# b0nes164/GPUSorting

Measured on NVIDIA H100. Metric: OneSweep sort throughput, 2^30 uint32 keys per GPU, keys-only, uniform-random, higher is better.
Workload: dtype u32

## Files before the change

gpusorting_b200/csrc/osb_common.cuh:

```cuda
#pragma once
#include <cstdint>
#include <type_traits>
#include <cuda_runtime.h>

namespace osb {

constexpr int kRadix = 256;
constexpr int kRadixLog = 8;

constexpr uint64_t kFlagNotReady = 0;
constexpr uint64_t kFlagReduction = 1;
constexpr uint64_t kFlagInclusive = 2;
constexpr uint64_t kFlagMask = 3;
constexpr int kValueBits = 38;
constexpr int kEpochShift = 40;
constexpr uint32_t kEpochMax = (1u << 24) - 1;

__host__ __device__ __forceinline__ uint64_t desc_pack(uint32_t epoch, uint64_t flag, uint64_t value)
{
    return (static_cast<uint64_t>(epoch) << kEpochShift) | ((value & ((1ull << kValueBits) - 1)) << 2) | flag;
}
__host__ __device__ __forceinline__ uint64_t desc_value(uint64_t d) { return (d >> 2) & ((1ull << kValueBits) - 1); }
__host__ __device__ __forceinline__ uint32_t desc_epoch(uint64_t d) { return static_cast<uint32_t>(d >> kEpochShift); }

__device__ __forceinline__ uint32_t lane_id() { uint32_t v; asm("mov.u32 %0, %%laneid;" : "=r"(v)); return v; }
__device__ __forceinline__ uint32_t lanemask_lt() { uint32_t v; asm("mov.u32 %0, %%lanemask_lt;" : "=r"(v)); return v; }

__device__ __forceinline__ uint64_t ld_relaxed_gpu_u64(const uint64_t* p)
{
    uint64_t v;
    asm volatile("ld.relaxed.gpu.global.u64 %0, [%1];" : "=l"(v) : "l"(p) : "memory");
    return v;
}
__device__ __forceinline__ void st_relaxed_gpu_u64(uint64_t* p, uint64_t v)
{
    asm volatile("st.relaxed.gpu.global.u64 [%0], %1;" ::"l"(p), "l"(v) : "memory");
}

template <typename T> __device__ __forceinline__ T ld_stream(const T* p) { return __ldcg(p); }
template <typename T> __device__ __forceinline__ void st_stream(T* p, T v) { __stcs(p, v); }
template <typename T> __device__ __forceinline__ void st_scatter(T* p, T v) { *p = v; }

struct KeyCodec {
    unsigned long long a = 0, b = 0, d = 0;
    uint32_t flags = 0;
};
constexpr uint32_t kCodecEncodeOnLoad = 1u, kCodecDecodeOnStore = 2u;
constexpr uint32_t kCodecFromPlan = 4u;

template <typename KeyT> __device__ __forceinline__ KeyT codec_encode(KeyT k, KeyT a, KeyT b, KeyT d)
{
    using S = typename std::make_signed<KeyT>::type;
    const KeyT sar = static_cast<KeyT>(static_cast<S>(k) >> (sizeof(KeyT) * 8 - 1));
    return k ^ (((sar & a) | b) ^ d);
}
template <typename KeyT> __device__ __forceinline__ KeyT codec_decode(KeyT e, KeyT a, KeyT b, KeyT d)
{
    using S = typename std::make_signed<KeyT>::type;
    e ^= d;
    const KeyT sar = static_cast<KeyT>(static_cast<S>(e) >> (sizeof(KeyT) * 8 - 1));
    return e ^ ((~sar & a) | b);
}

template <typename KeyT> __device__ __forceinline__ uint32_t digit_of(KeyT k, uint32_t shift)
{
    return static_cast<uint32_t>(k >> shift) & (kRadix - 1);
}
template <typename KeyT> __device__ __forceinline__ uint32_t digit_of(KeyT k, uint32_t shift, uint32_t mask)
{
    return static_cast<uint32_t>(k >> shift) & mask;
}

constexpr uint32_t kPlanHotShift = 16;
struct SortPlan {
    uint32_t skip_mask;
    uint32_t executed;
    uint32_t first_exec;
    uint32_t last_exec;
};
__device__ __forceinline__ bool plan_src_is_alt(const SortPlan& pl, uint32_t place)
{
    return __popc(~pl.skip_mask & ((1u << place) - 1u)) & 1u;
}

}
```

gpusorting_b200/csrc/osb_host.cu:

```cuda
#include <cstdio>
#include <cstring>
#include <new>

#include "../../include/onesweep_b200.h"
#include "osb_kernels.cuh"
#include "osb_common.cuh"
#include "osb_internal.h"

namespace {

constexpr int kVersion = 1006;
constexpr int kMaxPlaces = 8;

inline int cuda_status(cudaError_t e) { return e == cudaSuccess ? OSB200_OK : OSB200_ERR_CUDA - static_cast<int>(e); }

#define OSB_TRY(expr)                                      \
    do {                                                   \
        cudaError_t e__ = (expr);                          \
        if (e__ != cudaSuccess) return cuda_status(e__);   \
    } while (0)

struct ControlLayout {
    static constexpr size_t ghist_bytes = kMaxPlaces * osb::kRadix * sizeof(unsigned long long);
    static constexpr size_t ticket_bytes = 64;
    static constexpr size_t zeroed_bytes = ghist_bytes + ticket_bytes;
    static constexpr size_t gbase_bytes = kMaxPlaces * osb::kRadix * sizeof(unsigned long long);
    static constexpr size_t err_bytes = 64;
    static constexpr size_t plan_bytes = 64;
    static constexpr size_t total = zeroed_bytes + gbase_bytes + err_bytes + plan_bytes;
};

}

struct osb200_sorter {
    int device = 0;
    int sm_count = 132;
    uint64_t max_n = 0;
    int key_bytes = 4;
    int value_bytes = 0;
    osb::BinningConfig cfg;
    bool atomic_order_ok = false;
    bool short_circuit = true;
    bool small_path = true;
    bool hot_passes = true;
    bool debug_rows_block = false;

    void* alt_keys = nullptr;
    uint32_t* alt_vals = nullptr;
    unsigned char* control = nullptr;
    uint64_t* desc = nullptr;
    uint16_t* agg16 = nullptr;
    uint64_t desc_tiles = 0;
    uint32_t epoch = 0;

    bool profile = false;
    cudaEvent_t ev[kMaxPlaces + 3] = {};
    int ev_count = 0;

    void* stage_keys = nullptr;
    uint32_t* stage_vals = nullptr;
    cudaStream_t own_stream = nullptr;

    unsigned long long* ghist() const { return reinterpret_cast<unsigned long long*>(control); }
    uint32_t* tickets() const { return reinterpret_cast<uint32_t*>(control + ControlLayout::ghist_bytes); }
    unsigned long long* gbase() const { return reinterpret_cast<unsigned long long*>(control + ControlLayout::zeroed_bytes); }
    unsigned long long* err() const
    {
        return reinterpret_cast<unsigned long long*>(control + ControlLayout::zeroed_bytes + ControlLayout::gbase_bytes);
    }
    osb::SortPlan* plan() const
    {
        return reinterpret_cast<osb::SortPlan*>(control + ControlLayout::zeroed_bytes + ControlLayout::gbase_bytes + ControlLayout::err_bytes);
    }
};

namespace {

uint64_t tiles_for(uint64_t n, uint32_t tile_keys) { return (n + tile_keys - 1) / tile_keys; }
uint64_t agg_tiles_for(uint64_t n, uint32_t tile_keys) { return (tiles_for(n, tile_keys) + 7) / 8 * 8; }

uint32_t smallest_tile(int key_bytes, bool pairs)
{
    osb::BinningConfig c;
    uint32_t t = osb::binning_tile_keys(key_bytes, pairs, c);
    for (int v = 1; v < osb::kNumVariants; ++v) {
        c.variant = v;
        const uint32_t t2 = osb::binning_tile_keys(key_bytes, pairs, c);
        if (t2 < t) t = t2;
    }
    return t;
}

int next_epoch(osb200_sorter* s, cudaStream_t stream, uint32_t* out)
{
    if (s->epoch >= osb::kEpochMax) {
        OSB_TRY(cudaMemsetAsync(s->desc, 0, s->desc_tiles * osb::kRadix * sizeof(uint64_t), stream));
        s->epoch = 0;
    }
    *out = ++s->epoch;
    return OSB200_OK;
}

int is_capturing(cudaStream_t stream, bool* out)
{
    cudaStreamCaptureStatus st = cudaStreamCaptureStatusNone;
    OSB_TRY(cudaStreamGetCaptureInfo(stream, &st));
    *out = st == cudaStreamCaptureStatusActive;
    return OSB200_OK;
}

int check_handle(const osb200_sorter* s) { return s ? OSB200_OK : OSB200_ERR_INVALID_ARG; }

bool overlaps(uintptr_t a, uint64_t alen, uintptr_t b, uint64_t blen) { return a < b + blen && b < a + alen; }

int sort_impl(osb200_sorter* s, int key_bytes, void* d_keys, uint32_t* d_vals, uint64_t n, cudaStream_t stream,
              const osb::KeyCodec* codec = nullptr, int begin_bit = 0, int end_bit = -1, const void* keys_in = nullptr)
{
    const int key_bits = key_bytes * 8;
    if (end_bit < 0) end_bit = key_bits;
    if (begin_bit < 0 || end_bit > key_bits || begin_bit > end_bit) return OSB200_ERR_INVALID_ARG;
    if (n <= 1 || begin_bit == end_bit) return OSB200_OK;
    if (n > s->max_n) return OSB200_ERR_SIZE;
    if (!d_keys || (reinterpret_cast<uintptr_t>(d_keys) & 15u)) return OSB200_ERR_INVALID_ARG;
    if (d_vals && !s->value_bytes) return OSB200_ERR_INVALID_ARG;
    const int places = (end_bit - begin_bit + 7) / 8;
    const uint32_t last_bits = static_cast<uint32_t>(end_bit - begin_bit - 8 * (places - 1));
    const bool whole_key = begin_bit == 0 && end_bit == key_bits;
    const bool wide = s->cfg.variant == osb::kVariantWide;
    if (!wide && !whole_key) return OSB200_ERR_UNSUPPORTED;
    const bool use_plan = wide;

    if (wide && s->small_path && n <= osb::segment_sort_capacity(key_bytes)) {
        osb::KeyCodec c;
        if (codec) { c = *codec; c.flags = osb::kCodecEncodeOnLoad | osb::kCodecDecodeOnStore; }
        s->ev_count = 0;
        OSB_TRY(osb::launch_segment_sort(d_keys, d_vals, key_bytes, nullptr, 1, n, static_cast<uint32_t>(n),
                                         static_cast<uint32_t>(begin_bit), static_cast<uint32_t>(places), last_bits,
                                         codec ? &c : nullptr, s->cfg.rank_mode, s->sm_count, stream, keys_in));
        return OSB200_OK;
    }

    bool capturing = false;
    int st = is_capturing(stream, &capturing);
    if (st != OSB200_OK) return st;
    const uint32_t tile_keys = osb::binning_tile_keys(key_bytes, d_vals != nullptr, s->cfg);
    const size_t desc_bytes = tiles_for(n, tile_keys) * osb::kRadix * sizeof(uint64_t);
    if (capturing) OSB_TRY(cudaMemsetAsync(s->desc, 0, desc_bytes, stream));
    OSB_TRY(cudaMemsetAsync(s->control, 0, ControlLayout::zeroed_bytes, stream));
    const bool compact = s->cfg.variant != osb::kVariantTilePerCta;
    const uint64_t agg_stride = agg_tiles_for(n, tile_keys) * osb::kRadix;
    if (compact) OSB_TRY(cudaMemsetAsync(s->agg16, 0, agg_stride * places * sizeof(uint16_t), stream));
    int ne = 0;
    auto mark = [&]() -> cudaError_t {
        if (!s->profile) return cudaSuccess;
        if (!s->ev[ne]) { cudaError_t e = cudaEventCreate(&s->ev[ne]); if (e != cudaSuccess) return e; }
        return cudaEventRecord(s->ev[ne++], stream);
    };
    s->ev_count = 0;
    OSB_TRY(mark());
    osb::KeyCodec enc;
    if (codec) { enc = *codec; enc.flags = osb::kCodecEncodeOnLoad; }
    if (whole_key)
        OSB_TRY(osb::launch_global_histogram(keys_in ? keys_in : d_keys, n, key_bytes, s->ghist(), s->sm_count, stream,
                                             codec ? &enc : nullptr));
    else
        OSB_TRY(osb::launch_global_histogram_bits(d_keys, n, key_bytes, s->ghist(), s->sm_count, stream, codec ? &enc : nullptr,
                                                  static_cast<uint32_t>(begin_bit), places, last_bits));
    OSB_TRY(mark());
    const bool hot_passes = use_plan && s->hot_passes && osb::binning_has_hot_twin(key_bytes, d_vals != nullptr, keys_in != nullptr, s->cfg);
    OSB_TRY(osb::launch_scan(s->ghist(), s->gbase(), places, stream, use_plan ? s->plan() : nullptr, n, s->short_circuit, hot_passes));
    OSB_TRY(mark());

    void* src = d_keys;
    void* dst = s->alt_keys;
    uint32_t* sv = d_vals;
    uint32_t* dv = d_vals ? s->alt_vals : nullptr;
    for (int p = 0; p < places; ++p) {
        uint32_t epoch = 0;
        st = next_epoch(s, stream, &epoch);
        if (st != OSB200_OK) return st;
        osb::BinningConfig cfg = s->cfg;
        cfg.digit_bits = p == places - 1 ? last_bits : 8u;
        cfg.place = static_cast<uint32_t>(p);
        if (use_plan) cfg.plan = s->plan();
        cfg.hot_passes = hot_passes;
        cfg.argsort_in = keys_in;
        if (codec) {
            cfg.codec = *codec;
            cfg.codec.flags = use_plan ? osb::kCodecFromPlan
                                       : (p == 0 ? osb::kCodecEncodeOnLoad : 0u) | (p == places - 1 ? osb::kCodecDecodeOnStore : 0u);
        }
        OSB_TRY(osb::launch_digit_binning(use_plan ? d_keys : src, use_plan ? s->alt_keys : dst, use_plan ? d_vals : sv,
                                          use_plan ? (d_vals ? s->alt_vals : nullptr) : dv, n, key_bytes,
                                          static_cast<uint32_t>(begin_bit + 8 * p), s->gbase() + p * osb::kRadix, s->desc,
                                          s->agg16 + p * agg_stride, s->tickets() + p, epoch, cfg, stream));
        OSB_TRY(mark());
        void* t = src; src = dst; dst = t;
        uint32_t* tv = sv; sv = dv; dv = tv;
    }
    if (use_plan && (s->short_circuit || (places & 1))) {
        if (keys_in)
            OSB_TRY(osb::launch_argsort_copy_back(s->plan(), keys_in, s->alt_keys, d_keys, s->alt_vals, d_vals, n, key_bytes, s->sm_count,
                                                      stream));
        else
            OSB_TRY(osb::launch_copy_back(s->plan(), s->alt_keys, d_keys, d_vals ? s->alt_vals : nullptr, d_vals, n, key_bytes,
                                          s->sm_count, stream));
    }
    if (capturing) OSB_TRY(cudaMemsetAsync(s->desc, 0, desc_bytes, stream));
    s->ev_count = ne;
    return OSB200_OK;
}

int ensure_staging(osb200_sorter* s)
{
    if (!s->own_stream) OSB_TRY(cudaStreamCreateWithFlags(&s->own_stream, cudaStreamNonBlocking));
    if (!s->stage_keys) {
        if (cudaMalloc(&s->stage_keys, s->max_n * s->key_bytes) != cudaSuccess) return OSB200_ERR_ALLOC;
    }
    if (s->value_bytes && !s->stage_vals) {
        if (cudaMalloc(&s->stage_vals, s->max_n * sizeof(uint32_t)) != cudaSuccess) return OSB200_ERR_ALLOC;
    }
    return OSB200_OK;
}

int sort_host_impl(osb200_sorter* s, void* h_keys, uint32_t* h_vals, uint64_t n)
{
    if (n <= 1) return OSB200_OK;
    if (n > s->max_n) return OSB200_ERR_SIZE;
    if (!h_keys || (h_vals && !s->value_bytes)) return OSB200_ERR_INVALID_ARG;
    int st = ensure_staging(s);
    if (st != OSB200_OK) return st;
    cudaStream_t q = s->own_stream;
    OSB_TRY(cudaMemcpyAsync(s->stage_keys, h_keys, n * s->key_bytes, cudaMemcpyHostToDevice, q));
    if (h_vals) OSB_TRY(cudaMemcpyAsync(s->stage_vals, h_vals, n * sizeof(uint32_t), cudaMemcpyHostToDevice, q));
    st = sort_impl(s, s->key_bytes, s->stage_keys, h_vals ? s->stage_vals : nullptr, n, q);
    if (st != OSB200_OK) return st;
    OSB_TRY(cudaMemcpyAsync(h_keys, s->stage_keys, n * s->key_bytes, cudaMemcpyDeviceToHost, q));
    if (h_vals) OSB_TRY(cudaMemcpyAsync(h_vals, s->stage_vals, n * sizeof(uint32_t), cudaMemcpyDeviceToHost, q));
    OSB_TRY(cudaStreamSynchronize(q));
    return OSB200_OK;
}

}

int osb_internal_digit_histogram(osb200_handle h, const void* d_in, uint64_t n, uint32_t shift,
                                 unsigned long long* d_hist256, cudaStream_t stream)
{
    OSB_TRY(cudaMemsetAsync(d_hist256, 0, osb::kRadix * sizeof(unsigned long long), stream));
    if (n) OSB_TRY(osb::launch_digit_histogram(d_in, n, h->key_bytes, shift, d_hist256, h->sm_count, stream));
    return OSB200_OK;
}

int osb_internal_binning_pass(osb200_handle h, const void* d_in, void* d_out, uint64_t n, uint32_t shift,
                              const unsigned long long* d_hist256, const unsigned long long* out_base,
                              cudaStream_t stream)
{
    if (n == 0) return OSB200_OK;
    if (n > h->max_n) return OSB200_ERR_SIZE;
    const unsigned long long* base = out_base;
    OSB_TRY(cudaMemsetAsync(h->tickets(), 0, ControlLayout::ticket_bytes, stream));
    if (!base) {
        OSB_TRY(osb::launch_scan(d_hist256, h->gbase(), 1, stream));
        base = h->gbase();
    }
    if (h->cfg.variant != osb::kVariantTilePerCta) {
        const uint64_t tiles = agg_tiles_for(n, osb::binning_tile_keys(h->key_bytes, false, h->cfg));
        OSB_TRY(cudaMemsetAsync(h->agg16, 0, tiles * osb::kRadix * sizeof(uint16_t), stream));
    }
    uint32_t epoch = 0;
    int st = next_epoch(h, stream, &epoch);
    if (st != OSB200_OK) return st;
    osb::BinningConfig cfg = h->cfg;
    const uint32_t key_bits = static_cast<uint32_t>(h->key_bytes) * 8u;
    cfg.digit_bits = key_bits - shift < 8u ? key_bits - shift : 8u;
    OSB_TRY(osb::launch_digit_binning(d_in, d_out, nullptr, nullptr, n, h->key_bytes, shift, base, h->desc, h->agg16,
                                      h->tickets(), epoch, cfg, stream));
    return OSB200_OK;
}

extern "C" {

int osb200_version(void) { return kVersion; }

const char* osb200_status_string(int status)
{
    switch (status) {
        case OSB200_OK: return "ok";
        case OSB200_ERR_INVALID_ARG: return "invalid argument";
        case OSB200_ERR_SIZE: return "n exceeds the sorter's max_n";
        case OSB200_ERR_UNSUPPORTED: return "unsupported key/value combination";
        case OSB200_ERR_NO_DEVICE: return "no usable sm_90 CUDA device";
        case OSB200_ERR_ALLOC: return "device allocation failed";
        case OSB200_ERR_NCCL: return "NCCL error";
        default: break;
    }
    if (status <= OSB200_ERR_CUDA) return cudaGetErrorString(static_cast<cudaError_t>(OSB200_ERR_CUDA - status));
    return "unknown status";
}

uint64_t osb200_workspace_bytes(uint64_t max_n, int key_bytes, int value_bytes)
{
    if ((key_bytes != 4 && key_bytes != 8) || (value_bytes != 0 && value_bytes != 4)) return 0;
    const uint64_t tiles = tiles_for(max_n ? max_n : 1, smallest_tile(key_bytes, value_bytes != 0));
    return max_n * key_bytes + max_n * value_bytes + tiles * osb::kRadix * sizeof(uint64_t) +
           (tiles + 8) * osb::kRadix * sizeof(uint16_t) * key_bytes + ControlLayout::total;
}

}

namespace {

int create_impl(osb200_handle* out, uint64_t max_n, int key_bytes, int value_bytes)
{
    if (max_n == 0 || max_n > (1ull << 34)) return OSB200_ERR_INVALID_ARG;

    int dev = 0;
    if (cudaGetDevice(&dev) != cudaSuccess) { cudaGetLastError(); return OSB200_ERR_NO_DEVICE; }
    cudaDeviceProp prop;
    if (cudaGetDeviceProperties(&prop, dev) != cudaSuccess) { cudaGetLastError(); return OSB200_ERR_NO_DEVICE; }
    if (prop.major != 9 || prop.minor != 0) return OSB200_ERR_NO_DEVICE;

    osb200_sorter* s = new (std::nothrow) osb200_sorter();
    if (!s) return OSB200_ERR_ALLOC;
    s->device = dev;
    s->sm_count = prop.multiProcessorCount;
    s->cfg.sm_count = s->sm_count;
    s->cfg.variant = osb::kVariantWide;
    s->max_n = max_n;
    s->key_bytes = key_bytes;
    s->value_bytes = value_bytes;

    cudaError_t e = osb::configure_kernels();
    if (e != cudaSuccess) { delete s; return cuda_status(e); }

    s->desc_tiles = tiles_for(max_n, smallest_tile(key_bytes, value_bytes != 0));
    bool ok = cudaMalloc(&s->alt_keys, max_n * key_bytes) == cudaSuccess;
    if (ok && value_bytes) ok = cudaMalloc(&s->alt_vals, max_n * sizeof(uint32_t)) == cudaSuccess;
    ok = ok && cudaMalloc(&s->control, ControlLayout::total) == cudaSuccess;
    ok = ok && cudaMalloc(&s->desc, s->desc_tiles * osb::kRadix * sizeof(uint64_t)) == cudaSuccess;
    ok = ok && cudaMalloc(&s->agg16, (s->desc_tiles + 8) * osb::kRadix * sizeof(uint16_t) * key_bytes) == cudaSuccess;
    if (!ok) { cudaGetLastError(); osb200_destroy(s); return OSB200_ERR_ALLOC; }
    e = cudaMemset(s->desc, 0, s->desc_tiles * osb::kRadix * sizeof(uint64_t));
    if (e == cudaSuccess) e = cudaMemset(s->control, 0, ControlLayout::total);

    if (e == cudaSuccess) e = osb::launch_atomic_order_selftest(s->err(), s->sm_count, nullptr);
    unsigned long long mism = 1;
    if (e == cudaSuccess) e = cudaMemcpy(&mism, s->err(), sizeof(mism), cudaMemcpyDeviceToHost);
    if (e != cudaSuccess) { osb200_destroy(s); return cuda_status(e); }
    s->atomic_order_ok = (mism == 0);
    s->cfg.rank_mode = s->atomic_order_ok ? osb::kRankAtomic : osb::kRankBallot;
    *out = s;
    return OSB200_OK;
}

}

extern "C" {

int osb200_create(osb200_handle* out, uint64_t max_n, int key_bytes, int value_bytes)
{
    if (!out) return OSB200_ERR_INVALID_ARG;
    *out = nullptr;
    if ((key_bytes != 4 && key_bytes != 8) || (value_bytes != 0 && value_bytes != 4)) return OSB200_ERR_INVALID_ARG;
    if (key_bytes == 8 && value_bytes != 0) return OSB200_ERR_UNSUPPORTED;
    return create_impl(out, max_n, key_bytes, value_bytes);
}

int osb200_create_pairs64(osb200_handle* out, uint64_t max_n)
{
    if (!out) return OSB200_ERR_INVALID_ARG;
    *out = nullptr;
    return create_impl(out, max_n, 8, 4);
}

int osb200_destroy(osb200_handle h)
{
    if (!h) return OSB200_ERR_INVALID_ARG;
    cudaFree(h->alt_keys);
    cudaFree(h->alt_vals);
    cudaFree(h->control);
    cudaFree(h->desc);
    cudaFree(h->agg16);
    cudaFree(h->stage_keys);
    cudaFree(h->stage_vals);
    if (h->own_stream) cudaStreamDestroy(h->own_stream);
    for (cudaEvent_t e : h->ev) if (e) cudaEventDestroy(e);
    delete h;
    return OSB200_OK;
}

int osb200_sort_keys_u32(osb200_handle h, uint32_t* d_keys, uint64_t n, void* stream)
{
    if (check_handle(h) != OSB200_OK || h->key_bytes != 4) return OSB200_ERR_INVALID_ARG;
    return sort_impl(h, h->key_bytes, d_keys, nullptr, n, static_cast<cudaStream_t>(stream));
}

int osb200_sort_pairs_u32(osb200_handle h, uint32_t* d_keys, uint32_t* d_values, uint64_t n, void* stream)
{
    if (check_handle(h) != OSB200_OK || h->key_bytes != 4 || h->value_bytes != 4) return OSB200_ERR_INVALID_ARG;
    if (n > 1 && !d_values) return OSB200_ERR_INVALID_ARG;
    return sort_impl(h, h->key_bytes, d_keys, d_values, n, static_cast<cudaStream_t>(stream));
}

int osb200_sort_keys_u64(osb200_handle h, uint64_t* d_keys, uint64_t n, void* stream)
{
    if (check_handle(h) != OSB200_OK || h->key_bytes != 8) return OSB200_ERR_INVALID_ARG;
    return sort_impl(h, h->key_bytes, d_keys, nullptr, n, static_cast<cudaStream_t>(stream));
}

static int make_codec(int key_bytes, int key_type, int descending, osb::KeyCodec* c, const osb::KeyCodec** codec)
{
    const bool wide64 = key_bytes == 8;
    const unsigned long long all = wide64 ? ~0ull : 0xffffffffull, sign = wide64 ? (1ull << 63) : (1ull << 31);
    switch (key_type) {
        case OSB200_KEY_U32: if (wide64) return OSB200_ERR_INVALID_ARG; c->a = 0; c->b = 0; break;
        case OSB200_KEY_I32: if (wide64) return OSB200_ERR_INVALID_ARG; c->a = 0; c->b = sign; break;
        case OSB200_KEY_F32: if (wide64) return OSB200_ERR_INVALID_ARG; c->a = all; c->b = sign; break;
        case OSB200_KEY_U64: if (!wide64) return OSB200_ERR_INVALID_ARG; c->a = 0; c->b = 0; break;
        case OSB200_KEY_I64: if (!wide64) return OSB200_ERR_INVALID_ARG; c->a = 0; c->b = sign; break;
        case OSB200_KEY_F64: if (!wide64) return OSB200_ERR_INVALID_ARG; c->a = all; c->b = sign; break;
        default: return OSB200_ERR_INVALID_ARG;
    }
    c->d = descending ? all : 0;
    c->flags = 0;
    *codec = c->a == 0 && c->b == 0 && c->d == 0 ? nullptr : c;
    return OSB200_OK;
}

static int make_codec16(int key_type, int descending, osb::KeyCodec* c, const osb::KeyCodec** codec)
{
    switch (key_type) {
        case OSB200_KEY16_U16: c->a = 0; c->b = 0; break;
        case OSB200_KEY16_I16: c->a = 0; c->b = 0x8000u; break;
        case OSB200_KEY16_F16:
        case OSB200_KEY16_BF16: c->a = 0xFFFFu; c->b = 0x8000u; break;
        default: return OSB200_ERR_INVALID_ARG;
    }
    c->d = descending ? 0xFFFFu : 0;
    c->flags = 0;
    *codec = c->a == 0 && c->b == 0 && c->d == 0 ? nullptr : c;
    return OSB200_OK;
}

static int typed_codec(const osb200_sorter* h, int key_bytes, int key_type, int descending, osb::KeyCodec* c, const osb::KeyCodec** codec)
{
    const int st = key_bytes == 2 ? make_codec16(key_type, descending, c, codec) : make_codec(key_bytes, key_type, descending, c, codec);
    if (st != OSB200_OK) return st;
    return h->cfg.variant == osb::kVariantWide ? OSB200_OK : OSB200_ERR_UNSUPPORTED;
}

static int typed_sort(osb200_sorter* h, int key_bytes, void* d_keys, uint32_t* d_vals, bool pairs, uint64_t n, int key_type,
                      int descending, void* stream)
{
    osb::KeyCodec c;
    const osb::KeyCodec* codec = nullptr;
    const int st = typed_codec(h, key_bytes, key_type, descending, &c, &codec);
    if (st != OSB200_OK) return st;
    if (pairs && n > 1 && !d_vals) return OSB200_ERR_INVALID_ARG;
    return sort_impl(h, key_bytes, d_keys, d_vals, n, static_cast<cudaStream_t>(stream), codec);
}

static int argsort_impl(osb200_sorter* h, int key_bytes, const void* d_keys_in, void* d_keys_out, uint32_t* d_indices, uint64_t n,
                        int key_type, int descending, void* stream)
{
    osb::KeyCodec c;
    const osb::KeyCodec* codec = nullptr;
    const int st = typed_codec(h, key_bytes, key_type, descending, &c, &codec);
    if (st != OSB200_OK) return st;
    if (n == 0) return OSB200_OK;
    const uintptr_t in = reinterpret_cast<uintptr_t>(d_keys_in), out = reinterpret_cast<uintptr_t>(d_keys_out),
                    idx = reinterpret_cast<uintptr_t>(d_indices);
    if (!in || !out || !idx || ((in | out | idx) & 15u)) return OSB200_ERR_INVALID_ARG;
    if (n > h->max_n || n > (1ull << 32)) return OSB200_ERR_SIZE;
    const uint64_t kb = n * static_cast<uint64_t>(key_bytes), ib = n * sizeof(uint32_t);
    if (overlaps(in, kb, out, kb) || overlaps(in, kb, idx, ib) || overlaps(out, kb, idx, ib)) return OSB200_ERR_INVALID_ARG;
    cudaStream_t q = static_cast<cudaStream_t>(stream);
    if (n == 1) {
        OSB_TRY(cudaMemcpyAsync(d_keys_out, d_keys_in, key_bytes, cudaMemcpyDeviceToDevice, q));
        OSB_TRY(cudaMemsetAsync(d_indices, 0, sizeof(uint32_t), q));
        return OSB200_OK;
    }
    return sort_impl(h, key_bytes, d_keys_out, d_indices, n, q, codec, 0, -1, d_keys_in);
}

int osb200_sort_keys_typed(osb200_handle h, void* d_keys, uint64_t n, int key_type, int descending, void* stream)
{
    if (check_handle(h) != OSB200_OK) return OSB200_ERR_INVALID_ARG;
    return typed_sort(h, h->key_bytes, d_keys, nullptr, false, n, key_type, descending, stream);
}

int osb200_segmented_sort_u32(osb200_handle h, uint32_t* d_keys, uint32_t* d_values, const uint64_t* d_segment_offsets,
                              uint64_t num_segments, uint32_t max_segment_len, void* stream)
{
    if (check_handle(h) != OSB200_OK) return OSB200_ERR_INVALID_ARG;
    if (h->key_bytes != 4 || (d_values && h->value_bytes != 4)) return OSB200_ERR_INVALID_ARG;
    if (num_segments == 0 || max_segment_len <= 1) return OSB200_OK;
    if (!d_keys || !d_segment_offsets) return OSB200_ERR_INVALID_ARG;
    if (max_segment_len > osb::segment_sort_capacity(4)) return OSB200_ERR_SIZE;
    OSB_TRY(osb::launch_segment_sort(d_keys, d_values, 4, reinterpret_cast<const unsigned long long*>(d_segment_offsets), num_segments,
                                     0, max_segment_len, 0, 4, 8, nullptr, h->cfg.rank_mode, h->sm_count,
                                     static_cast<cudaStream_t>(stream)));
    return OSB200_OK;
}

int osb200_sort_bits(osb200_handle h, void* d_keys, uint32_t* d_values, uint64_t n, int begin_bit, int end_bit, void* stream)
{
    if (check_handle(h) != OSB200_OK) return OSB200_ERR_INVALID_ARG;
    if (d_values && (h->key_bytes != 4 || h->value_bytes != 4)) return OSB200_ERR_INVALID_ARG;
    return sort_impl(h, h->key_bytes, d_keys, d_values, n, static_cast<cudaStream_t>(stream), nullptr, begin_bit, end_bit);
}

int osb200_sort_pairs_typed(osb200_handle h, void* d_keys, uint32_t* d_values, uint64_t n, int key_type, int descending,
                            void* stream)
{
    if (check_handle(h) != OSB200_OK || h->value_bytes != 4) return OSB200_ERR_INVALID_ARG;
    if (n > 1 && !d_values) return OSB200_ERR_INVALID_ARG;
    return typed_sort(h, h->key_bytes, d_keys, d_values, true, n, key_type, descending, stream);
}

int osb200_argsort(osb200_handle h, const void* d_keys_in, void* d_keys_out, uint32_t* d_indices, uint64_t n, int key_type,
                   int descending, void* stream)
{
    if (check_handle(h) != OSB200_OK || h->value_bytes != 4) return OSB200_ERR_INVALID_ARG;
    return argsort_impl(h, h->key_bytes, d_keys_in, d_keys_out, d_indices, n, key_type, descending, stream);
}

int osb200_sort_keys16(osb200_handle h, void* d_keys, uint64_t n, int key_type, int descending, void* stream)
{
    if (check_handle(h) != OSB200_OK || h->key_bytes != 4) return OSB200_ERR_INVALID_ARG;
    return typed_sort(h, 2, d_keys, nullptr, false, n, key_type, descending, stream);
}

int osb200_sort_pairs16(osb200_handle h, void* d_keys, uint32_t* d_values, uint64_t n, int key_type, int descending, void* stream)
{
    if (check_handle(h) != OSB200_OK || h->key_bytes != 4 || h->value_bytes != 4) return OSB200_ERR_INVALID_ARG;
    return typed_sort(h, 2, d_keys, d_values, true, n, key_type, descending, stream);
}

int osb200_argsort16(osb200_handle h, const void* d_keys_in, void* d_keys_out, uint32_t* d_indices, uint64_t n, int key_type,
                     int descending, void* stream)
{
    if (check_handle(h) != OSB200_OK || h->key_bytes != 4 || h->value_bytes != 4) return OSB200_ERR_INVALID_ARG;
    return argsort_impl(h, 2, d_keys_in, d_keys_out, d_indices, n, key_type, descending, stream);
}

int osb200_sort_rows(osb200_handle h, const void* d_keys_in, void* d_keys_out, uint32_t* d_indices, uint64_t num_rows,
                     uint32_t row_len, int key_bytes, int key_type, int descending, void* stream)
{
    if (check_handle(h) != OSB200_OK) return OSB200_ERR_INVALID_ARG;
    osb::KeyCodec c;
    const osb::KeyCodec* codec = nullptr;
    int st = key_bytes == 2 ? make_codec16(key_type, descending, &c, &codec)
             : key_bytes == 4 || key_bytes == 8 ? make_codec(key_bytes, key_type, descending, &c, &codec)
                                                : OSB200_ERR_INVALID_ARG;
    if (st != OSB200_OK) return st;
    if (num_rows == 0 || row_len == 0) return OSB200_OK;
    const uintptr_t in = reinterpret_cast<uintptr_t>(d_keys_in), out = reinterpret_cast<uintptr_t>(d_keys_out),
                    idx = reinterpret_cast<uintptr_t>(d_indices);
    if (!in || !out) return OSB200_ERR_INVALID_ARG;
    if (((in | out) & static_cast<uintptr_t>(key_bytes - 1)) || (idx & 3u)) return OSB200_ERR_INVALID_ARG;
    if (num_rows > UINT64_MAX / row_len) return OSB200_ERR_INVALID_ARG;
    const uint64_t n = num_rows * row_len;
    if (n > UINT64_MAX / 8) return OSB200_ERR_INVALID_ARG;
    const uint64_t kb = n * static_cast<uint64_t>(key_bytes), ib = n * sizeof(uint32_t);
    if ((in != out && overlaps(in, kb, out, kb)) || (idx && (overlaps(in, kb, idx, ib) || overlaps(out, kb, idx, ib))))
        return OSB200_ERR_INVALID_ARG;
    if (row_len > osb::row_sort_capacity(key_bytes)) return OSB200_ERR_SIZE;
    cudaStream_t q = static_cast<cudaStream_t>(stream);
    if (row_len == 1) {
        if (in != out) OSB_TRY(cudaMemcpyAsync(d_keys_out, d_keys_in, kb, cudaMemcpyDeviceToDevice, q));
        if (idx) OSB_TRY(cudaMemsetAsync(d_indices, 0, ib, q));
        return OSB200_OK;
    }
    c.flags = osb::kCodecEncodeOnLoad | osb::kCodecDecodeOnStore;
    OSB_TRY(osb::launch_row_sort(d_keys_in, d_keys_out, d_indices, num_rows, row_len, key_bytes, codec,
                                 h->cfg.rank_mode, h->debug_rows_block, h->sm_count, q));
    return OSB200_OK;
}

int osb200_sort_host_keys_u32(osb200_handle h, uint32_t* h_keys, uint64_t n)
{
    if (check_handle(h) != OSB200_OK || h->key_bytes != 4) return OSB200_ERR_INVALID_ARG;
    return sort_host_impl(h, h_keys, nullptr, n);
}

int osb200_sort_host_pairs_u32(osb200_handle h, uint32_t* h_keys, uint32_t* h_values, uint64_t n)
{
    if (check_handle(h) != OSB200_OK || h->key_bytes != 4 || h->value_bytes != 4) return OSB200_ERR_INVALID_ARG;
    if (n > 1 && !h_values) return OSB200_ERR_INVALID_ARG;
    return sort_host_impl(h, h_keys, h_values, n);
}

int osb200_sort_host_keys_u64(osb200_handle h, uint64_t* h_keys, uint64_t n)
{
    if (check_handle(h) != OSB200_OK || h->key_bytes != 8) return OSB200_ERR_INVALID_ARG;
    return sort_host_impl(h, h_keys, nullptr, n);
}

int osb200_global_histogram(osb200_handle h, const void* d_keys, uint64_t n, uint64_t* d_hist, void* stream)
{
    if (check_handle(h) != OSB200_OK || !d_hist || (n && !d_keys)) return OSB200_ERR_INVALID_ARG;
    if (reinterpret_cast<uintptr_t>(d_keys) & 15u) return OSB200_ERR_INVALID_ARG;
    cudaStream_t q = static_cast<cudaStream_t>(stream);
    OSB_TRY(cudaMemsetAsync(d_hist, 0, static_cast<size_t>(h->key_bytes) * osb::kRadix * sizeof(uint64_t), q));
    if (n == 0) return OSB200_OK;
    OSB_TRY(osb::launch_global_histogram(d_keys, n, h->key_bytes, reinterpret_cast<unsigned long long*>(d_hist),
                                         h->sm_count, q));
    return OSB200_OK;
}

int osb200_digit_binning_pass(osb200_handle h, const void* d_in, void* d_out, const uint32_t* d_in_values,
                              uint32_t* d_out_values, uint64_t n, uint32_t radix_shift, void* stream)
{
    if (check_handle(h) != OSB200_OK) return OSB200_ERR_INVALID_ARG;
    if (n == 0) return OSB200_OK;
    if (!d_in || !d_out || d_in == d_out) return OSB200_ERR_INVALID_ARG;
    if ((reinterpret_cast<uintptr_t>(d_in) & 15u) || (reinterpret_cast<uintptr_t>(d_out) & 15u)) return OSB200_ERR_INVALID_ARG;
    if (n > h->max_n) return OSB200_ERR_SIZE;
    if (radix_shift >= static_cast<uint32_t>(h->key_bytes) * 8u) return OSB200_ERR_INVALID_ARG;
    if ((d_in_values != nullptr) != (d_out_values != nullptr)) return OSB200_ERR_INVALID_ARG;
    if (d_in_values && (h->key_bytes != 4 || h->value_bytes != 4)) return OSB200_ERR_UNSUPPORTED;
    cudaStream_t q = static_cast<cudaStream_t>(stream);
    bool capturing = false;
    int st = is_capturing(q, &capturing);
    if (st != OSB200_OK) return st;
    const size_t desc_bytes = tiles_for(n, osb::binning_tile_keys(h->key_bytes, d_in_values != nullptr, h->cfg)) * osb::kRadix *
                              sizeof(uint64_t);
    if (capturing) OSB_TRY(cudaMemsetAsync(h->desc, 0, desc_bytes, q));
    st = osb_internal_digit_histogram(h, d_in, n, radix_shift, h->ghist(), q);
    if (st != OSB200_OK) return st;
    OSB_TRY(cudaMemsetAsync(h->tickets(), 0, ControlLayout::ticket_bytes, q));
    OSB_TRY(osb::launch_scan(h->ghist(), h->gbase(), 1, q));
    if (h->cfg.variant != osb::kVariantTilePerCta)
        OSB_TRY(cudaMemsetAsync(h->agg16, 0, (h->desc_tiles + 8) * osb::kRadix * sizeof(uint16_t), q));
    uint32_t epoch = 0;
    st = next_epoch(h, q, &epoch);
    if (st != OSB200_OK) return st;
    osb::BinningConfig cfg = h->cfg;
    const uint32_t key_bits = static_cast<uint32_t>(h->key_bytes) * 8u;
    cfg.digit_bits = key_bits - radix_shift < 8u ? key_bits - radix_shift : 8u;
    OSB_TRY(osb::launch_digit_binning(d_in, d_out, d_in_values, d_out_values, n, h->key_bytes, radix_shift, h->gbase(), h->desc,
                                      h->agg16, h->tickets(), epoch, cfg, q));
    if (capturing) OSB_TRY(cudaMemsetAsync(h->desc, 0, desc_bytes, q));
    return OSB200_OK;
}

int osb200_debug_digit_histogram(osb200_handle h, const uint32_t* d_in, uint64_t n, uint32_t shift, uint64_t* d_hist256,
                                 void* stream)
{
    if (check_handle(h) != OSB200_OK || h->key_bytes != 4 || !d_hist256 || shift >= 32) return OSB200_ERR_INVALID_ARG;
    if (n && (!d_in || (reinterpret_cast<uintptr_t>(d_in) & 15u))) return OSB200_ERR_INVALID_ARG;
    if (n > h->max_n) return OSB200_ERR_SIZE;
    return osb_internal_digit_histogram(h, d_in, n, shift, reinterpret_cast<unsigned long long*>(d_hist256),
                                        static_cast<cudaStream_t>(stream));
}

int osb200_debug_exchange_pass(osb200_handle h, const uint32_t* d_in, uint32_t* d_out, uint64_t n, uint32_t shift,
                               const uint64_t* d_hist256, const uint64_t* d_out_base, void* stream)
{
    if (check_handle(h) != OSB200_OK || h->key_bytes != 4 || shift >= 32) return OSB200_ERR_INVALID_ARG;
    if (d_out_base && d_out) return OSB200_ERR_INVALID_ARG;
    if (n == 0) return OSB200_OK;
    if (!d_in || (reinterpret_cast<uintptr_t>(d_in) & 15u) || d_in == d_out) return OSB200_ERR_INVALID_ARG;
    if (!d_out_base && (!d_out || !d_hist256 || (reinterpret_cast<uintptr_t>(d_out) & 3u))) return OSB200_ERR_INVALID_ARG;
    if (n > h->max_n) return OSB200_ERR_SIZE;
    return osb_internal_binning_pass(h, d_in, d_out, n, shift, reinterpret_cast<const unsigned long long*>(d_hist256),
                                     reinterpret_cast<const unsigned long long*>(d_out_base), static_cast<cudaStream_t>(stream));
}

int osb200_validate(osb200_handle h, const void* d_keys, uint64_t n, uint64_t* h_err_count, void* stream)
{
    if (check_handle(h) != OSB200_OK || !h_err_count) return OSB200_ERR_INVALID_ARG;
    *h_err_count = 0;
    if (n < 2) return OSB200_OK;
    if (!d_keys) return OSB200_ERR_INVALID_ARG;
    cudaStream_t q = static_cast<cudaStream_t>(stream);
    OSB_TRY(cudaMemsetAsync(h->err(), 0, sizeof(unsigned long long), q));
    OSB_TRY(osb::launch_validate(d_keys, n, h->key_bytes, h->err(), h->sm_count, q));
    unsigned long long v = 0;
    OSB_TRY(cudaMemcpyAsync(&v, h->err(), sizeof(v), cudaMemcpyDeviceToHost, q));
    OSB_TRY(cudaStreamSynchronize(q));
    *h_err_count = v;
    return OSB200_OK;
}

int osb200_init_random_u32(uint32_t* d_keys, uint32_t* d_payload, uint64_t n, uint32_t and_count, uint32_t seed,
                           int payload_is_index, void* stream)
{
    if (n == 0) return OSB200_OK;
    if (!d_keys) return OSB200_ERR_INVALID_ARG;
    OSB_TRY(osb::launch_init_random(d_keys, d_payload, n, and_count, seed, payload_is_index != 0,
                                    static_cast<cudaStream_t>(stream)));
    return OSB200_OK;
}

int osb200_set_option(osb200_handle h, const char* key, int64_t value)
{
    if (check_handle(h) != OSB200_OK || !key) return OSB200_ERR_INVALID_ARG;
    if (!std::strcmp(key, "rank_mode")) {
        if (value != osb::kRankAtomic && value != osb::kRankBallot) return OSB200_ERR_INVALID_ARG;
        if (value == osb::kRankAtomic && !h->atomic_order_ok) return OSB200_ERR_UNSUPPORTED;
        h->cfg.rank_mode = static_cast<int>(value);
        return OSB200_OK;
    }
    if (!std::strcmp(key, "profile")) { h->profile = value != 0; return OSB200_OK; }
    if (!std::strcmp(key, "short_circuit")) { h->short_circuit = value != 0; return OSB200_OK; }
    if (!std::strcmp(key, "small_path")) { h->small_path = value != 0; return OSB200_OK; }
    if (!std::strcmp(key, "hot_passes")) { h->hot_passes = value != 0; return OSB200_OK; }
    if (!std::strcmp(key, "spin_cap")) {
        if (value < 1 || value > (1ll << 30)) return OSB200_ERR_INVALID_ARG;
        h->cfg.spin_cap = static_cast<uint32_t>(value);
        return OSB200_OK;
    }
    if (!std::strcmp(key, "debug_stall_every")) {
        if (value < 0 || value > (1ll << 30)) return OSB200_ERR_INVALID_ARG;
        h->cfg.debug_stall_every = static_cast<uint32_t>(value);
        return OSB200_OK;
    }
    if (!std::strcmp(key, "debug_max_ctas")) {
        if (value < 0 || value > (1ll << 30)) return OSB200_ERR_INVALID_ARG;
        h->cfg.debug_max_ctas = static_cast<uint32_t>(value);
        return OSB200_OK;
    }
    if (!std::strcmp(key, "debug_rows_block")) { h->debug_rows_block = value != 0; return OSB200_OK; }
    if (!std::strcmp(key, "debug_epoch")) {
        if (value < 0 || value > osb::kEpochMax) return OSB200_ERR_INVALID_ARG;
        h->epoch = static_cast<uint32_t>(value);
        return OSB200_OK;
    }
    if (!std::strcmp(key, "variant")) {
        if (value < 0 || value >= osb::kNumVariants) return OSB200_ERR_INVALID_ARG;
        h->cfg.variant = static_cast<int>(value);
        return OSB200_OK;
    }
    return OSB200_ERR_INVALID_ARG;
}

int osb200_get_profile(osb200_handle h, float* out_ms, int capacity)
{
    if (check_handle(h) != OSB200_OK || !out_ms) return OSB200_ERR_INVALID_ARG;
    if (h->ev_count < 2) return 0;
    OSB_TRY(cudaEventSynchronize(h->ev[h->ev_count - 1]));
    int k = 0;
    for (int i = 0; i + 1 < h->ev_count && k < capacity; ++i, ++k) OSB_TRY(cudaEventElapsedTime(&out_ms[k], h->ev[i], h->ev[i + 1]));
    return k;
}

int64_t osb200_get_info(osb200_handle h, const char* key)
{
    if (check_handle(h) != OSB200_OK || !key) return OSB200_ERR_INVALID_ARG;
    if (!std::strcmp(key, "tile_keys")) return osb::binning_tile_keys(h->key_bytes, h->value_bytes != 0, h->cfg);
    if (!std::strcmp(key, "launches_per_sort")) {
        const bool wide = h->cfg.variant == osb::kVariantWide;
        const bool cb = wide && h->short_circuit;
        return 2 + h->key_bytes * ((wide && h->hot_passes) ? 2 : 1) + (cb ? (h->value_bytes ? 2 : 1) : 0);
    }
    if (!std::strcmp(key, "memsets_per_sort")) return h->cfg.variant != osb::kVariantTilePerCta ? 2 : 1;
    if (!std::strcmp(key, "short_circuit")) return h->short_circuit ? 1 : 0;
    if (!std::strcmp(key, "small_path")) return h->small_path ? 1 : 0;
    if (!std::strcmp(key, "hot_passes")) return h->hot_passes ? 1 : 0;
    if (!std::strcmp(key, "last_hot_mask")) {
        osb::SortPlan pl;
        if (cudaMemcpy(&pl, h->plan(), sizeof(pl), cudaMemcpyDeviceToHost) != cudaSuccess) return -1;
        return static_cast<int>((pl.skip_mask >> osb::kPlanHotShift) & 0xffu);
    }
    if (!std::strcmp(key, "small_path_max_n")) return osb::segment_sort_capacity(h->key_bytes);
    if (!std::strcmp(key, "spin_cap")) return h->cfg.spin_cap;
    if (!std::strcmp(key, "last_skip_mask") || !std::strcmp(key, "last_executed_passes")) {
        osb::SortPlan pl;
        if (cudaMemcpy(&pl, h->plan(), sizeof(pl), cudaMemcpyDeviceToHost) != cudaSuccess) return OSB200_ERR_CUDA;
        return key[5] == 's' ? static_cast<int64_t>(pl.skip_mask & 0xffffu) : static_cast<int64_t>(pl.executed);
    }
    if (!std::strcmp(key, "sm_count")) return h->sm_count;
    if (!std::strcmp(key, "rank_mode")) return h->cfg.rank_mode;
    if (!std::strcmp(key, "variant")) return h->cfg.variant;
    if (!std::strcmp(key, "atomic_order_ok")) return h->atomic_order_ok ? 1 : 0;
    if (!std::strcmp(key, "max_n")) return static_cast<int64_t>(h->max_n);
    if (!std::strcmp(key, "epoch")) return h->epoch;
    return OSB200_ERR_INVALID_ARG;
}

}
```

gpusorting_b200/csrc/osb_kernels.cu:

```cuda
#include <type_traits>

#include "osb_kernels.cuh"
#include "osb_common.cuh"

namespace osb {

template <typename... Ts> struct TypeList {};

template <typename... Ts, typename F>
static cudaError_t for_each_type(TypeList<Ts...>, F&& f)
{
    cudaError_t e = cudaSuccess;
    (void)(((e = f(Ts{})) == cudaSuccess) && ...);
    return e;
}

template <typename... Ts, typename M, typename F>
static cudaError_t find_type(TypeList<Ts...>, M&& match, F&& f)
{
    cudaError_t e = cudaErrorInvalidValue;
    (void)((match(Ts{}) && ((e = f(Ts{})), true)) || ...);
    return e;
}

template <typename... Keys, typename F>
static cudaError_t with_key_type(TypeList<Keys...> keys, int key_bytes, F&& f)
{
    return find_type(keys, [&](auto k) { return key_bytes == static_cast<int>(sizeof(k)); }, f);
}

template <typename F>
static cudaError_t with_rank_mode(int rank_mode, F&& f)
{
    return rank_mode == kRankBallot ? f(std::integral_constant<int, kRankBallot>{}) : f(std::integral_constant<int, kRankAtomic>{});
}

static unsigned capped_grid(uint64_t work, uint64_t per_cta, uint64_t cap)
{
    uint64_t want = (work + per_cta - 1) / per_cta;
    if (want < 1) want = 1;
    return static_cast<unsigned>(want < cap ? want : cap);
}

template <typename K>
static cudaError_t set_smem(K* kernel, size_t bytes)
{
    return cudaFuncSetAttribute(kernel, cudaFuncAttributeMaxDynamicSharedMemorySize, static_cast<int>(bytes));
}

template <typename Shape>
static cudaError_t configure_shape(Shape)
{
    cudaError_t e = set_smem(Shape::template kernel<kRankAtomic>(), Shape::smem);
    if (e == cudaSuccess) e = set_smem(Shape::template kernel<kRankBallot>(), Shape::smem);
    if constexpr (Shape::has_hot) {
        if (e == cudaSuccess) e = set_smem(Shape::template kernel<kRankAtomic, true>(), Shape::smem);
        if (e == cudaSuccess) e = set_smem(Shape::template kernel<kRankBallot, true>(), Shape::smem);
    }
    return e;
}

constexpr int kHistThreads = 1024;

template <typename KeyT> struct HistGeom;
template <> struct HistGeom<uint32_t> { static constexpr int COLS = 32; };
template <> struct HistGeom<uint64_t> { static constexpr int COLS = 16; };
template <> struct HistGeom<uint16_t> { static constexpr int COLS = 32; };

template <typename KeyT, bool MASKED = false>
__device__ __forceinline__ void hist_count_word(uint32_t* s_col, uint32_t w, int word_in_vec, int places = 0, uint32_t last_mask = 255u)
{
    constexpr int PLACES = sizeof(KeyT);
    constexpr int COLS = HistGeom<KeyT>::COLS;
#pragma unroll
    for (int q = 0; q < 4; ++q) {
        const int place = (word_in_vec * 4 + q) % PLACES;
        if constexpr (MASKED) {
            if (place < places)
                atomicAdd(&s_col[(place * kRadix + ((w >> (8 * q)) & (place == places - 1 ? last_mask : 255u))) * COLS], 1u);
        } else {
            atomicAdd(&s_col[(place * kRadix + ((w >> (8 * q)) & 255u)) * COLS], 1u);
        }
    }
}

template <typename KeyT>
__device__ __forceinline__ uint4 hist_encode_vec(uint4 v, const KeyCodec& c)
{
    if constexpr (sizeof(KeyT) == 4) {
        const uint32_t a = static_cast<uint32_t>(c.a), b = static_cast<uint32_t>(c.b), d = static_cast<uint32_t>(c.d);
        v.x = codec_encode<uint32_t>(v.x, a, b, d); v.y = codec_encode<uint32_t>(v.y, a, b, d);
        v.z = codec_encode<uint32_t>(v.z, a, b, d); v.w = codec_encode<uint32_t>(v.w, a, b, d);
    } else if constexpr (sizeof(KeyT) == 2) {
        const uint16_t a = static_cast<uint16_t>(c.a), b = static_cast<uint16_t>(c.b), d = static_cast<uint16_t>(c.d);
        auto enc2 = [&](uint32_t w) {
            return static_cast<uint32_t>(codec_encode<uint16_t>(static_cast<uint16_t>(w), a, b, d)) |
                   (static_cast<uint32_t>(codec_encode<uint16_t>(static_cast<uint16_t>(w >> 16), a, b, d)) << 16);
        };
        v.x = enc2(v.x); v.y = enc2(v.y); v.z = enc2(v.z); v.w = enc2(v.w);
    } else {
        unsigned long long k0 = (static_cast<unsigned long long>(v.y) << 32) | v.x, k1 = (static_cast<unsigned long long>(v.w) << 32) | v.z;
        k0 = codec_encode<unsigned long long>(k0, c.a, c.b, c.d); k1 = codec_encode<unsigned long long>(k1, c.a, c.b, c.d);
        v.x = static_cast<uint32_t>(k0); v.y = static_cast<uint32_t>(k0 >> 32); v.z = static_cast<uint32_t>(k1); v.w = static_cast<uint32_t>(k1 >> 32);
    }
    return v;
}

template <typename KeyT, bool MASKED = false>
__device__ __forceinline__ void hist_count_vec(uint32_t* s_col, const uint4& v, int places = 0, uint32_t last_mask = 255u)
{
    hist_count_word<KeyT, MASKED>(s_col, v.x, 0, places, last_mask);
    hist_count_word<KeyT, MASKED>(s_col, v.y, 1, places, last_mask);
    hist_count_word<KeyT, MASKED>(s_col, v.z, 2, places, last_mask);
    hist_count_word<KeyT, MASKED>(s_col, v.w, 3, places, last_mask);
}

template <typename KeyT, bool MASKED = false>
__global__ void __launch_bounds__(kHistThreads, 1)
global_histogram_kernel(const KeyT* __restrict__ keys, uint64_t n, unsigned long long* __restrict__ ghist, KeyCodec codec,
                        int places = 0, uint32_t last_mask = 255u)
{
    constexpr int PLACES = sizeof(KeyT);
    constexpr int VEC = 16 / sizeof(KeyT);
    constexpr int COLS = HistGeom<KeyT>::COLS;
    constexpr int BINS = PLACES * kRadix;
    extern __shared__ __align__(16) uint32_t s_hist[];
    for (int i = threadIdx.x; i < BINS * COLS; i += kHistThreads) s_hist[i] = 0;
    __syncthreads();
    uint32_t* s_col = s_hist + (threadIdx.x & (COLS - 1));

    const uint64_t nvec = n / VEC;
    const uint4* __restrict__ vp = reinterpret_cast<const uint4*>(keys);
    const uint64_t stride = static_cast<uint64_t>(gridDim.x) * kHistThreads;
    uint64_t i = static_cast<uint64_t>(blockIdx.x) * kHistThreads + threadIdx.x;
    const bool enc = codec.flags & kCodecEncodeOnLoad;
    for (; i + 3 * stride < nvec; i += 4 * stride) {
        uint4 a = __ldcs(vp + i);
        uint4 b = __ldcs(vp + i + stride);
        uint4 c = __ldcs(vp + i + 2 * stride);
        uint4 d = __ldcs(vp + i + 3 * stride);
        if (enc) { a = hist_encode_vec<KeyT>(a, codec); b = hist_encode_vec<KeyT>(b, codec); c = hist_encode_vec<KeyT>(c, codec); d = hist_encode_vec<KeyT>(d, codec); }
        hist_count_vec<KeyT, MASKED>(s_col, a, places, last_mask);
        hist_count_vec<KeyT, MASKED>(s_col, b, places, last_mask);
        hist_count_vec<KeyT, MASKED>(s_col, c, places, last_mask);
        hist_count_vec<KeyT, MASKED>(s_col, d, places, last_mask);
    }
    for (; i < nvec; i += stride) {
        uint4 a = __ldcs(vp + i);
        if (enc) a = hist_encode_vec<KeyT>(a, codec);
        hist_count_vec<KeyT, MASKED>(s_col, a, places, last_mask);
    }
    if (blockIdx.x == 0) {
        const uint64_t t = nvec * VEC + threadIdx.x;
        if (t < n) {
            KeyT k = keys[t];
            if (enc) k = codec_encode<KeyT>(k, static_cast<KeyT>(codec.a), static_cast<KeyT>(codec.b), static_cast<KeyT>(codec.d));
#pragma unroll
            for (int p = 0; p < PLACES; ++p) {
                if (MASKED && p >= places) break;
                const uint32_t m = (MASKED && p == places - 1) ? last_mask : 255u;
                atomicAdd(&s_col[(p * kRadix + (static_cast<uint32_t>(k >> (8 * p)) & m)) * COLS], 1u);
            }
        }
    }
    __syncthreads();
    for (int bin = threadIdx.x; bin < BINS; bin += kHistThreads) {
        uint32_t sum = 0;
#pragma unroll 8
        for (int c = 0; c < COLS; ++c) sum += s_hist[bin * COLS + ((c + threadIdx.x) & (COLS - 1))];
        if (sum) atomicAdd(&ghist[bin], static_cast<unsigned long long>(sum));
    }
}

template <typename KeyT> constexpr size_t hist_smem_bytes() { return sizeof(KeyT) * kRadix * HistGeom<KeyT>::COLS * sizeof(uint32_t); }

using HistKeys = TypeList<uint16_t, uint32_t, uint64_t>;
using HistBitsKeys = TypeList<uint32_t, uint64_t>;

template <typename KeyT, bool MASKED>
static cudaError_t launch_histogram_vec(const void* keys, uint64_t n, unsigned long long* ghist, int sm_count, cudaStream_t stream,
                                        const KeyCodec& codec, int places = 0, uint32_t last_mask = 255u)
{
    const unsigned grid = capped_grid(n / (16 / sizeof(KeyT)), kHistThreads, sm_count);
    global_histogram_kernel<KeyT, MASKED><<<grid, kHistThreads, hist_smem_bytes<KeyT>(), stream>>>(
        static_cast<const KeyT*>(keys), n, ghist, codec, places, last_mask);
    return cudaGetLastError();
}

cudaError_t launch_global_histogram(const void* keys, uint64_t n, int key_bytes, unsigned long long* ghist,
                                    int sm_count, cudaStream_t stream, const KeyCodec* codec_in)
{
    const KeyCodec codec = codec_in ? *codec_in : KeyCodec();
    return with_key_type(HistKeys{}, key_bytes, [&](auto k) {
        return launch_histogram_vec<decltype(k), false>(keys, n, ghist, sm_count, stream, codec);
    });
}

template <typename KeyT>
__global__ void __launch_bounds__(kHistThreads, 1)
digit_histogram_kernel(const KeyT* __restrict__ keys, uint64_t n, uint32_t shift, unsigned long long* __restrict__ hist256)
{
    __shared__ uint32_t s_hist[kRadix * 32];
    for (int i = threadIdx.x; i < kRadix * 32; i += kHistThreads) s_hist[i] = 0;
    __syncthreads();
    uint32_t* s_col = s_hist + (threadIdx.x & 31);
    const uint64_t stride = static_cast<uint64_t>(gridDim.x) * kHistThreads;
    uint64_t i = static_cast<uint64_t>(blockIdx.x) * kHistThreads + threadIdx.x;
    for (; i + 3 * stride < n; i += 4 * stride) {
        const KeyT a = __ldcs(keys + i), b = __ldcs(keys + i + stride), c = __ldcs(keys + i + 2 * stride),
                   d = __ldcs(keys + i + 3 * stride);
        atomicAdd(&s_col[digit_of(a, shift) * 32], 1u);
        atomicAdd(&s_col[digit_of(b, shift) * 32], 1u);
        atomicAdd(&s_col[digit_of(c, shift) * 32], 1u);
        atomicAdd(&s_col[digit_of(d, shift) * 32], 1u);
    }
    for (; i < n; i += stride) atomicAdd(&s_col[digit_of(__ldcs(keys + i), shift) * 32], 1u);
    __syncthreads();
    for (int bin = threadIdx.x; bin < kRadix; bin += kHistThreads) {
        uint32_t sum = 0;
#pragma unroll 8
        for (int c = 0; c < 32; ++c) sum += s_hist[bin * 32 + ((c + threadIdx.x) & 31)];
        if (sum) atomicAdd(&hist256[bin], static_cast<unsigned long long>(sum));
    }
}

cudaError_t launch_digit_histogram(const void* keys, uint64_t n, int key_bytes, uint32_t shift,
                                   unsigned long long* hist256, int sm_count, cudaStream_t stream)
{
    const unsigned grid = capped_grid(n, kHistThreads * 4, static_cast<uint64_t>(sm_count) * 2);
    return with_key_type(TypeList<uint32_t, uint64_t>{}, key_bytes, [&](auto k) {
        using KeyT = decltype(k);
        digit_histogram_kernel<KeyT><<<grid, kHistThreads, 0, stream>>>(static_cast<const KeyT*>(keys), n, shift, hist256);
        return cudaGetLastError();
    });
}

__global__ void __launch_bounds__(kRadix)
scan_kernel(const unsigned long long* __restrict__ ghist, unsigned long long* __restrict__ gbase, int places,
            SortPlan* plan, unsigned long long n, int allow_skip, int allow_hot)
{
    __shared__ unsigned long long s_warp[kRadix / 32];
    const int d = threadIdx.x, lane = d & 31, warp = d >> 5;
    uint32_t skip_mask = 0;
    for (int p = 0; p < places; ++p) {
        const unsigned long long c = ghist[p * kRadix + d];
        unsigned long long incl = c;
#pragma unroll
        for (int o = 1; o < 32; o <<= 1) {
            const unsigned long long t = __shfl_up_sync(0xffffffffu, incl, o);
            if (lane >= o) incl += t;
        }
        if (lane == 31) s_warp[warp] = incl;
        const int single_bin = __syncthreads_or(plan != nullptr && allow_skip && c == n);
        const int hot_bin = __syncthreads_or(plan != nullptr && allow_hot && n >= (1ull << 22) && c * 8ull >= n);
        unsigned long long pre = 0;
        for (int w = 0; w < warp; ++w) pre += s_warp[w];
        gbase[p * kRadix + d] = pre + incl - c;
        if (single_bin) skip_mask |= 1u << p;
        else if (hot_bin) skip_mask |= 1u << (kPlanHotShift + p);
        __syncthreads();
    }
    if (plan != nullptr && d == 0) {
        SortPlan pl;
        pl.skip_mask = skip_mask;
        const uint32_t run = ~skip_mask & ((places >= 32 ? 0u : (1u << places)) - 1u);
        pl.executed = __popc(run);
        pl.first_exec = run ? static_cast<uint32_t>(__ffs(run) - 1) : 0xffffffffu;
        pl.last_exec = run ? static_cast<uint32_t>(31 - __clz(run)) : 0xffffffffu;
        *plan = pl;
    }
}

cudaError_t launch_scan(const unsigned long long* ghist, unsigned long long* gbase, int places, cudaStream_t stream,
                        SortPlan* plan, uint64_t n, bool allow_skip, bool allow_hot)
{
    scan_kernel<<<1, kRadix, 0, stream>>>(ghist, gbase, places, plan, n, allow_skip ? 1 : 0, allow_hot ? 1 : 0);
    return cudaGetLastError();
}

template <typename KeyT>
__global__ void __launch_bounds__(kHistThreads, 1)
global_histogram_bits_kernel(const KeyT* __restrict__ keys, uint64_t n, unsigned long long* __restrict__ ghist, KeyCodec codec,
                             uint32_t begin_bit, int places, uint32_t last_mask)
{
    constexpr int COLS = HistGeom<KeyT>::COLS;
    extern __shared__ __align__(16) uint32_t s_hist[];
    const int bins = places * kRadix;
    for (int i = threadIdx.x; i < bins * COLS; i += kHistThreads) s_hist[i] = 0;
    __syncthreads();
    uint32_t* s_col = s_hist + (threadIdx.x & (COLS - 1));
    const bool enc = codec.flags & kCodecEncodeOnLoad;
    const KeyT ca = static_cast<KeyT>(codec.a), cb = static_cast<KeyT>(codec.b), cd = static_cast<KeyT>(codec.d);
    const uint64_t stride = static_cast<uint64_t>(gridDim.x) * kHistThreads;
    for (uint64_t i = static_cast<uint64_t>(blockIdx.x) * kHistThreads + threadIdx.x; i < n; i += stride) {
        KeyT k = __ldcs(keys + i);
        if (enc) k = codec_encode<KeyT>(k, ca, cb, cd);
        for (int p = 0; p < places; ++p) {
            const uint32_t dg = digit_of(k, begin_bit + 8u * p, p == places - 1 ? last_mask : 255u);
            atomicAdd(&s_col[(p * kRadix + dg) * COLS], 1u);
        }
    }
    __syncthreads();
    for (int bin = threadIdx.x; bin < bins; bin += kHistThreads) {
        uint32_t sum = 0;
#pragma unroll 8
        for (int c = 0; c < COLS; ++c) sum += s_hist[bin * COLS + ((c + threadIdx.x) & (COLS - 1))];
        if (sum) atomicAdd(&ghist[bin], static_cast<unsigned long long>(sum));
    }
}

cudaError_t launch_global_histogram_bits(const void* keys, uint64_t n, int key_bytes, unsigned long long* ghist, int sm_count,
                                         cudaStream_t stream, const KeyCodec* codec_in, uint32_t begin_bit, int places,
                                         uint32_t last_bits)
{
    const KeyCodec codec = codec_in ? *codec_in : KeyCodec();
    const uint32_t last_mask = (1u << last_bits) - 1u;
    return with_key_type(HistBitsKeys{}, key_bytes, [&](auto k) {
        using KeyT = decltype(k);
        if (begin_bit == 0) return launch_histogram_vec<KeyT, true>(keys, n, ghist, sm_count, stream, codec, places, last_mask);
        global_histogram_bits_kernel<KeyT><<<capped_grid(n, kHistThreads * 4, sm_count), kHistThreads, hist_smem_bytes<KeyT>(), stream>>>(
            static_cast<const KeyT*>(keys), n, ghist, codec, begin_bit, places, last_mask);
        return cudaGetLastError();
    });
}

template <typename W>
__global__ void __launch_bounds__(512)
copy_back_kernel(const SortPlan* __restrict__ plan, const W* __restrict__ src, W* __restrict__ dst, uint64_t words,
                 const unsigned char* __restrict__ src_tail, unsigned char* __restrict__ dst_tail, uint32_t tail_bytes)
{
    if (!(plan->executed & 1u)) return;
    const uint64_t stride = static_cast<uint64_t>(gridDim.x) * blockDim.x;
    for (uint64_t i = static_cast<uint64_t>(blockIdx.x) * blockDim.x + threadIdx.x; i < words; i += stride) __stcs(dst + i, __ldcs(src + i));
    if (blockIdx.x == 0 && threadIdx.x < tail_bytes) dst_tail[threadIdx.x] = src_tail[threadIdx.x];
}

cudaError_t launch_copy_back(const SortPlan* plan, const void* alt_keys, void* keys, const uint32_t* alt_vals, uint32_t* vals,
                             uint64_t n, int key_bytes, int sm_count, cudaStream_t stream)
{
    auto launch = [&](auto word, const void* s, void* d, uint64_t bytes) {
        using W = decltype(word);
        const uint64_t words = bytes / sizeof(W);
        copy_back_kernel<W><<<capped_grid(words, 512, static_cast<uint64_t>(sm_count) * 4), 512, 0, stream>>>(plan, static_cast<const W*>(s), static_cast<W*>(d), words,
                                                      static_cast<const unsigned char*>(s) + words * sizeof(W),
                                                      static_cast<unsigned char*>(d) + words * sizeof(W),
                                                      static_cast<uint32_t>(bytes - words * sizeof(W)));
    };
    auto one = [&](const void* s, void* d, uint64_t bytes) {
        if (((reinterpret_cast<uintptr_t>(s) | reinterpret_cast<uintptr_t>(d)) & 15u) == 0) launch(uint4{}, s, d, bytes);
        else launch(uint32_t{}, s, d, bytes);
    };
    one(alt_keys, keys, n * key_bytes);
    if (vals) one(alt_vals, vals, n * sizeof(uint32_t));
    return cudaGetLastError();
}

template <typename KeyT>
__global__ void __launch_bounds__(512)
argsort_copy_back_kernel(const SortPlan* __restrict__ plan, const KeyT* __restrict__ keys_in, const KeyT* __restrict__ alt_keys,
                         KeyT* __restrict__ keys, const uint32_t* __restrict__ alt_idx, uint32_t* __restrict__ idx, uint64_t n)
{
    using KV = typename std::conditional<sizeof(KeyT) == 2, uint2, uint4>::type;
    constexpr int KV_PER_STEP = 4 * sizeof(KeyT) / sizeof(KV);
    static_assert(KV_PER_STEP * sizeof(KV) == 4 * sizeof(KeyT), "four keys per step");
    const uint32_t ex = plan->executed;
    if (ex != 0 && !(ex & 1u)) return;
    const KeyT* src = ex ? alt_keys : keys_in;
    const uint64_t vecs = n / 4, stride = static_cast<uint64_t>(gridDim.x) * blockDim.x;
    for (uint64_t i = static_cast<uint64_t>(blockIdx.x) * blockDim.x + threadIdx.x; i < vecs; i += stride) {
#pragma unroll
        for (int v = 0; v < KV_PER_STEP; ++v)
            __stcs(reinterpret_cast<KV*>(keys) + i * KV_PER_STEP + v, __ldcs(reinterpret_cast<const KV*>(src) + i * KV_PER_STEP + v));
        const uint32_t b = static_cast<uint32_t>(i * 4);
        __stcs(reinterpret_cast<uint4*>(idx) + i, ex ? __ldcs(reinterpret_cast<const uint4*>(alt_idx) + i) : make_uint4(b, b + 1, b + 2, b + 3));
    }
    if (blockIdx.x == 0 && threadIdx.x < (n & 3u)) {
        const uint64_t j = vecs * 4 + threadIdx.x;
        keys[j] = src[j];
        idx[j] = ex ? alt_idx[j] : static_cast<uint32_t>(j);
    }
}

cudaError_t launch_argsort_copy_back(const SortPlan* plan, const void* keys_in, const void* alt_keys, void* keys,
                                     const uint32_t* alt_idx, uint32_t* idx, uint64_t n, int key_bytes, int sm_count,
                                     cudaStream_t stream)
{
    const unsigned grid = capped_grid(n / 4, 512, static_cast<uint64_t>(sm_count) * 4);
    return with_key_type(TypeList<uint16_t, uint32_t, uint64_t>{}, key_bytes, [&](auto k) {
        using KeyT = decltype(k);
        argsort_copy_back_kernel<KeyT><<<grid, 512, 0, stream>>>(plan, static_cast<const KeyT*>(keys_in), static_cast<const KeyT*>(alt_keys),
                                                                 static_cast<KeyT*>(keys), alt_idx, idx, n);
        return cudaGetLastError();
    });
}


__device__ __forceinline__ uint32_t warp_match_digit(uint32_t d)
{
    uint32_t m = 0xffffffffu;
#pragma unroll
    for (int b = 0; b < kRadixLog; ++b) {
        const bool p = (d >> b) & 1u;
        const uint32_t bal = __ballot_sync(0xffffffffu, p);
        m &= p ? bal : ~bal;
    }
    return m;
}

template <int RANK_MODE>
__device__ __forceinline__ uint32_t warp_rank_and_count(uint32_t* wh, uint32_t d, uint32_t lt_mask)
{
    if constexpr (RANK_MODE == kRankAtomic) {
        (void)lt_mask;
        return atomicAdd(&wh[d], 1u);
    } else {
        const uint32_t m = warp_match_digit(d);
        const uint32_t below = __popc(m & lt_mask);
        uint32_t pre = 0;
        if (below == 0) { pre = wh[d]; wh[d] = pre + __popc(m); }
        __syncwarp();
        pre = __shfl_sync(0xffffffffu, pre, __ffs(m) - 1);
        return pre + below;
    }
}

template <int THREADS>
__device__ __forceinline__ uint32_t block_excl_scan_256(uint32_t c, uint32_t* s_wtot )
{
    const int tid = threadIdx.x, lane = tid & 31, warp = tid >> 5;
    uint32_t incl = c;
#pragma unroll
    for (int o = 1; o < 32; o <<= 1) {
        const uint32_t t = __shfl_up_sync(0xffffffffu, incl, o);
        if (lane >= o) incl += t;
    }
    if (tid < kRadix && lane == 31) s_wtot[warp] = incl;
    __syncthreads();
    uint32_t pre = 0;
    if (tid < kRadix) {
#pragma unroll
        for (int w = 0; w < kRadix / 32; ++w) pre += (w < warp) ? s_wtot[w] : 0u;
    }
    return pre + incl - c;
}

__device__ __forceinline__ unsigned long long
lookback_and_publish(uint64_t* desc, uint32_t tile, uint32_t d, uint32_t tile_count, uint32_t epoch,
                     const unsigned long long* __restrict__ gbase)
{
    uint64_t* mine = desc + static_cast<uint64_t>(tile) * kRadix + d;
    unsigned long long excl = 0;
    int64_t k = static_cast<int64_t>(tile) - 1;
    while (true) {
        if (k < 0) break;
        const uint64_t v = ld_relaxed_gpu_u64(desc + static_cast<uint64_t>(k) * kRadix + d);
        const uint64_t flag = v & kFlagMask;
        if (desc_epoch(v) != epoch || flag == kFlagNotReady) { __nanosleep(20); continue; }
        excl += desc_value(v);
        if (flag == kFlagInclusive) break;
        --k;
    }
    st_relaxed_gpu_u64(mine, desc_pack(epoch, kFlagInclusive, excl + tile_count));
    return excl + gbase[d];
}

template <typename KeyT, bool PAIRS, int K, int WARPS, int RANK_MODE>
__global__ void __launch_bounds__(WARPS * 32, (RANK_MODE == kRankAtomic && !PAIRS) ? 2 : 1)
digit_binning_tile_kernel(const KeyT* __restrict__ in, KeyT* __restrict__ out, const uint32_t* __restrict__ in_val,
                          uint32_t* __restrict__ out_val, uint64_t n, uint32_t shift,
                          const unsigned long long* __restrict__ gbase, uint64_t* desc, uint32_t* ticket, uint32_t epoch)
{
    constexpr int THREADS = WARPS * 32;
    constexpr int T = THREADS * K;
    static_assert(WARPS >= 8, "need one thread per digit");
    extern __shared__ __align__(128) unsigned char s_raw[];
    uint32_t* s_hist = reinterpret_cast<uint32_t*>(s_raw);
    KeyT* s_keys = reinterpret_cast<KeyT*>(s_raw);
    uint32_t* s_vals = reinterpret_cast<uint32_t*>(s_raw);
    __shared__ unsigned long long s_keyptr[kRadix];
    __shared__ unsigned long long s_valptr[PAIRS ? kRadix : 1];
    __shared__ uint32_t s_wtot[kRadix / 32];
    __shared__ uint32_t s_tile;

    const int tid = threadIdx.x, lane = tid & 31, warp = tid >> 5;

    for (int i = tid; i < WARPS * kRadix; i += THREADS) s_hist[i] = 0;
    if (tid == 0) s_tile = atomicAdd(ticket, 1u);
    __syncthreads();
    const uint32_t tile = s_tile;
    const uint64_t tile_base = static_cast<uint64_t>(tile) * T;
    const uint32_t valid = static_cast<uint32_t>(n - tile_base < static_cast<uint64_t>(T) ? n - tile_base : T);

    KeyT key[K];
    const uint32_t warp_off = warp * (32 * K) + lane;
    if (valid == T) {
#pragma unroll
        for (int i = 0; i < K; ++i) key[i] = ld_stream(in + tile_base + warp_off + i * 32);
    } else {
#pragma unroll
        for (int i = 0; i < K; ++i) {
            const uint32_t idx = warp_off + i * 32;
            key[i] = idx < valid ? in[tile_base + idx] : static_cast<KeyT>(~static_cast<KeyT>(0));
        }
    }

    uint32_t off[K];
    uint32_t* wh = s_hist + warp * kRadix;
    const uint32_t lt = lanemask_lt();
#pragma unroll
    for (int i = 0; i < K; ++i) off[i] = warp_rank_and_count<RANK_MODE>(wh, digit_of(key[i], shift), lt);
    __syncthreads();

    uint32_t tile_count = 0, tile_excl = 0;
    {
        if (tid < kRadix) {
#pragma unroll
            for (int w = 0; w < WARPS; ++w) tile_count += s_hist[w * kRadix + tid];
            st_relaxed_gpu_u64(desc + static_cast<uint64_t>(tile) * kRadix + tid,
                               desc_pack(epoch, kFlagReduction, tile_count));
        }
        tile_excl = block_excl_scan_256<THREADS>(tile_count, s_wtot);
        if (tid < kRadix) {
            uint32_t run = tile_excl;
#pragma unroll
            for (int w = 0; w < WARPS; ++w) { const uint32_t c = s_hist[w * kRadix + tid]; s_hist[w * kRadix + tid] = run; run += c; }
        }
    }
    __syncthreads();

#pragma unroll
    for (int i = 0; i < K; ++i) off[i] += wh[digit_of(key[i], shift)];
    __syncthreads();

#pragma unroll
    for (int i = 0; i < K; ++i) s_keys[off[i]] = key[i];

    uint32_t val[PAIRS ? K : 1];
    if constexpr (PAIRS) {
#pragma unroll
        for (int i = 0; i < K; ++i) {
            const uint32_t idx = warp_off + i * 32;
            val[i] = idx < valid ? ld_stream(in_val + tile_base + idx) : 0u;
        }
    }

    if (tid < kRadix) {
        const unsigned long long excl = lookback_and_publish(desc, tile, tid, tile_count, epoch, gbase);
        const unsigned long long first = excl - tile_excl;
        s_keyptr[tid] = reinterpret_cast<unsigned long long>(out) + first * sizeof(KeyT);
        if constexpr (PAIRS) s_valptr[tid] = reinterpret_cast<unsigned long long>(out_val) + first * sizeof(uint32_t);
    }
    __syncthreads();

    uint32_t dg[PAIRS ? K : 1];
#pragma unroll
    for (int j = 0; j < K; ++j) {
        const uint32_t idx = j * THREADS + tid;
        if (idx < valid) {
            const KeyT k = s_keys[idx];
            const uint32_t d = digit_of(k, shift);
            if constexpr (PAIRS) dg[j] = d;
            KeyT* dst = reinterpret_cast<KeyT*>(s_keyptr[d]) + idx;
            st_stream(dst, k);
        }
    }
    if constexpr (PAIRS) {
        __syncthreads();
#pragma unroll
        for (int i = 0; i < K; ++i) s_vals[off[i]] = val[i];
        __syncthreads();
#pragma unroll
        for (int j = 0; j < K; ++j) {
            const uint32_t idx = j * THREADS + tid;
            if (idx < valid) {
                uint32_t* dst = reinterpret_cast<uint32_t*>(s_valptr[dg[j]]) + idx;
                st_stream(dst, s_vals[idx]);
            }
        }
    }
}

__device__ __forceinline__ uint32_t smem_addr(const void* p) { return static_cast<uint32_t>(__cvta_generic_to_shared(p)); }

__device__ __forceinline__ void mbar_init(uint64_t* bar, uint32_t count)
{
    asm volatile("mbarrier.init.shared::cta.b64 [%0], %1;" ::"r"(smem_addr(bar)), "r"(count) : "memory");
}
__device__ __forceinline__ void mbar_expect_tx(uint64_t* bar, uint32_t bytes)
{
    asm volatile("mbarrier.arrive.expect_tx.shared::cta.b64 _, [%0], %1;" ::"r"(smem_addr(bar)), "r"(bytes) : "memory");
}
__device__ __forceinline__ void mbar_wait(uint64_t* bar, uint32_t parity)
{
    asm volatile(
        "{\n\t.reg .pred p;\n\t"
        "WAIT_%=:\n\t"
        "mbarrier.try_wait.parity.shared::cta.b64 p, [%0], %1;\n\t"
        "@p bra DONE_%=;\n\t"
        "bra WAIT_%=;\n\t"
        "DONE_%=:\n\t}" ::"r"(smem_addr(bar)), "r"(parity) : "memory");
}
__device__ __forceinline__ void tma_load_1d(void* dst_smem, const void* src_gmem, uint32_t bytes, uint64_t* bar)
{
    asm volatile("cp.async.bulk.shared::cluster.global.mbarrier::complete_tx::bytes [%0], [%1], %2, [%3];" ::"r"(
                     smem_addr(dst_smem)),
                 "l"(src_gmem), "r"(bytes), "r"(smem_addr(bar))
                 : "memory");
}
__device__ __forceinline__ void fence_proxy_async_smem() { asm volatile("fence.proxy.async.shared::cta;" ::: "memory"); }
__device__ __forceinline__ void fence_mbar_init() { asm volatile("fence.mbarrier_init.release.cluster;" ::: "memory"); }

#ifndef OSB_PHASE_PROBE
#define OSB_PHASE_PROBE 0
#endif

#if OSB_PHASE_PROBE
__device__ unsigned long long g_phase[11];
#define OSB_PHASE(i) do { if (tid == 0) { const long long t_now = clock64(); atomicAdd(&g_phase[i], static_cast<unsigned long long>(t_now - t_prev)); t_prev = t_now; } } while (0)
}
extern "C" __attribute__((visibility("default"))) int osb200_debug_phases(unsigned long long* out11 , int reset)
{
    if (out11) cudaMemcpyFromSymbol(out11, osb::g_phase, sizeof(osb::g_phase));
    if (reset) { unsigned long long z[11] = {0}; cudaMemcpyToSymbol(osb::g_phase, z, sizeof(z)); }
    return 0;
}
namespace osb {
#else
#define OSB_PHASE(i) do {} while (0)
#endif

constexpr uint32_t kAggReady = 0x8000u;

__device__ __forceinline__ void st_relaxed_gpu_u16(uint16_t* p, uint32_t v)
{
    asm volatile("st.relaxed.gpu.global.u16 [%0], %1;" ::"l"(p), "h"(static_cast<uint16_t>(v)) : "memory");
}

template <typename KeyT>
struct TileRereduce {
    const KeyT* in;
    uint32_t tile_keys;
    uint32_t shift, mask;
    bool encode;
    KeyT ca, cb, cd;
};

template <typename KeyT>
__device__ __noinline__ uint32_t rereduce_tile(const KeyT* p, uint32_t tile_keys, uint32_t shift, uint32_t mask, uint32_t encode,
                                               KeyT ca, KeyT cb, KeyT cd, uint16_t* dst, uint32_t d)
{
    uint32_t c = 0;
#pragma unroll 8
    for (uint32_t i = 0; i < tile_keys; ++i) {
        KeyT k = p[i];
        if (encode) k = codec_encode<KeyT>(k, ca, cb, cd);
        c += digit_of(k, shift, mask) == d;
    }
    st_relaxed_gpu_u16(dst, kAggReady | c);
    return c;
}

__device__ __forceinline__ uint64_t agg_index(uint64_t tile, uint32_t d) { return ((tile >> 3) * kRadix + d) * 8 + (tile & 7); }

__device__ __forceinline__ uint4 ld_relaxed_gpu_v4(const void* p)
{
    uint4 v;
    asm volatile("ld.relaxed.gpu.global.v4.u32 {%0, %1, %2, %3}, [%4];" : "=r"(v.x), "=r"(v.y), "=r"(v.z), "=r"(v.w) : "l"(p) : "memory");
    return v;
}
__device__ __forceinline__ uint32_t agg_elem(const uint4& v, int t)
{
    const uint32_t w = t < 2 ? v.x : t < 4 ? v.y : t < 6 ? v.z : v.w;
    return (t & 1) ? (w >> 16) : (w & 0xffffu);
}

template <int NBLK, typename KeyT>
__device__ __forceinline__ unsigned long long
lookback_wide(uint16_t* agg16, const uint64_t* incl64, uint32_t tile, uint32_t d, uint32_t epoch, uint32_t spin_cap,
              const TileRereduce<KeyT>& rr)
{
    unsigned long long sum = 0;
    int64_t cur = static_cast<int64_t>(tile) - 1;
    uint32_t polls = 0;
    while (true) {
        if (cur < 0) return sum;
#if OSB_PHASE_PROBE
        if (d == 0) atomicAdd(&g_phase[9], 1ull);
#endif
        const int64_t b0 = cur >> 3;
        uint4 v[NBLK];
        uint64_t c[NBLK];
#pragma unroll
        for (int k = 0; k < NBLK; ++k) {
            const int64_t b = b0 - k;
            v[k] = b >= 0 ? ld_relaxed_gpu_v4(agg16 + (static_cast<uint64_t>(b) * kRadix + d) * 8)
                          : make_uint4(0x80008000u, 0x80008000u, 0x80008000u, 0x80008000u);
            c[k] = b > 0 ? ld_relaxed_gpu_u64(incl64 + (static_cast<uint64_t>(b) * 8 - 1) * kRadix + d) : 0ull;
        }
        unsigned long long run = sum;
        int64_t next = (b0 - NBLK + 1) * 8 - 1;
        bool stalled = false;
        const int hi0 = static_cast<int>(cur & 7);
#pragma unroll
        for (int k = 0; k < NBLK; ++k) {
            const int64_t b = b0 - k;
            if (b < 0) return run;
#pragma unroll
            for (int t = 7; t >= 0; --t) {
                if (k == 0 && t > hi0) continue;
                const uint32_t a = agg_elem(v[k], t);
                if (!(a & kAggReady)) { next = b * 8 + t; stalled = true; break; }
                run += a & 0x7fffu;
            }
            if (stalled) break;
            if (b == 0) return run;
            if (desc_epoch(c[k]) == epoch && (c[k] & kFlagMask) == kFlagInclusive) return run + desc_value(c[k]);
        }
        sum = run;
        if (stalled) {
            polls = next == cur ? polls + 1 : 1;
            if (polls > spin_cap) {
                const uint64_t w = ld_relaxed_gpu_u64(incl64 + next * kRadix + d);
                if (desc_epoch(w) == epoch && (w & kFlagMask) == kFlagInclusive) return sum + desc_value(w);
                sum += rereduce_tile<KeyT>(rr.in + static_cast<uint64_t>(next) * rr.tile_keys, rr.tile_keys, rr.shift, rr.mask,
                                           rr.encode ? 1u : 0u, rr.ca, rr.cb, rr.cd, agg16 + agg_index(next, d), d);
                --next;
                polls = 0;
            } else {
#if OSB_PHASE_PROBE
                if (d == 0) atomicAdd(&g_phase[10], 1ull);
#endif
                __nanosleep(40);
            }
        } else {
            polls = 0;
        }
        cur = next;
    }
}


constexpr uint32_t kNoHotDigit = 0xffffffffu;
#ifndef OSB_HOT_MINB
#define OSB_HOT_MINB 1
#endif

__device__ __forceinline__ void hot_digit_publish(uint32_t tile_count, uint32_t* s_wmax)
{
    const int tid = threadIdx.x;
    if (tid < kRadix) {
        const uint32_t m = __reduce_max_sync(0xffffffffu, (tile_count << 8) | static_cast<uint32_t>(tid));
        if ((tid & 31) == 0) s_wmax[tid >> 5] = m;
    }
}
__device__ __forceinline__ uint32_t hot_digit_of_tile(const uint32_t* s_wmax, uint32_t tile_keys)
{
    uint32_t m = 0;
#pragma unroll
    for (int w = 0; w < kRadix / 32; ++w) m = max(m, s_wmax[w]);
    m = __shfl_sync(0xffffffffu, m, 0);
    return (m >> 8) >= tile_keys / 8 ? (m & 255u) : kNoHotDigit;
}

struct PassParams {
    uint32_t shift;
    uint32_t dbits;
    uint32_t epoch;
    uint32_t place;
    uint32_t spin_cap;
    uint32_t stall_every;
    const SortPlan* plan;
    const void* keys_in = nullptr;
};

constexpr uint32_t kPlanBitsFirstIndices = 8u;

__device__ __forceinline__ uint32_t opaque_copy(const uint32_t* smem_copy)
{
    return *reinterpret_cast<const volatile uint32_t*>(smem_copy);
}

template <typename KeyT, bool PAIRS, int K, int WARPS>
struct WideSmem {
    static constexpr int THREADS = WARPS * 32;
    static constexpr int T = THREADS * K;
    static constexpr bool KV_IN_SORTED = PAIRS && sizeof(KeyT) == 2;
    alignas(16) KeyT sorted[KV_IN_SORTED ? T * 8 / sizeof(KeyT) : T];
    alignas(16) uint32_t sorted_val[PAIRS && !KV_IN_SORTED ? T : 4];
    alignas(16) uint32_t hist[WARPS * kRadix];
    unsigned long long keyptr[kRadix];
    unsigned long long valptr[PAIRS ? kRadix : 1];
    uint32_t run[32];
    uint32_t wtot[kRadix / 32];
    uint32_t wmax[kRadix / 32];
    uint32_t next_tile;
    uint32_t plan_bits;
    uint32_t digit_shift, digit_mask;
};

template <typename KeyT, bool PAIRS, int K, int WARPS, int RANK_MODE, int LOOK, int MINB, bool HOT = false, bool INDICES = false>
__global__ void __launch_bounds__(WARPS * 32, HOT ? OSB_HOT_MINB : MINB)
digit_binning_wide_kernel(KeyT* buf0, KeyT* buf1, uint32_t* val0, uint32_t* val1, uint64_t n,
                          const unsigned long long* __restrict__ gbase, uint16_t* agg16, uint64_t* incl64,
                          uint32_t* ticket, PassParams pp, KeyCodec codec)
{
    static_assert(!INDICES || PAIRS, "the indices are the 32-bit payloads of a pairs pass");
    using S = WideSmem<KeyT, PAIRS, K, WARPS>;
    constexpr int THREADS = S::THREADS;
    constexpr int T = S::T;
    static_assert(T < 32768, "agg16 holds 15-bit counts");
    extern __shared__ __align__(128) unsigned char s_raw[];
    S& sm = *reinterpret_cast<S*>(s_raw);
    constexpr bool KV_WORD = PAIRS && sizeof(KeyT) <= 4;
    static_assert(!PAIRS || (sizeof(KeyT) == 4 && offsetof(S, sorted_val) == offsetof(S, sorted) + sizeof(KeyT) * T) ||
                  (S::KV_IN_SORTED && sizeof(S::sorted) == sizeof(uint2) * T) ||
                  (sizeof(KeyT) == 8 && sizeof(S::sorted) == sizeof(KeyT) * T && sizeof(S::sorted_val) == sizeof(uint32_t) * T),
                  "kv layout");
    uint2* const kv = reinterpret_cast<uint2*>(sm.sorted);
    auto put_slot = [&](uint32_t slot, KeyT k, uint32_t v) {
        if constexpr (KV_WORD) kv[slot] = make_uint2(static_cast<uint32_t>(k), v);
        else { sm.sorted[slot] = k; sm.sorted_val[slot] = v; }
    };
    auto get_slot = [&](uint32_t x, KeyT& k, uint32_t& v) {
        if constexpr (KV_WORD) { const uint2 e = kv[x]; k = static_cast<KeyT>(e.x); v = e.y; }
        else { k = sm.sorted[x]; v = sm.sorted_val[x]; }
    };

    const int tid = threadIdx.x, lane = tid & 31, warp = tid >> 5;
    const uint32_t lt = lanemask_lt();
    uint32_t* wh = sm.hist + warp * kRadix;
    const uint32_t shift = pp.shift, epoch = pp.epoch;
    const uint32_t dmask = (1u << pp.dbits) - 1u;
#if OSB_PHASE_PROBE
    long long t_prev = clock64();
#endif

    uint32_t my_bits = (codec.flags & (kCodecEncodeOnLoad | kCodecDecodeOnStore)) << 1;
    bool my_skip = false, my_hot = false;
    if (pp.plan != nullptr) {
        const uint4 raw = __ldg(reinterpret_cast<const uint4*>(pp.plan));
        SortPlan pl; pl.skip_mask = raw.x; pl.executed = raw.y; pl.first_exec = raw.z; pl.last_exec = raw.w;
        my_skip = (pl.skip_mask >> pp.place) & 1u;
        my_hot = (pl.skip_mask >> (kPlanHotShift + pp.place)) & 1u;
        my_bits = plan_src_is_alt(pl, pp.place) ? 1u : 0u;
        if (codec.flags & kCodecFromPlan)
            my_bits |= (pp.place == pl.first_exec ? kCodecEncodeOnLoad << 1 : 0u) | (pp.place == pl.last_exec ? kCodecDecodeOnStore << 1 : 0u);
        if constexpr (INDICES) my_bits |= pp.place == pl.first_exec ? kPlanBitsFirstIndices : 0u;
    }
    if (my_skip) return;
    if (HOT != my_hot) return;
    const uint32_t num_tiles = static_cast<uint32_t>((n + T - 1) / T);

    using KeyReg = typename std::conditional<sizeof(KeyT) == 2 && !PAIRS, uint32_t, KeyT>::type;
    KeyReg key[K];
    uint32_t val[PAIRS ? K : 1];
    const uint32_t warp_off = warp * (32 * K) + lane;
    auto load_tile = [&](uint32_t t) {
        const bool swap = my_bits & 1u;
        const bool iota = INDICES && (my_bits & kPlanBitsFirstIndices);
        const KeyT* __restrict__ in = iota ? static_cast<const KeyT*>(pp.keys_in) : swap ? buf1 : buf0;
        const uint32_t* __restrict__ in_val = swap ? val1 : val0;
        const uint64_t base = static_cast<uint64_t>(t) * T;
        const uint32_t pos0 = static_cast<uint32_t>(base) + warp_off;
        if (base + T <= n) {
#pragma unroll
            for (int i = 0; i < K; ++i) key[i] = ld_stream(in + base + warp_off + i * 32);
            if constexpr (PAIRS) {
                if (iota) {
#pragma unroll
                    for (int i = 0; i < K; ++i) val[i] = pos0 + i * 32;
                } else {
#pragma unroll
                    for (int i = 0; i < K; ++i) val[i] = ld_stream(in_val + base + warp_off + i * 32);
                }
            }
        } else {
            const uint32_t live = base < n ? static_cast<uint32_t>(n - base) : 0u;
#pragma unroll
            for (int i = 0; i < K; ++i) {
                const uint32_t idx = warp_off + i * 32;
                key[i] = idx < live ? in[base + idx] : static_cast<KeyT>(~static_cast<KeyT>(0));
                if constexpr (PAIRS) val[i] = iota ? pos0 + i * 32 : idx < live ? in_val[base + idx] : 0u;
            }
        }
    };

    uint32_t tile = blockIdx.x;
    load_tile(tile);
    {
        uint4* h4 = reinterpret_cast<uint4*>(sm.hist);
        for (int i = tid; i < WARPS * kRadix / 4; i += THREADS) h4[i] = make_uint4(0, 0, 0, 0);
    }
    if (tid == 0) { sm.plan_bits = my_bits; sm.digit_shift = shift; sm.digit_mask = dmask; }
    __syncthreads();
    constexpr bool kPersistent = (sizeof(KeyT) <= 4 && !PAIRS) || HOT;
    while (true) {
    const uint64_t tile_base = static_cast<uint64_t>(tile) * T;
    const bool full = tile_base + T <= n;
    const uint32_t valid = full ? T : static_cast<uint32_t>(n - tile_base);
    OSB_PHASE(0);

    if ((sm.plan_bits >> 1) & kCodecEncodeOnLoad) {
        const KeyT ca = static_cast<KeyT>(codec.a), cb = static_cast<KeyT>(codec.b), cd = static_cast<KeyT>(codec.d);
#pragma unroll
        for (int i = 0; i < K; ++i) {
            key[i] = codec_encode<KeyT>(static_cast<KeyT>(key[i]), ca, cb, cd);
            if (!full && warp_off + i * 32 >= valid) key[i] = static_cast<KeyT>(~static_cast<KeyT>(0));
        }
    }

#if OSB_PHASE_PROBE
#pragma unroll
    for (int i = 0; i < K; ++i) asm volatile("" ::"l"(static_cast<unsigned long long>(key[i])));
    OSB_PHASE(1);
#endif
#pragma unroll
    for (int i = 0; i < K; ++i) atomicAdd(&wh[digit_of(key[i], shift, dmask)], 1u);
    __syncthreads();
    OSB_PHASE(2);
    uint32_t drawn = 0;
    if (kPersistent && tid == 0) drawn = atomicAdd(ticket, 1u);

    uint32_t tile_count = 0, tile_excl = 0;
    if (tid < kRadix) {
#pragma unroll
        for (int w = 0; w < WARPS; ++w) tile_count += sm.hist[w * kRadix + tid];
        if (pp.stall_every == 0 || (tile % pp.stall_every) != pp.stall_every - 1)
            st_relaxed_gpu_u16(agg16 + agg_index(tile, tid), kAggReady | tile_count);
    }
    if constexpr (HOT) hot_digit_publish(tile_count, sm.wmax);
    tile_excl = block_excl_scan_256<THREADS>(tile_count, sm.wtot);
    if (tid < kRadix) {
        uint32_t run = tile_excl;
#pragma unroll
        for (int w = 0; w < WARPS; ++w) { const uint32_t c = sm.hist[w * kRadix + tid]; sm.hist[w * kRadix + tid] = run; run += c; }
    }
    if (tid == 0) sm.next_tile = kPersistent ? gridDim.x + drawn : num_tiles;
    __syncthreads();
    OSB_PHASE(3);

    auto chained_scan = [&]() {
        if (tid < kRadix) {
            TileRereduce<KeyT> rr;
            rr.in = (INDICES && (sm.plan_bits & kPlanBitsFirstIndices)) ? static_cast<const KeyT*>(pp.keys_in)
                    : (sm.plan_bits & 1u) ? buf1 : buf0;
            rr.tile_keys = T; rr.shift = shift; rr.mask = dmask;
            rr.encode = (sm.plan_bits >> 1) & kCodecEncodeOnLoad;
            rr.ca = static_cast<KeyT>(codec.a); rr.cb = static_cast<KeyT>(codec.b); rr.cd = static_cast<KeyT>(codec.d);
            const unsigned long long prior = lookback_wide<LOOK / 8, KeyT>(agg16, incl64, tile, tid, epoch, pp.spin_cap, rr);
            const bool swap = sm.plan_bits & 1u;
            KeyT* out = swap ? buf0 : buf1;
            uint32_t* out_val = swap ? val0 : val1;
            st_relaxed_gpu_u64(incl64 + static_cast<uint64_t>(tile) * kRadix + tid,
                               desc_pack(epoch, kFlagInclusive, prior + tile_count));
            const unsigned long long first = gbase[tid] + prior - tile_excl;
            sm.keyptr[tid] = reinterpret_cast<unsigned long long>(out) + first * sizeof(KeyT);
            if constexpr (PAIRS) sm.valptr[tid] = reinterpret_cast<unsigned long long>(out_val) + first * sizeof(uint32_t);
            if (tid < 32) {
                const uint32_t pad_digit = digit_of(static_cast<KeyT>(~static_cast<KeyT>(0)), shift, dmask);
                const uint32_t live = tile_count - ((tid == pad_digit && !full) ? (T - valid) : 0u);
                sm.run[tid] = tile_excl | (live << 16);
            }
        }
    };

    constexpr bool kRecompute = RANK_MODE == kRankAtomic && !HOT;
    const uint32_t rshift = kRecompute ? opaque_copy(&sm.digit_shift) : shift;
    const uint32_t rmask = kRecompute ? opaque_copy(&sm.digit_mask) : dmask;
    uint32_t hot = kNoHotDigit;
    if constexpr (HOT && RANK_MODE == kRankAtomic) hot = hot_digit_of_tile(sm.wmax, T);
    if (HOT && hot != kNoHotDigit) {
        uint32_t hot_run = __shfl_sync(0xffffffffu, wh[hot], 0);
#pragma unroll
        for (int i = 0; i < K; ++i) {
            const uint32_t d = digit_of(key[i], rshift, rmask);
            const bool is_hot = d == hot;
            const uint32_t b = __ballot_sync(0xffffffffu, is_hot);
            uint32_t slot = hot_run + __popc(b & lt);
            if (!is_hot) slot = warp_rank_and_count<RANK_MODE>(wh, d, lt);
            hot_run += __popc(b);
            if constexpr (PAIRS) put_slot(slot, key[i], val[i]);
            else sm.sorted[slot] = key[i];
        }
    } else {
#pragma unroll
        for (int i = 0; i < K; ++i) {
            const uint32_t slot = warp_rank_and_count<RANK_MODE>(wh, digit_of(key[i], rshift, rmask), lt);
            if constexpr (PAIRS) put_slot(slot, key[i], val[i]);
            else sm.sorted[slot] = key[i];
        }
    }
    __syncwarp();
    {
        uint4* r4 = reinterpret_cast<uint4*>(wh);
#pragma unroll
        for (int i = lane; i < kRadix / 4; i += 32) r4[i] = make_uint4(0, 0, 0, 0);
    }

    const uint32_t next = sm.next_tile;
    if constexpr (kPersistent) { if (!HOT || warp >= kRadix / 32) load_tile(next); }
    OSB_PHASE(4);
    chained_scan();
    OSB_PHASE(5);
    __syncthreads();
    OSB_PHASE(8);
    if constexpr (HOT) { if (warp < kRadix / 32) load_tile(next); }

    const bool dec = (sm.plan_bits >> 1) & kCodecDecodeOnStore;
    const KeyT ca = static_cast<KeyT>(codec.a), cb = static_cast<KeyT>(codec.b), cd = static_cast<KeyT>(codec.d);
    long long val_delta = 0;
    if constexpr (PAIRS && sizeof(KeyT) == 4) {
        const bool swap = sm.plan_bits & 1u;
        val_delta = reinterpret_cast<const char*>(swap ? val0 : val1) - reinterpret_cast<const char*>(swap ? buf0 : buf1);
    }
    auto val_dst = [&](KeyT* dst, uint32_t d, uint32_t x) -> uint32_t* {
        if constexpr (sizeof(KeyT) == 4) return reinterpret_cast<uint32_t*>(reinterpret_cast<char*>(dst) + val_delta);
        else return reinterpret_cast<uint32_t*>(sm.valptr[d]) + x;
    };
    (void)val_dst;
    auto slot_key = [&](uint32_t x) -> KeyT { if constexpr (KV_WORD) return static_cast<KeyT>(kv[x].x); else return sm.sorted[x]; };
    (void)slot_key;
    if (pp.dbits <= 5) {
        const uint32_t nbins = 1u << pp.dbits;
        for (uint32_t b = 0; b < nbins; ++b) {
            const uint32_t rd = sm.run[b];
            const uint32_t lo = rd & 0xffffu, len = rd >> 16;
            if (len == 0) continue;
            const unsigned long long kp = sm.keyptr[b];
            constexpr uint32_t kLine = 128 / sizeof(KeyT);
            const uint32_t ga = static_cast<uint32_t>((kp / sizeof(KeyT) + lo) & (kLine - 1));
            const uint32_t total = len + ga;
            for (uint32_t p = tid; p < total; p += THREADS) {
                if (p >= ga) {
                    const uint32_t x = lo + p - ga;
                    if constexpr (PAIRS) {
                        KeyT k;
                        uint32_t v;
                        get_slot(x, k, v);
                        if (dec) k = codec_decode<KeyT>(k, ca, cb, cd);
                        KeyT* dst = reinterpret_cast<KeyT*>(kp) + x;
                        st_scatter(dst, k);
                        st_scatter(val_dst(dst, b, x), v);
                    } else {
                        KeyT k = sm.sorted[x];
                        if (dec) k = codec_decode<KeyT>(k, ca, cb, cd);
                        st_scatter(reinterpret_cast<KeyT*>(kp) + x, k);
                    }
                }
            }
        }
    } else if (full && !dec) {
#pragma unroll
        for (int j = 0; j < K; ++j) {
            const uint32_t idx = j * THREADS + tid;
            if constexpr (PAIRS) {
                KeyT k;
                uint32_t v;
                get_slot(idx, k, v);
                const uint32_t d = digit_of(k, shift, dmask);
                KeyT* dst = reinterpret_cast<KeyT*>(sm.keyptr[d]) + idx;
                st_scatter(dst, k);
                st_scatter(val_dst(dst, d, idx), v);
            } else {
                const KeyT k = sm.sorted[idx];
                const uint32_t d = digit_of(k, shift, dmask);
                st_scatter(reinterpret_cast<KeyT*>(sm.keyptr[d]) + idx, k);
            }
        }
    } else {
#pragma unroll 4
        for (int j = 0; j < K; ++j) {
            const uint32_t idx = j * THREADS + tid;
            if (idx < valid) {
                if constexpr (PAIRS) {
                    KeyT k;
                    uint32_t v;
                    get_slot(idx, k, v);
                    const uint32_t d = digit_of(k, shift, dmask);
                    KeyT* dst = reinterpret_cast<KeyT*>(sm.keyptr[d]) + idx;
                    st_scatter(dst, dec ? codec_decode<KeyT>(k, ca, cb, cd) : k);
                    st_scatter(val_dst(dst, d, idx), v);
                } else {
                    const KeyT k = sm.sorted[idx];
                    const uint32_t d = digit_of(k, shift, dmask);
                    st_scatter(reinterpret_cast<KeyT*>(sm.keyptr[d]) + idx, dec ? codec_decode<KeyT>(k, ca, cb, cd) : k);
                }
            }
        }
    }
    OSB_PHASE(6);
#if OSB_PHASE_PROBE
    if (tid == 0) atomicAdd(&g_phase[7], 1ull);
#endif
    if (!kPersistent || next >= num_tiles) break;
    tile = next;
    }
}

#ifndef OSB_PAIRS16K
#define OSB_PAIRS16K 0
#endif
template <int WARPS, int K>
struct PairsSmem {
    static constexpr int THREADS = WARPS * 32;
    static constexpr int T = THREADS * K;
    alignas(16) uint32_t sorted[T];
    alignas(16) uint32_t hist[WARPS * kRadix];
    unsigned long long keyptr[kRadix];
    unsigned long long valptr[kRadix];
    alignas(16) unsigned char dig[T];
    uint32_t wtot[kRadix / 32];
    uint32_t tile;
    uint32_t plan_bits;
};

template <int K, int WARPS, int RANK_MODE, int LOOK>
__global__ void __launch_bounds__(WARPS * 32, 2)
digit_binning_pairs_kernel(uint32_t* buf0, uint32_t* buf1, uint32_t* val0, uint32_t* val1, uint64_t n,
                           const unsigned long long* __restrict__ gbase, uint16_t* agg16, uint64_t* incl64,
                           uint32_t* ticket, PassParams pp, KeyCodec codec)
{
    using KeyT = uint32_t;
    using S = PairsSmem<WARPS, K>;
    constexpr int THREADS = S::THREADS;
    constexpr int T = S::T;
    static_assert(T <= 16384 && (K % 2) == 0, "slots are kept as 14-bit halves of a register");
    extern __shared__ __align__(128) unsigned char s_raw[];
    S& sm = *reinterpret_cast<S*>(s_raw);

    const int tid = threadIdx.x, lane = tid & 31, warp = tid >> 5;
    const uint32_t lt = lanemask_lt();
    uint32_t* wh = sm.hist + warp * kRadix;
    const uint32_t shift = pp.shift, epoch = pp.epoch;
    const uint32_t dmask = (1u << pp.dbits) - 1u;

    {
        uint4* h4 = reinterpret_cast<uint4*>(sm.hist);
        for (int i = tid; i < WARPS * kRadix / 4; i += THREADS) h4[i] = make_uint4(0, 0, 0, 0);
    }
    uint32_t my_bits = (codec.flags & (kCodecEncodeOnLoad | kCodecDecodeOnStore)) << 1;
    if (pp.plan != nullptr) {
        const uint4 raw = __ldg(reinterpret_cast<const uint4*>(pp.plan));
        SortPlan pl; pl.skip_mask = raw.x; pl.executed = raw.y; pl.first_exec = raw.z; pl.last_exec = raw.w;
        if ((pl.skip_mask >> pp.place) & 1u) return;
        my_bits = plan_src_is_alt(pl, pp.place) ? 1u : 0u;
        if (codec.flags & kCodecFromPlan)
            my_bits |= (pp.place == pl.first_exec ? kCodecEncodeOnLoad << 1 : 0u) | (pp.place == pl.last_exec ? kCodecDecodeOnStore << 1 : 0u);
    }
    if (tid == 0) { sm.plan_bits = my_bits; sm.tile = blockIdx.x; }
    const uint32_t tile = blockIdx.x;
    const uint64_t tile_base = static_cast<uint64_t>(tile) * T;
    const bool full = tile_base + T <= n;
    const uint32_t valid = full ? T : static_cast<uint32_t>(n - tile_base);
    const uint32_t warp_off = warp * (32 * K) + lane;

    uint32_t key[K];
    {
        const KeyT* __restrict__ in = (my_bits & 1u) ? buf1 : buf0;
        if (full) {
#pragma unroll
            for (int i = 0; i < K; ++i) key[i] = ld_stream(in + tile_base + warp_off + i * 32);
        } else {
#pragma unroll
            for (int i = 0; i < K; ++i) {
                const uint32_t idx = warp_off + i * 32;
                key[i] = idx < valid ? in[tile_base + idx] : 0xffffffffu;
            }
        }
    }
    __syncthreads();
    if ((sm.plan_bits >> 1) & kCodecEncodeOnLoad) {
        const KeyT ca = static_cast<KeyT>(codec.a), cb = static_cast<KeyT>(codec.b), cd = static_cast<KeyT>(codec.d);
#pragma unroll
        for (int i = 0; i < K; ++i) {
            key[i] = codec_encode<KeyT>(key[i], ca, cb, cd);
            if (!full && warp_off + i * 32 >= valid) key[i] = 0xffffffffu;
        }
    }
#pragma unroll
    for (int i = 0; i < K; ++i) atomicAdd(&wh[digit_of(key[i], shift, dmask)], 1u);
    __syncthreads();

    uint32_t tile_count = 0, tile_excl = 0;
    if (tid < kRadix) {
#pragma unroll
        for (int w = 0; w < WARPS; ++w) tile_count += sm.hist[w * kRadix + tid];
        if (pp.stall_every == 0 || (tile % pp.stall_every) != pp.stall_every - 1)
            st_relaxed_gpu_u16(agg16 + agg_index(tile, tid), kAggReady | tile_count);
    }
    tile_excl = block_excl_scan_256<THREADS>(tile_count, sm.wtot);
    if (tid < kRadix) {
        uint32_t run = tile_excl;
#pragma unroll
        for (int w = 0; w < WARPS; ++w) { const uint32_t c = sm.hist[w * kRadix + tid]; sm.hist[w * kRadix + tid] = run; run += c; }
    }
    __syncthreads();

    uint32_t slots[K / 2];
#pragma unroll
    for (int i = 0; i < K; ++i) {
        const uint32_t slot = warp_rank_and_count<RANK_MODE>(wh, digit_of(key[i], shift, dmask), lt);
        sm.sorted[slot] = key[i];
        if (i & 1) slots[i / 2] |= slot << 16; else slots[i / 2] = slot;
    }
    if (tid < kRadix) {
        TileRereduce<KeyT> rr;
        rr.in = (sm.plan_bits & 1u) ? buf1 : buf0; rr.tile_keys = T; rr.shift = shift; rr.mask = dmask;
        rr.encode = (sm.plan_bits >> 1) & kCodecEncodeOnLoad;
        rr.ca = static_cast<KeyT>(codec.a); rr.cb = static_cast<KeyT>(codec.b); rr.cd = static_cast<KeyT>(codec.d);
        const unsigned long long prior = lookback_wide<LOOK / 8, KeyT>(agg16, incl64, tile, tid, epoch, pp.spin_cap, rr);
        st_relaxed_gpu_u64(incl64 + static_cast<uint64_t>(tile) * kRadix + tid, desc_pack(epoch, kFlagInclusive, prior + tile_count));
        const bool swap = sm.plan_bits & 1u;
        const unsigned long long first = gbase[tid] + prior - tile_excl;
        sm.keyptr[tid] = reinterpret_cast<unsigned long long>(swap ? buf0 : buf1) + first * sizeof(KeyT);
        sm.valptr[tid] = reinterpret_cast<unsigned long long>(swap ? val0 : val1) + first * sizeof(uint32_t);
    }
    __syncthreads();

    asm volatile("" ::: "memory");
    {
        const uint32_t* __restrict__ in_val = (sm.plan_bits & 1u) ? val1 : val0;
        if (full) {
#pragma unroll
            for (int i = 0; i < K; ++i) key[i] = ld_stream(in_val + tile_base + warp_off + i * 32);
        } else {
#pragma unroll
            for (int i = 0; i < K; ++i) {
                const uint32_t idx = warp_off + i * 32;
                key[i] = idx < valid ? in_val[tile_base + idx] : 0u;
            }
        }
    }

    {
        const bool dec = (sm.plan_bits >> 1) & kCodecDecodeOnStore;
        const KeyT ca = static_cast<KeyT>(codec.a), cb = static_cast<KeyT>(codec.b), cd = static_cast<KeyT>(codec.d);
        if (full && !dec) {
#pragma unroll
            for (int j = 0; j < K; ++j) {
                const uint32_t idx = j * THREADS + tid;
                const KeyT k = sm.sorted[idx];
                const uint32_t d = digit_of(k, shift, dmask);
                sm.dig[idx] = static_cast<unsigned char>(d);
                st_stream(reinterpret_cast<KeyT*>(sm.keyptr[d]) + idx, k);
            }
        } else {
#pragma unroll 4
            for (int j = 0; j < K; ++j) {
                const uint32_t idx = j * THREADS + tid;
                const KeyT k = sm.sorted[idx];
                const uint32_t d = digit_of(k, shift, dmask);
                sm.dig[idx] = static_cast<unsigned char>(d);
                if (idx < valid) st_stream(reinterpret_cast<KeyT*>(sm.keyptr[d]) + idx, dec ? codec_decode<KeyT>(k, ca, cb, cd) : k);
            }
        }
    }
    __syncthreads();

#pragma unroll
    for (int i = 0; i < K; ++i) sm.sorted[(slots[i / 2] >> (16 * (i & 1))) & 0xffffu] = key[i];
    __syncthreads();
    if (full) {
#pragma unroll
        for (int j = 0; j < K; ++j) {
            const uint32_t idx = j * THREADS + tid;
            st_stream(reinterpret_cast<uint32_t*>(sm.valptr[sm.dig[idx]]) + idx, sm.sorted[idx]);
        }
    } else {
#pragma unroll 4
        for (int j = 0; j < K; ++j) {
            const uint32_t idx = j * THREADS + tid;
            if (idx < valid) st_stream(reinterpret_cast<uint32_t*>(sm.valptr[sm.dig[idx]]) + idx, sm.sorted[idx]);
        }
    }
}

template <typename KeyT, int K, int WARPS>
struct RingSmem {
    static constexpr int THREADS = WARPS * 32;
    static constexpr int T = THREADS * K;
    alignas(128) KeyT stage[2][T];
    alignas(16) uint32_t hist[WARPS * kRadix];
    unsigned long long keyptr[kRadix];
    alignas(8) uint64_t bar[2];
    uint32_t tile[2];
    uint32_t wtot[kRadix / 32];
};

#ifndef OSB_LOOK
#define OSB_LOOK 16
#endif
#ifndef OSB_PAIRS_LOOK
#define OSB_PAIRS_LOOK 8
#endif
#ifndef OSB_U64_LOOK
#define OSB_U64_LOOK 32
#endif
#ifndef OSB_RING_K
#define OSB_RING_K 16
#define OSB_RING_MINB 2
#endif
template <typename KeyT, int K, int WARPS, int RANK_MODE, int LOOK>
__global__ void __launch_bounds__(WARPS * 32, (sizeof(KeyT) == 4 ? OSB_RING_MINB : 2))
digit_binning_ring_kernel(const KeyT* __restrict__ in, KeyT* __restrict__ out, uint64_t n, uint32_t shift,
                          const unsigned long long* __restrict__ gbase, uint16_t* agg16, uint64_t* incl64,
                          uint32_t* ticket, uint32_t epoch, uint32_t num_tiles)
{
    using S = RingSmem<KeyT, K, WARPS>;
    constexpr int THREADS = S::THREADS;
    constexpr int T = S::T;
    constexpr uint32_t TILE_BYTES = T * sizeof(KeyT);
    extern __shared__ __align__(128) unsigned char s_raw[];
    S& sm = *reinterpret_cast<S*>(s_raw);

    const int tid = threadIdx.x, lane = tid & 31, warp = tid >> 5;
    const uint32_t lt = lanemask_lt();
    uint32_t* wh = sm.hist + warp * kRadix;
    const uint32_t warp_off = warp * (32 * K) + lane;

    auto fetch = [&](int slot) {
        const uint32_t t = atomicAdd(ticket, 1u);
        sm.tile[slot] = t;
        if (t < num_tiles && static_cast<uint64_t>(t + 1) * T <= n) {
            mbar_expect_tx(&sm.bar[slot], TILE_BYTES);
            tma_load_1d(sm.stage[slot], in + static_cast<uint64_t>(t) * T, TILE_BYTES, &sm.bar[slot]);
        }
    };
    auto zero_hist = [&]() {
        uint4* h4 = reinterpret_cast<uint4*>(sm.hist);
        for (int i = tid; i < WARPS * kRadix / 4; i += THREADS) h4[i] = make_uint4(0, 0, 0, 0);
    };

    zero_hist();
    if (tid == 0) {
        mbar_init(&sm.bar[0], 1);
        mbar_init(&sm.bar[1], 1);
        fence_mbar_init();
        fetch(0);
        fetch(1);
    }
    __syncthreads();

    for (uint32_t it = 0;; ++it) {
        const int slot = it & 1;
        const uint32_t tile = sm.tile[slot];
        if (tile >= num_tiles) break;
        const uint64_t tile_base = static_cast<uint64_t>(tile) * T;
        const bool full = tile_base + T <= n;
        const uint32_t valid = full ? T : static_cast<uint32_t>(n - tile_base);
        KeyT* s_keys = sm.stage[slot];

        KeyT key[K];
        if (full) {
            mbar_wait(&sm.bar[slot], (it >> 1) & 1u);
#pragma unroll
            for (int i = 0; i < K; ++i) key[i] = s_keys[warp_off + i * 32];
        } else {
#pragma unroll
            for (int i = 0; i < K; ++i) {
                const uint32_t idx = warp_off + i * 32;
                key[i] = idx < valid ? in[tile_base + idx] : static_cast<KeyT>(~static_cast<KeyT>(0));
            }
        }

#pragma unroll
        for (int i = 0; i < K; ++i) atomicAdd(&wh[digit_of(key[i], shift)], 1u);
        __syncthreads();

        uint32_t tile_count = 0, tile_excl = 0;
        if (tid < kRadix) {
#pragma unroll
            for (int w = 0; w < WARPS; ++w) tile_count += sm.hist[w * kRadix + tid];
            st_relaxed_gpu_u16(agg16 + agg_index(tile, tid), kAggReady | tile_count);
        }
        tile_excl = block_excl_scan_256<THREADS>(tile_count, sm.wtot);
        if (tid < kRadix) {
            uint32_t run = tile_excl;
#pragma unroll
            for (int w = 0; w < WARPS; ++w) { const uint32_t c = sm.hist[w * kRadix + tid]; sm.hist[w * kRadix + tid] = run; run += c; }
        }
        __syncthreads();

#pragma unroll
        for (int i = 0; i < K; ++i) s_keys[warp_rank_and_count<RANK_MODE>(wh, digit_of(key[i], shift), lt)] = key[i];

        if (tid < kRadix) {
            TileRereduce<KeyT> rr;
            rr.in = in; rr.tile_keys = T; rr.shift = shift; rr.mask = kRadix - 1; rr.encode = false;
            rr.ca = rr.cb = rr.cd = 0;
            const unsigned long long prior = lookback_wide<LOOK / 8, KeyT>(agg16, incl64, tile, tid, epoch, 1u << 20, rr);
            st_relaxed_gpu_u64(incl64 + static_cast<uint64_t>(tile) * kRadix + tid,
                               desc_pack(epoch, kFlagInclusive, prior + tile_count));
            sm.keyptr[tid] = reinterpret_cast<unsigned long long>(out) + (gbase[tid] + prior - tile_excl) * sizeof(KeyT);
        }
        __syncthreads();

        if (full) {
#pragma unroll
            for (int j = 0; j < K; ++j) {
                const uint32_t idx = j * THREADS + tid;
                const KeyT k = s_keys[idx];
                st_stream(reinterpret_cast<KeyT*>(sm.keyptr[digit_of(k, shift)]) + idx, k);
            }
        } else {
#pragma unroll 4
            for (int j = 0; j < K; ++j) {
                const uint32_t idx = j * THREADS + tid;
                if (idx < valid) {
                    const KeyT k = s_keys[idx];
                    st_stream(reinterpret_cast<KeyT*>(sm.keyptr[digit_of(k, shift)]) + idx, k);
                }
            }
        }
        zero_hist();
        __syncthreads();
        if (tid == 0) {
            fence_proxy_async_smem();
            fetch(slot);
        }
    }
}

template <typename KeyT> struct RingGeom;
template <> struct RingGeom<uint32_t> { static constexpr int K = OSB_RING_K, WARPS = 16, LOOK = OSB_LOOK; };
template <> struct RingGeom<uint64_t> { static constexpr int K = 8,  WARPS = 16, LOOK = OSB_LOOK; };

struct PassArgs {
    const void* in; void* out; const uint32_t* in_val; uint32_t* out_val; uint64_t n; uint32_t shift;
    const unsigned long long* gbase; uint64_t* desc; uint16_t* agg16; uint32_t* ticket; uint32_t epoch;
    const BinningConfig& cfg; cudaStream_t stream;

    PassParams params() const
    {
        PassParams pp;
        pp.shift = shift;
        pp.dbits = cfg.digit_bits;
        pp.epoch = epoch;
        pp.place = cfg.place;
        pp.spin_cap = cfg.spin_cap;
        pp.stall_every = cfg.debug_stall_every;
        pp.plan = cfg.plan;
        pp.keys_in = cfg.argsort_in;
        return pp;
    }
};

template <typename KeyT, bool PAIRS, bool INDICES = false>
struct PassShape {
    using Key = KeyT;
    static constexpr bool pairs = PAIRS, indices = INDICES;
    static constexpr bool enabled = true;
    static constexpr bool has_hot = false;
};

template <typename KeyT>
struct RingShape : PassShape<KeyT, false> {
    using G = RingGeom<KeyT>;
    using S = RingSmem<KeyT, G::K, G::WARPS>;
    static constexpr uint32_t T = S::T;
    static constexpr size_t smem = sizeof(S);
    template <int RANK_MODE, bool HOT = false>
    static auto kernel() { return digit_binning_ring_kernel<KeyT, G::K, G::WARPS, RANK_MODE, G::LOOK>; }
    template <int RANK_MODE>
    static cudaError_t launch(const PassArgs& a)
    {
        const uint64_t tiles = (a.n + T - 1) / T;
        const uint64_t cap = static_cast<uint64_t>(a.cfg.sm_count) * (sizeof(KeyT) == 4 ? OSB_RING_MINB : 2);
        const auto kern = kernel<RANK_MODE>();
        kern<<<static_cast<unsigned>(tiles < cap ? tiles : cap), S::THREADS, smem, a.stream>>>(
            static_cast<const KeyT*>(a.in), static_cast<KeyT*>(a.out), a.n, a.shift, a.gbase, a.agg16, a.desc, a.ticket, a.epoch,
            static_cast<uint32_t>(tiles));
        return cudaGetLastError();
    }
};

template <typename KeyT, bool PAIRS> struct WideGeom;
#ifndef OSB_WIDE_WARPS
#define OSB_WIDE_WARPS 16
#define OSB_WIDE_K 32
#define OSB_WIDE_MINB 2
#endif
#ifndef OSB_PAIRS_WIDE_WARPS
#define OSB_PAIRS_WIDE_WARPS 16
#define OSB_PAIRS_WIDE_K 16
#define OSB_PAIRS_WIDE_MINB 2
#endif
#ifndef OSB_U64_WARPS
#define OSB_U64_WARPS 16
#define OSB_U64_MINB 2
#endif
#ifndef OSB_U64_K
#define OSB_U64_K 16
#endif
template <> struct WideGeom<uint32_t, false> { static constexpr int K = OSB_WIDE_K, WARPS = OSB_WIDE_WARPS, MINB = OSB_WIDE_MINB, LOOK = OSB_LOOK; };
template <> struct WideGeom<uint32_t, true>  { static constexpr int K = OSB_PAIRS_WIDE_K, WARPS = OSB_PAIRS_WIDE_WARPS, MINB = OSB_PAIRS_WIDE_MINB, LOOK = OSB_PAIRS_LOOK; };
template <> struct WideGeom<uint64_t, false> { static constexpr int K = OSB_U64_K, WARPS = OSB_U64_WARPS, MINB = OSB_U64_MINB, LOOK = OSB_U64_LOOK; };
#ifndef OSB_K16_K
#define OSB_K16_K 24
#define OSB_K16_WARPS 16
#endif
#ifndef OSB_P16_K
#define OSB_P16_K 16
#define OSB_P16_WARPS 16
#endif
template <> struct WideGeom<uint16_t, false> { static constexpr int K = OSB_K16_K, WARPS = OSB_K16_WARPS, MINB = 2, LOOK = OSB_LOOK; };
template <> struct WideGeom<uint16_t, true>  { static constexpr int K = OSB_P16_K, WARPS = OSB_P16_WARPS, MINB = 2, LOOK = OSB_PAIRS_LOOK; };
#ifndef OSB_P64_K
#define OSB_P64_K 16
#define OSB_P64_WARPS 16
#define OSB_P64_MINB 1
#endif
#ifndef OSB_P64_LOOK
#define OSB_P64_LOOK 32
#endif
template <> struct WideGeom<uint64_t, true>  { static constexpr int K = OSB_P64_K, WARPS = OSB_P64_WARPS, MINB = OSB_P64_MINB, LOOK = OSB_P64_LOOK; };
template <typename KeyT, bool PAIRS, bool INDICES = false>
struct WideShape : PassShape<KeyT, PAIRS, INDICES> {
    using G = WideGeom<KeyT, PAIRS>;
    using S = WideSmem<KeyT, PAIRS, G::K, G::WARPS>;
    static constexpr uint32_t T = S::T;
    static constexpr size_t smem = sizeof(S);
    static constexpr bool has_hot = true;
    template <int RANK_MODE, bool HOT = false>
    static auto kernel() { return digit_binning_wide_kernel<KeyT, PAIRS, G::K, G::WARPS, RANK_MODE, G::LOOK, G::MINB, HOT, INDICES>; }
    template <int RANK_MODE>
    static cudaError_t launch(const PassArgs& a)
    {
        const uint64_t tiles = (a.n + T - 1) / T;
        const PassParams pp = a.params();
        auto grid_for = [&](auto kernel, int& per_sm, bool persistent) -> unsigned {
            if (!persistent) return static_cast<unsigned>(tiles);
            if (per_sm == 0) {
                int b = 0;
                if (cudaOccupancyMaxActiveBlocksPerMultiprocessor(&b, kernel, S::THREADS, smem) != cudaSuccess || b < 1) b = 1;
                per_sm = b;
            }
            uint64_t cap = static_cast<uint64_t>(a.cfg.sm_count) * per_sm;
            if (a.cfg.debug_max_ctas && a.cfg.debug_max_ctas < cap) cap = a.cfg.debug_max_ctas;
            return static_cast<unsigned>(tiles < cap ? tiles : cap);
        };
        KeyT* buf0 = static_cast<KeyT*>(const_cast<void*>(a.in));
        uint32_t* val0 = const_cast<uint32_t*>(a.in_val);
        const auto kern = kernel<RANK_MODE>();
        static int plain_per_sm = 0;
        kern<<<grid_for(kern, plain_per_sm, sizeof(KeyT) <= 4 && !PAIRS), S::THREADS, smem, a.stream>>>(
            buf0, static_cast<KeyT*>(a.out), val0, a.out_val, a.n, a.gbase, a.agg16, a.desc, a.ticket, pp, a.cfg.codec);
        if (a.cfg.plan != nullptr && a.cfg.hot_passes) {
            const auto hot = kernel<RANK_MODE, true>();
            static int hot_per_sm = 0;
            hot<<<grid_for(hot, hot_per_sm, true), S::THREADS, smem, a.stream>>>(
                buf0, static_cast<KeyT*>(a.out), val0, a.out_val, a.n, a.gbase, a.agg16, a.desc, a.ticket, pp, a.cfg.codec);
        }
        return cudaGetLastError();
    }
};

constexpr int kPairsK = 32, kPairsWarps = 16;

struct Pairs16KShape : PassShape<uint32_t, true> {
    static constexpr bool enabled = OSB_PAIRS16K != 0;
    using S = PairsSmem<kPairsWarps, kPairsK>;
    static constexpr uint32_t T = S::T;
    static constexpr size_t smem = sizeof(S);
    template <int RANK_MODE, bool HOT = false>
    static auto kernel() { return digit_binning_pairs_kernel<kPairsK, kPairsWarps, RANK_MODE, OSB_PAIRS_LOOK>; }
    template <int RANK_MODE>
    static cudaError_t launch(const PassArgs& a)
    {
        const auto kern = kernel<RANK_MODE>();
        kern<<<static_cast<unsigned>((a.n + T - 1) / T), S::THREADS, smem, a.stream>>>(
            static_cast<uint32_t*>(const_cast<void*>(a.in)), static_cast<uint32_t*>(a.out), const_cast<uint32_t*>(a.in_val), a.out_val,
            a.n, a.gbase, a.agg16, a.desc, a.ticket, a.params(), a.cfg.codec);
        return cudaGetLastError();
    }
};

template <typename KeyT, bool PAIRS> struct TileGeom;
template <> struct TileGeom<uint32_t, false> { static constexpr int K = 16, WARPS = 16; };
template <> struct TileGeom<uint32_t, true>  { static constexpr int K = 16, WARPS = 16; };
template <> struct TileGeom<uint64_t, false> { static constexpr int K = 8,  WARPS = 16; };

template <typename KeyT, bool PAIRS>
struct TileShape : PassShape<KeyT, PAIRS> {
    using G = TileGeom<KeyT, PAIRS>;
    static constexpr uint32_t T = G::WARPS * 32 * G::K;
    static constexpr size_t hist_bytes = static_cast<size_t>(G::WARPS) * kRadix * 4, keys_bytes = T * sizeof(KeyT);
    static constexpr size_t smem = hist_bytes > keys_bytes ? hist_bytes : keys_bytes;
    template <int RANK_MODE, bool HOT = false>
    static auto kernel() { return digit_binning_tile_kernel<KeyT, PAIRS, G::K, G::WARPS, RANK_MODE>; }
    template <int RANK_MODE>
    static cudaError_t launch(const PassArgs& a)
    {
        const auto kern = kernel<RANK_MODE>();
        kern<<<static_cast<unsigned>((a.n + T - 1) / T), G::WARPS * 32, smem, a.stream>>>(
            static_cast<const KeyT*>(a.in), static_cast<KeyT*>(a.out), a.in_val, a.out_val, a.n, a.shift, a.gbase, a.desc, a.ticket,
            a.epoch);
        return cudaGetLastError();
    }
};

using DefaultPassShapes = TypeList<Pairs16KShape,
                                   WideShape<uint16_t, false>, WideShape<uint16_t, true>, WideShape<uint16_t, true, true>,
                                   WideShape<uint32_t, false>, WideShape<uint32_t, true>, WideShape<uint32_t, true, true>,
                                   WideShape<uint64_t, false>, WideShape<uint64_t, true>, WideShape<uint64_t, true, true>>;
using RingShapes = TypeList<RingShape<uint32_t>, RingShape<uint64_t>>;
using TileShapes = TypeList<TileShape<uint32_t, false>, TileShape<uint32_t, true>, TileShape<uint64_t, false>>;

template <typename F>
static cudaError_t with_pass_shape(int key_bytes, bool pairs, bool indices, int variant, F&& f)
{
    auto match = [&](auto s) {
        using S = decltype(s);
        return S::enabled && key_bytes == static_cast<int>(sizeof(typename S::Key)) && S::pairs == pairs && S::indices == indices;
    };
    if (variant == kVariantWide) return find_type(DefaultPassShapes{}, match, f);
    if (variant == kVariantPersistent && !pairs) return find_type(RingShapes{}, match, f);
    return find_type(TileShapes{}, match, f);
}

constexpr uint32_t cmin(uint32_t a, uint32_t b) { return a < b ? a : b; }
constexpr uint32_t kSmallestTileU32Keys = cmin(cmin(TileShape<uint32_t, false>::T, RingShape<uint32_t>::T), WideShape<uint32_t, false>::T);
constexpr uint32_t kSmallestTileU32Pairs = cmin(TileShape<uint32_t, true>::T, WideShape<uint32_t, true>::T);
static_assert(WideShape<uint16_t, false>::T >= kSmallestTileU32Keys && WideShape<uint16_t, false>::T >= kSmallestTileU32Pairs,
              "16-bit keys (either 4-byte handle): a smaller tile would need more descriptors than the handle has");
static_assert(WideShape<uint16_t, true>::T >= kSmallestTileU32Pairs,
              "16-bit pairs (a (4, 4) handle): a smaller tile would need more descriptors than the handle has");
static_assert(WideShape<uint16_t, false>::T < 32768 && WideShape<uint16_t, true>::T < 32768, "agg16 holds 15-bit counts");
static_assert(WideShape<uint64_t, true>::T >= TileShape<uint64_t, false>::T,
              "64-bit pairs: a smaller tile would need more descriptors than the handle has");
static_assert(WideShape<uint64_t, true>::T < 32768, "agg16 holds 15-bit counts");

uint32_t binning_tile_keys(int key_bytes, bool pairs, const BinningConfig& cfg)
{
    uint32_t t = 0;
    auto tile = [&](auto s) { t = decltype(s)::T; return cudaSuccess; };
    if (with_pass_shape(key_bytes, pairs, false, cfg.variant, tile) != cudaSuccess) with_pass_shape(key_bytes, false, false, cfg.variant, tile);
    return t;
}

bool binning_has_hot_twin(int key_bytes, bool pairs, bool indices, const BinningConfig& cfg)
{
    bool hot = false;
    with_pass_shape(key_bytes, pairs, indices, cfg.variant, [&](auto s) { hot = decltype(s)::has_hot; return cudaSuccess; });
    return hot;
}

cudaError_t launch_digit_binning(const void* in, void* out, const uint32_t* in_val, uint32_t* out_val, uint64_t n,
                                 int key_bytes, uint32_t shift, const unsigned long long* gbase_place, uint64_t* desc,
                                 uint16_t* agg16, uint32_t* ticket, uint32_t epoch, const BinningConfig& cfg,
                                 cudaStream_t stream)
{
    const bool pairs = in_val != nullptr;
    if (cfg.variant != kVariantWide && (cfg.codec.flags || cfg.plan != nullptr || cfg.debug_stall_every || cfg.argsort_in))
        return cudaErrorNotSupported;
    if (cfg.digit_bits < 1 || cfg.digit_bits > 8) return cudaErrorInvalidValue;
    if (cfg.variant != kVariantWide && cfg.digit_bits != 8 && shift + cfg.digit_bits != static_cast<uint32_t>(key_bytes) * 8u)
        return cudaErrorNotSupported;
    const bool indices = cfg.argsort_in != nullptr;
    if (indices && (!pairs || cfg.plan == nullptr)) return cudaErrorInvalidValue;
    const PassArgs a{in, out, in_val, out_val, n, shift, gbase_place, desc, agg16, ticket, epoch, cfg, stream};
    return with_rank_mode(cfg.rank_mode, [&](auto r) {
        return with_pass_shape(key_bytes, pairs, indices, cfg.variant,
                               [&](auto s) { return decltype(s)::template launch<decltype(r)::value>(a); });
    });
}

template <typename KeyT, bool PAIRS, int K, int WARPS>
struct SegSmem {
    static constexpr int THREADS = WARPS * 32;
    static constexpr int T = THREADS * K;
    alignas(16) KeyT sorted[T];
    alignas(16) uint32_t sorted_val[PAIRS ? T : 4];
    alignas(16) uint32_t hist[WARPS * kRadix];
    uint32_t wtot[kRadix / 32];
};

template <typename KeyT, bool PAIRS, int K, int WARPS, int RANK_MODE, bool INDICES = false, bool ROWS = false>
__global__ void __launch_bounds__(WARPS * 32, ROWS ? 1 : 0)
segment_sort_kernel(KeyT* keys, uint32_t* vals, const unsigned long long* __restrict__ seg_off, uint64_t num_segments,
                    uint64_t single_n, uint32_t max_len, uint32_t begin_bit, uint32_t places, uint32_t last_bits, KeyCodec codec,
                    const KeyT* __restrict__ keys_in)
{
    static_assert(!INDICES || PAIRS, "the indices are the payloads");
    using S = SegSmem<KeyT, PAIRS, K, WARPS>;
    constexpr int THREADS = S::THREADS;
    constexpr int T = S::T;
    static_assert(WARPS >= 8, "one thread per digit");
    extern __shared__ __align__(128) unsigned char s_raw[];
    S& sm = *reinterpret_cast<S*>(s_raw);
    const int tid = threadIdx.x, lane = tid & 31, warp = tid >> 5;
    const uint32_t lt = lanemask_lt();
    uint32_t* wh = sm.hist + warp * kRadix;
    const uint32_t warp_off = warp * (32 * K) + lane;
    const KeyT ca = static_cast<KeyT>(codec.a), cb = static_cast<KeyT>(codec.b), cd = static_cast<KeyT>(codec.d);
    const bool enc = codec.flags & kCodecEncodeOnLoad, dec = codec.flags & kCodecDecodeOnStore;

    for (uint64_t seg = blockIdx.x; seg < num_segments; seg += gridDim.x) {
        const uint64_t lo = ROWS ? seg * single_n : seg_off ? seg_off[seg] : 0ull;
        const uint64_t hi = ROWS ? lo + single_n : seg_off ? seg_off[seg + 1] : single_n;
        if (hi <= lo + 1 || hi - lo > static_cast<uint64_t>(max_len) || hi - lo > static_cast<uint64_t>(T)) continue;
        const uint32_t len = static_cast<uint32_t>(hi - lo);

        KeyT key[K];
        uint32_t val[PAIRS ? K : 1];
#pragma unroll
        for (int i = 0; i < K; ++i) {
            const uint32_t idx = warp_off + i * 32;
            KeyT k = idx < len ? (INDICES || ROWS ? keys_in : keys)[lo + idx] : static_cast<KeyT>(0);
            if (enc) k = codec_encode<KeyT>(k, ca, cb, cd);
            key[i] = idx < len ? k : static_cast<KeyT>(~static_cast<KeyT>(0));
            if constexpr (PAIRS) val[i] = INDICES ? idx : idx < len ? vals[lo + idx] : 0u;
        }

        const uint32_t warp_lo = warp * (32 * K);
        const uint32_t live_chunks = ROWS ? (len > warp_lo ? (len - warp_lo + 31) / 32 : 0u) : static_cast<uint32_t>(K);
        auto live = [&](int i) { return !ROWS || static_cast<uint32_t>(i) < live_chunks; };
        for (uint32_t p = 0; p < places; ++p) {
            const uint32_t shift = begin_bit + 8u * p;
            const uint32_t dmask = p == places - 1 ? (1u << last_bits) - 1u : 255u;
            __syncthreads();
            {
                uint4* h4 = reinterpret_cast<uint4*>(sm.hist);
                for (int i = tid; i < WARPS * kRadix / 4; i += THREADS) h4[i] = make_uint4(0, 0, 0, 0);
            }
            __syncthreads();
#pragma unroll
            for (int i = 0; i < K; ++i)
                if (live(i)) atomicAdd(&wh[digit_of(key[i], shift, dmask)], 1u);
            __syncthreads();
            uint32_t tile_count = 0;
            if (tid < kRadix) {
#pragma unroll
                for (int w = 0; w < WARPS; ++w) tile_count += sm.hist[w * kRadix + tid];
            }
            const uint32_t tile_excl = block_excl_scan_256<THREADS>(tile_count, sm.wtot);
            if (tid < kRadix) {
                uint32_t run = tile_excl;
#pragma unroll
                for (int w = 0; w < WARPS; ++w) { const uint32_t c = sm.hist[w * kRadix + tid]; sm.hist[w * kRadix + tid] = run; run += c; }
            }
            __syncthreads();
#pragma unroll
            for (int i = 0; i < K; ++i) {
                if (!live(i)) continue;
                const uint32_t slot = warp_rank_and_count<RANK_MODE>(wh, digit_of(key[i], shift, dmask), lt);
                sm.sorted[slot] = key[i];
                if constexpr (PAIRS) sm.sorted_val[slot] = val[i];
            }
            __syncthreads();
            if (p + 1 < places) {
#pragma unroll
                for (int i = 0; i < K; ++i) {
                    key[i] = sm.sorted[warp_off + i * 32];
                    if constexpr (PAIRS) val[i] = sm.sorted_val[warp_off + i * 32];
                }
            }
        }
        for (uint32_t idx = tid; idx < len; idx += THREADS) {
            KeyT k = sm.sorted[idx];
            if (dec) k = codec_decode<KeyT>(k, ca, cb, cd);
            keys[lo + idx] = k;
            if constexpr (PAIRS) vals[lo + idx] = sm.sorted_val[idx];
        }
    }
}

template <typename KeyT, int SIZE> struct SegGeomN;
template <> struct SegGeomN<uint32_t, 0> { static constexpr int K = 1,  WARPS = 8; };
template <> struct SegGeomN<uint32_t, 1> { static constexpr int K = 8,  WARPS = 8; };
template <> struct SegGeomN<uint32_t, 2> { static constexpr int K = 32, WARPS = 16; };
template <> struct SegGeomN<uint64_t, 0> { static constexpr int K = 1,  WARPS = 8; };
template <> struct SegGeomN<uint64_t, 1> { static constexpr int K = 8,  WARPS = 8; };
template <> struct SegGeomN<uint64_t, 2> { static constexpr int K = 16, WARPS = 16; };
template <> struct SegGeomN<uint16_t, 1> { static constexpr int K = 8,  WARPS = 8; };
template <> struct SegGeomN<uint16_t, 2> { static constexpr int K = 32, WARPS = 16; };
template <typename KeyT, bool PAIRS, int SIZE, bool INDICES = false, bool ROWS = false>
struct SegShape {
    using Key = KeyT;
    static constexpr bool pairs = PAIRS, indices = INDICES, rows = ROWS, has_hot = false;
    using G = SegGeomN<KeyT, SIZE>;
    using S = SegSmem<KeyT, PAIRS, G::K, G::WARPS>;
    static constexpr uint32_t T = S::T;
    static constexpr size_t smem = sizeof(S);
    static constexpr int ctas_per_sm = SIZE == 2 ? 2 : 8;
    template <int RANK_MODE, bool HOT = false>
    static auto kernel() { return segment_sort_kernel<KeyT, PAIRS, G::K, G::WARPS, RANK_MODE, INDICES, ROWS>; }
};
template <typename KeyT, int SIZE, bool INDICES> using RowShape = SegShape<KeyT, INDICES, SIZE, INDICES, true>;

using SegShapes = TypeList<
    SegShape<uint32_t, false, 0>, SegShape<uint32_t, false, 1>, SegShape<uint32_t, false, 2>,
    SegShape<uint32_t, true, 0>, SegShape<uint32_t, true, 1>, SegShape<uint32_t, true, 2>,
    SegShape<uint64_t, false, 0>, SegShape<uint64_t, false, 1>, SegShape<uint64_t, false, 2>,
    SegShape<uint16_t, false, 2>, SegShape<uint16_t, true, 2>, SegShape<uint64_t, true, 2>,
    SegShape<uint16_t, true, 2, true>, SegShape<uint32_t, true, 2, true>, SegShape<uint64_t, true, 2, true>,
    RowShape<uint16_t, 1, false>, RowShape<uint16_t, 2, false>, RowShape<uint16_t, 1, true>, RowShape<uint16_t, 2, true>,
    RowShape<uint32_t, 1, false>, RowShape<uint32_t, 2, false>, RowShape<uint32_t, 1, true>, RowShape<uint32_t, 2, true>,
    RowShape<uint64_t, 1, false>, RowShape<uint64_t, 2, false>, RowShape<uint64_t, 1, true>, RowShape<uint64_t, 2, true>>;

template <bool ROWS>
static uint32_t seg_capacity(int key_bytes)
{
    uint32_t cap = 0;
    for_each_type(SegShapes{}, [&](auto s) {
        using S = decltype(s);
        if (S::rows == ROWS && key_bytes == static_cast<int>(sizeof(typename S::Key)) && S::T > cap) cap = S::T;
        return cudaSuccess;
    });
    return cap;
}

uint32_t segment_sort_capacity(int key_bytes) { return seg_capacity<false>(key_bytes); }

template <typename Shape>
static cudaError_t launch_seg(Shape, void* keys, uint32_t* vals, const unsigned long long* seg_off, uint64_t num_segments,
                              uint64_t single_n, uint32_t max_len, uint32_t begin_bit, uint32_t places, uint32_t last_bits,
                              const KeyCodec& codec, int rank_mode, int sm_count, cudaStream_t stream, const void* keys_in)
{
    using KeyT = typename Shape::Key;
    const uint64_t cap = static_cast<uint64_t>(sm_count) * Shape::ctas_per_sm;
    const unsigned grid = static_cast<unsigned>(num_segments < cap ? num_segments : cap);
    return with_rank_mode(rank_mode, [&](auto r) {
        const auto kern = Shape::template kernel<decltype(r)::value>();
        kern<<<grid, Shape::S::THREADS, Shape::smem, stream>>>(static_cast<KeyT*>(keys), vals, seg_off, num_segments, single_n, max_len,
                                                              begin_bit, places, last_bits, codec, static_cast<const KeyT*>(keys_in));
        return cudaGetLastError();
    });
}

cudaError_t launch_segment_sort(void* keys, uint32_t* vals, int key_bytes, const unsigned long long* seg_off, uint64_t num_segments,
                                uint64_t single_n, uint32_t max_len, uint32_t begin_bit, uint32_t places, uint32_t last_bits,
                                const KeyCodec* codec_in, int rank_mode, int sm_count, cudaStream_t stream, const void* keys_in)
{
    if (num_segments == 0) return cudaSuccess;
    const bool pairs = vals != nullptr, indices = keys_in != nullptr;
    if ((indices || key_bytes == 2 || (key_bytes == 8 && pairs)) && (seg_off || num_segments != 1)) return cudaErrorInvalidValue;
    const KeyCodec codec = codec_in ? *codec_in : KeyCodec();
    return find_type(
        SegShapes{},
        [&](auto s) {
            using S = decltype(s);
            return !S::rows && key_bytes == static_cast<int>(sizeof(typename S::Key)) && S::pairs == pairs && S::indices == indices &&
                   max_len <= S::T;
        },
        [&](auto s) {
            return launch_seg(s, keys, vals, seg_off, num_segments, single_n, max_len, begin_bit, places, last_bits, codec, rank_mode,
                              sm_count, stream, keys_in);
        });
}

constexpr int kRowWarps = 8;

template <typename KeyT, int K, bool INDICES>
struct RowWarpSmem {
    alignas(16) uint32_t hist[kRadix];
    alignas(16) KeyT keys[32 * K];
    uint32_t idx[INDICES ? 32 * K : 1];
};

template <typename KeyT, int K, int RANK_MODE, bool INDICES>
__global__ void __launch_bounds__(kRowWarps * 32)
row_sort_warp_kernel(const KeyT* in, KeyT* out, uint32_t* __restrict__ idx_out, uint64_t num_rows, uint32_t row_len,
                     KeyCodec codec)
{
    using W = RowWarpSmem<KeyT, K, INDICES>;
    extern __shared__ __align__(16) unsigned char s_raw[];
    const int lane = threadIdx.x & 31, warp = threadIdx.x >> 5;
    W& sm = reinterpret_cast<W*>(s_raw)[warp];
    uint4* h4 = reinterpret_cast<uint4*>(sm.hist);
    const uint32_t lt = lanemask_lt();
    const KeyT ca = static_cast<KeyT>(codec.a), cb = static_cast<KeyT>(codec.b), cd = static_cast<KeyT>(codec.d);
    const bool enc = codec.flags & kCodecEncodeOnLoad, dec = codec.flags & kCodecDecodeOnStore;

    for (uint64_t row = static_cast<uint64_t>(blockIdx.x) * kRowWarps + warp; row < num_rows;
         row += static_cast<uint64_t>(gridDim.x) * kRowWarps) {
        const uint64_t base = row * row_len;
        KeyT key[K];
        uint32_t val[INDICES ? K : 1];
#pragma unroll
        for (int i = 0; i < K; ++i) {
            const uint32_t idx = i * 32 + lane;
            KeyT k = idx < row_len ? in[base + idx] : static_cast<KeyT>(0);
            if (enc) k = codec_encode<KeyT>(k, ca, cb, cd);
            key[i] = idx < row_len ? k : static_cast<KeyT>(~static_cast<KeyT>(0));
            if constexpr (INDICES) val[i] = idx;
        }
#pragma unroll 1
        for (uint32_t shift = 0; shift < sizeof(KeyT) * 8; shift += 8) {
            h4[2 * lane] = make_uint4(0, 0, 0, 0);
            h4[2 * lane + 1] = make_uint4(0, 0, 0, 0);
            __syncwarp();
#pragma unroll
            for (int i = 0; i < K; ++i)
                if (i * 32 + lane < row_len) atomicAdd(&sm.hist[digit_of(key[i], shift)], 1u);
            __syncwarp();
            const uint4 lo4 = h4[2 * lane], hi4 = h4[2 * lane + 1];
            const uint32_t c[8] = {lo4.x, lo4.y, lo4.z, lo4.w, hi4.x, hi4.y, hi4.z, hi4.w};
            uint32_t sum = 0;
            bool whole = false;
#pragma unroll
            for (int j = 0; j < 8; ++j) { sum += c[j]; whole |= c[j] == row_len; }
            if (__any_sync(0xffffffffu, whole)) continue;
            uint32_t incl = sum;
#pragma unroll
            for (int o = 1; o < 32; o <<= 1) {
                const uint32_t t = __shfl_up_sync(0xffffffffu, incl, o);
                if (lane >= o) incl += t;
            }
            uint32_t run = incl - sum, e[8];
#pragma unroll
            for (int j = 0; j < 8; ++j) { e[j] = run; run += c[j]; }
            h4[2 * lane] = make_uint4(e[0], e[1], e[2], e[3]);
            h4[2 * lane + 1] = make_uint4(e[4], e[5], e[6], e[7]);
            __syncwarp();
#pragma unroll
            for (int i = 0; i < K; ++i) {
                const uint32_t slot = warp_rank_and_count<RANK_MODE>(sm.hist, digit_of(key[i], shift), lt);
                sm.keys[slot] = key[i];
                if constexpr (INDICES) sm.idx[slot] = val[i];
            }
            __syncwarp();
#pragma unroll
            for (int i = 0; i < K; ++i) {
                key[i] = sm.keys[i * 32 + lane];
                if constexpr (INDICES) val[i] = sm.idx[i * 32 + lane];
            }
            __syncwarp();
        }
#pragma unroll
        for (int i = 0; i < K; ++i) {
            const uint32_t idx = i * 32 + lane;
            if (idx < row_len) {
                KeyT k = key[i];
                if (dec) k = codec_decode<KeyT>(k, ca, cb, cd);
                out[base + idx] = k;
                if constexpr (INDICES) idx_out[base + idx] = val[i];
            }
        }
    }
}

template <typename KeyT, int K, int RANK_MODE, bool INDICES>
static cudaError_t launch_row_warp(const void* in, void* out, uint32_t* idx, uint64_t num_rows, uint32_t row_len,
                                   const KeyCodec& codec, int sm_count, cudaStream_t stream)
{
    auto kern = row_sort_warp_kernel<KeyT, K, RANK_MODE, INDICES>;
    constexpr size_t smem = kRowWarps * sizeof(RowWarpSmem<KeyT, K, INDICES>);
    static const int per_sm = [&] {
        int b = 0;
        return cudaOccupancyMaxActiveBlocksPerMultiprocessor(&b, kern, kRowWarps * 32, smem) == cudaSuccess ? b : 0;
    }();
    if (per_sm <= 0) return cudaErrorLaunchOutOfResources;
    const uint64_t need = (num_rows + kRowWarps - 1) / kRowWarps, cap = static_cast<uint64_t>(sm_count) * per_sm;
    kern<<<static_cast<unsigned>(need < cap ? need : cap), kRowWarps * 32, smem, stream>>>(
        static_cast<const KeyT*>(in), static_cast<KeyT*>(out), idx, num_rows, row_len, codec);
    return cudaGetLastError();
}

template <typename KeyT, int RANK_MODE, bool INDICES>
static cudaError_t launch_row_warp_k(const void* in, void* out, uint32_t* idx, uint64_t num_rows, uint32_t row_len,
                                     const KeyCodec& codec, int sm_count, cudaStream_t stream)
{
    if (row_len <= 32) return launch_row_warp<KeyT, 1, RANK_MODE, INDICES>(in, out, idx, num_rows, row_len, codec, sm_count, stream);
    if (row_len <= 64) return launch_row_warp<KeyT, 2, RANK_MODE, INDICES>(in, out, idx, num_rows, row_len, codec, sm_count, stream);
    if (row_len <= 128) return launch_row_warp<KeyT, 4, RANK_MODE, INDICES>(in, out, idx, num_rows, row_len, codec, sm_count, stream);
    return launch_row_warp<KeyT, 8, RANK_MODE, INDICES>(in, out, idx, num_rows, row_len, codec, sm_count, stream);
}

uint32_t row_sort_capacity(int key_bytes) { return seg_capacity<true>(key_bytes); }

cudaError_t launch_row_sort(const void* keys_in, void* keys_out, uint32_t* indices, uint64_t num_rows, uint32_t row_len,
                            int key_bytes, const KeyCodec* codec_in, int rank_mode, bool block_only, int sm_count,
                            cudaStream_t stream)
{
    if (num_rows == 0 || row_len == 0) return cudaSuccess;
    if (row_len > row_sort_capacity(key_bytes)) return cudaErrorInvalidValue;
    const KeyCodec codec = codec_in ? *codec_in : KeyCodec();
    if (row_len <= kRowWarpMaxLen && !block_only) {
        return with_key_type(TypeList<uint16_t, uint32_t, uint64_t>{}, key_bytes, [&](auto k) {
            return with_rank_mode(rank_mode, [&](auto r) {
                using KeyT = decltype(k);
                constexpr int R = decltype(r)::value;
                return indices ? launch_row_warp_k<KeyT, R, true>(keys_in, keys_out, indices, num_rows, row_len, codec, sm_count, stream)
                               : launch_row_warp_k<KeyT, R, false>(keys_in, keys_out, indices, num_rows, row_len, codec, sm_count, stream);
            });
        });
    }
    return find_type(
        SegShapes{},
        [&](auto s) {
            using S = decltype(s);
            return S::rows && key_bytes == static_cast<int>(sizeof(typename S::Key)) && S::indices == (indices != nullptr) && row_len <= S::T;
        },
        [&](auto s) {
            return launch_seg(s, keys_out, indices, nullptr, num_rows, row_len, row_len, 0u, static_cast<uint32_t>(key_bytes), 8u, codec,
                              rank_mode, sm_count, stream, keys_in);
        });
}

cudaError_t configure_kernels()
{
    cudaError_t e = for_each_type(HistKeys{}, [](auto k) {
        using KeyT = decltype(k);
        return set_smem(global_histogram_kernel<KeyT>, hist_smem_bytes<KeyT>());
    });
    if (e == cudaSuccess) e = for_each_type(HistBitsKeys{}, [](auto k) {
        using KeyT = decltype(k);
        const cudaError_t m = set_smem(global_histogram_kernel<KeyT, true>, hist_smem_bytes<KeyT>());
        return m != cudaSuccess ? m : set_smem(global_histogram_bits_kernel<KeyT>, hist_smem_bytes<KeyT>());
    });
    auto shape = [](auto s) { return configure_shape(s); };
    if (e == cudaSuccess) e = for_each_type(DefaultPassShapes{}, shape);
    if (e == cudaSuccess) e = for_each_type(RingShapes{}, shape);
    if (e == cudaSuccess) e = for_each_type(TileShapes{}, shape);
    if (e == cudaSuccess) e = for_each_type(SegShapes{}, shape);
    return e;
}


template <typename KeyT>
__global__ void __launch_bounds__(256)
validate_kernel(const KeyT* __restrict__ keys, uint64_t n, unsigned long long* err_count)
{
    unsigned long long bad = 0;
    const uint64_t stride = static_cast<uint64_t>(gridDim.x) * blockDim.x;
    for (uint64_t i = static_cast<uint64_t>(blockIdx.x) * blockDim.x + threadIdx.x; i + 1 < n; i += stride)
        bad += keys[i] > keys[i + 1];
    for (int o = 16; o > 0; o >>= 1) bad += __shfl_down_sync(0xffffffffu, bad, o);
    if ((threadIdx.x & 31) == 0 && bad) atomicAdd(err_count, bad);
}

cudaError_t launch_validate(const void* keys, uint64_t n, int key_bytes, unsigned long long* err_count, int sm_count,
                            cudaStream_t stream)
{
    return with_key_type(TypeList<uint32_t, uint64_t>{}, key_bytes, [&](auto k) {
        using KeyT = decltype(k);
        validate_kernel<KeyT><<<static_cast<unsigned>(sm_count) * 8, 256, 0, stream>>>(static_cast<const KeyT*>(keys), n, err_count);
        return cudaGetLastError();
    });
}

constexpr uint32_t kGenStreams = 65536;

struct HybridTaus {
    uint32_t a, b, c, l;
    __device__ __forceinline__ uint32_t next()
    {
        a = ((a & 0xfffffffeu) << 12) ^ (((a << 13) ^ a) >> 19);
        b = ((b & 0xfffffff8u) << 4) ^ (((b << 2) ^ b) >> 25);
        c = ((c & 0xfffffff0u) << 17) ^ (((c << 3) ^ c) >> 11);
        l = l * 1664525u + 1013904223u;
        return a ^ b ^ c ^ l;
    }
};

__global__ void __launch_bounds__(256)
init_random_kernel(uint32_t* __restrict__ keys, uint32_t* __restrict__ payload, uint64_t n, uint32_t and_count,
                   uint32_t seed, bool payload_is_index)
{
    const uint32_t g = blockIdx.x * blockDim.x + threadIdx.x;
    HybridTaus s{(g * 4u) * seed, (g * 4u + 1u) * seed, (g * 4u + 2u) * seed, (g * 4u + 3u) * seed};
    (void)s.next();
    for (uint64_t i = g; i < n; i += kGenStreams) {
        uint32_t t = 0xffffffffu;
        for (uint32_t k = 0; k <= and_count; ++k) t &= s.next();
        keys[i] = t;
        if (payload) payload[i] = payload_is_index ? static_cast<uint32_t>(i) : t;
    }
}

cudaError_t launch_init_random(uint32_t* keys, uint32_t* payload, uint64_t n, uint32_t and_count, uint32_t seed,
                               bool payload_is_index, cudaStream_t stream)
{
    init_random_kernel<<<kGenStreams / 256, 256, 0, stream>>>(keys, payload, n, and_count, seed, payload_is_index);
    return cudaGetLastError();
}

constexpr int kSelfTestWarps = 16;
__global__ void __launch_bounds__(kSelfTestWarps * 32, 2)
atomic_order_selftest_kernel(unsigned long long* mismatches)
{
    __shared__ uint32_t s_hist[kSelfTestWarps * kRadix];
    __shared__ uint32_t s_ref[kSelfTestWarps * kRadix];
    __shared__ volatile uint32_t s_scratch[kSelfTestWarps * 32 * 4];
    const int lane = threadIdx.x & 31, warp = threadIdx.x >> 5;
    uint32_t* wh = s_hist + warp * kRadix;
    uint32_t* wr = s_ref + warp * kRadix;
    uint32_t s = (blockIdx.x * blockDim.x + threadIdx.x) * 2654435761u + 12345u;
    const uint32_t lt = lanemask_lt();
    unsigned long long bad = 0;
    constexpr int B = 16;
    for (int it = 0; it < 24; ++it) {
        for (int i = lane; i < kRadix; i += 32) { wh[i] = 0; wr[i] = 0; }
        __syncwarp();
        for (int batch = 0; batch < 2; ++batch) {
            uint32_t d[B], got[B];
#pragma unroll
            for (int i = 0; i < B; ++i) {
                uint32_t x = 255u;
                const int draws = 1 + (it % 6);
                for (int k = 0; k < draws; ++k) { s = s * 1664525u + 1013904223u; x &= (s >> 13); }
                if (it % 6 == 5) x = (it + i) & 255u;
                d[i] = x;
            }
#pragma unroll
            for (int i = 0; i < B; ++i) {
                got[i] = warp_rank_and_count<kRankAtomic>(wh, d[i], lt);
                s_scratch[(got[i] * 37u + d[i] * 5u + threadIdx.x) & (kSelfTestWarps * 32 * 4 - 1)] = d[i];
            }
#pragma unroll
            for (int i = 0; i < B; ++i) {
                const uint32_t want = warp_rank_and_count<kRankBallot>(wr, d[i], lt);
                bad += (got[i] != want);
                __syncwarp();
            }
        }
    }
    if (bad) atomicAdd(mismatches, bad);
}

cudaError_t launch_atomic_order_selftest(unsigned long long* mismatches, int sm_count, cudaStream_t stream)
{
    atomic_order_selftest_kernel<<<sm_count * 2, kSelfTestWarps * 32, 0, stream>>>(mismatches);
    return cudaGetLastError();
}

}
```

gpusorting_b200/csrc/osb_kernels.cuh:

```cuda
#pragma once
#include <cstdint>
#include <cuda_runtime.h>

#include "osb_common.cuh"

namespace osb {

enum BinningVariant : int {
    kVariantTilePerCta = 0,
    kVariantPersistent = 1,
    kVariantWide = 2,
};
constexpr int kNumVariants = 3;
enum RankMode : int {
    kRankAtomic = 0,
    kRankBallot = 1,
};

struct BinningConfig {
    int variant = kVariantTilePerCta;
    int rank_mode = kRankAtomic;
    int sm_count = 132;
    KeyCodec codec;
    uint32_t digit_bits = 8;
    const SortPlan* plan = nullptr;
    uint32_t place = 0;
    uint32_t spin_cap = 2048;
    uint32_t debug_stall_every = 0;
    uint32_t debug_max_ctas = 0;
    bool hot_passes = false;
    const void* argsort_in = nullptr;
};

uint32_t binning_tile_keys(int key_bytes, bool pairs, const BinningConfig& cfg);
bool binning_has_hot_twin(int key_bytes, bool pairs, bool indices, const BinningConfig& cfg);

cudaError_t configure_kernels();

cudaError_t launch_global_histogram(const void* keys, uint64_t n, int key_bytes, unsigned long long* ghist,
                                    int sm_count, cudaStream_t stream, const KeyCodec* codec = nullptr);

cudaError_t launch_digit_histogram(const void* keys, uint64_t n, int key_bytes, uint32_t shift,
                                   unsigned long long* hist256, int sm_count, cudaStream_t stream);

cudaError_t launch_scan(const unsigned long long* ghist, unsigned long long* gbase, int places, cudaStream_t stream,
                        SortPlan* plan = nullptr, uint64_t n = 0, bool allow_skip = false, bool allow_hot = false);

cudaError_t launch_global_histogram_bits(const void* keys, uint64_t n, int key_bytes, unsigned long long* ghist, int sm_count,
                                         cudaStream_t stream, const KeyCodec* codec, uint32_t begin_bit, int places,
                                         uint32_t last_bits);

cudaError_t launch_copy_back(const SortPlan* plan, const void* alt_keys, void* keys, const uint32_t* alt_vals, uint32_t* vals,
                             uint64_t n, int key_bytes, int sm_count, cudaStream_t stream);
cudaError_t launch_argsort_copy_back(const SortPlan* plan, const void* keys_in, const void* alt_keys, void* keys,
                                     const uint32_t* alt_idx, uint32_t* idx, uint64_t n, int key_bytes, int sm_count,
                                     cudaStream_t stream);

cudaError_t launch_digit_binning(const void* in, void* out, const uint32_t* in_val, uint32_t* out_val, uint64_t n,
                                 int key_bytes, uint32_t shift, const unsigned long long* gbase_place, uint64_t* desc,
                                 uint16_t* agg16, uint32_t* ticket, uint32_t epoch, const BinningConfig& cfg,
                                 cudaStream_t stream);

uint32_t segment_sort_capacity(int key_bytes);
cudaError_t launch_segment_sort(void* keys, uint32_t* vals, int key_bytes, const unsigned long long* seg_off, uint64_t num_segments,
                                uint64_t single_n, uint32_t max_len, uint32_t begin_bit, uint32_t places, uint32_t last_bits,
                                const KeyCodec* codec, int rank_mode, int sm_count, cudaStream_t stream,
                                const void* keys_in = nullptr);

constexpr uint32_t kRowWarpMaxLen = 256;
uint32_t row_sort_capacity(int key_bytes);
cudaError_t launch_row_sort(const void* keys_in, void* keys_out, uint32_t* indices, uint64_t num_rows, uint32_t row_len,
                            int key_bytes, const KeyCodec* codec, int rank_mode, bool block_only, int sm_count,
                            cudaStream_t stream);

cudaError_t launch_validate(const void* keys, uint64_t n, int key_bytes, unsigned long long* err_count, int sm_count,
                            cudaStream_t stream);

cudaError_t launch_init_random(uint32_t* keys, uint32_t* payload, uint64_t n, uint32_t and_count, uint32_t seed,
                               bool payload_is_index, cudaStream_t stream);

cudaError_t launch_atomic_order_selftest(unsigned long long* mismatches, int sm_count, cudaStream_t stream);

}
```

Baseline: 64.73.

## Fuse global histogram into first binning pass using gapped per-digit regions

The first digit-binning pass now scatters keys into fixed-size per-digit regions of an enlarged alternate buffer, so it no longer needs a prior global histogram. While doing so it accumulates the histograms of the upper digits for later passes. The second pass reads the gapped layout. If any digit overflows its region, an abort flag triggers a fallback that zeroes the descriptors and reruns the classic histogram and scan. This removes one full read of the input, at the cost of more allocated memory, extra shared-memory atomics in the first pass, and a rarely used fallback path.

```diff
diff --git a/gpusorting_b200/csrc/osb_common.cuh b/gpusorting_b200/csrc/osb_common.cuh
--- a/gpusorting_b200/csrc/osb_common.cuh
+++ b/gpusorting_b200/csrc/osb_common.cuh
@@ -83,4 +83,16 @@
     return __popc(~pl.skip_mask & ((1u << place) - 1u)) & 1u;
 }
 
+constexpr uint32_t kPlanFusedKept = 1u << 24;
+__host__ __device__ constexpr uint64_t fused_region_keys(uint64_t n)
+{
+    const uint64_t q = (n + 255) / 256;
+    return (q + q / 32 + 1024 + 31) / 32 * 32;
 }
+__device__ __forceinline__ bool plan_reads_gapped(const SortPlan& pl, uint32_t place)
+{
+    const uint32_t later = ~pl.skip_mask & 0xfeu;
+    return (pl.skip_mask & kPlanFusedKept) && later && place == static_cast<uint32_t>(__ffs(later) - 1);
+}
+
+}
diff --git a/gpusorting_b200/csrc/osb_host.cu b/gpusorting_b200/csrc/osb_host.cu
--- a/gpusorting_b200/csrc/osb_host.cu
+++ b/gpusorting_b200/csrc/osb_host.cu
@@ -44,8 +44,10 @@
     bool small_path = true;
     bool hot_passes = true;
     bool debug_rows_block = false;
+    bool fused_histogram = true;
 
     void* alt_keys = nullptr;
+    uint64_t alt_key_slots = 0;
     uint32_t* alt_vals = nullptr;
     unsigned char* control = nullptr;
     uint64_t* desc = nullptr;
@@ -54,8 +56,12 @@
     uint32_t epoch = 0;
 
     bool profile = false;
-    cudaEvent_t ev[kMaxPlaces + 3] = {};
+    static constexpr int kMaxEvents = kMaxPlaces + 6;
+    cudaEvent_t ev[kMaxEvents] = {};
     int ev_count = 0;
+    struct Span { int entry, from, to; };
+    Span spans[kMaxEvents] = {};
+    int span_count = 0;
 
     void* stage_keys = nullptr;
     uint32_t* stage_vals = nullptr;
@@ -77,6 +83,22 @@
 namespace {
 
 uint64_t tiles_for(uint64_t n, uint32_t tile_keys) { return (n + tile_keys - 1) / tile_keys; }
+
+constexpr uint64_t kFusedMinTiles = 64;
+constexpr int kFusedTicket = 4, kFusedAbort = 5;
+
+bool fused_size(uint64_t n)
+{
+    osb::BinningConfig wide;
+    wide.variant = osb::kVariantWide;
+    return n < (1ull << 32) && tiles_for(n, osb::binning_tile_keys(4, false, wide)) >= kFusedMinTiles;
+}
+
+uint64_t alt_key_slots_for(uint64_t max_n, int key_bytes)
+{
+    const uint64_t regions = key_bytes == 4 && fused_size(max_n) ? osb::kRadix * osb::fused_region_keys(max_n) : 0;
+    return regions > max_n ? regions : max_n;
+}
 uint64_t agg_tiles_for(uint64_t n, uint32_t tile_keys) { return (tiles_for(n, tile_keys) + 7) / 8 * 8; }
 
 uint32_t smallest_tile(int key_bytes, bool pairs)
@@ -151,40 +173,77 @@
     const uint64_t agg_stride = agg_tiles_for(n, tile_keys) * osb::kRadix;
     if (compact) OSB_TRY(cudaMemsetAsync(s->agg16, 0, agg_stride * places * sizeof(uint16_t), stream));
     int ne = 0;
+    s->span_count = 0;
     auto mark = [&]() -> cudaError_t {
         if (!s->profile) return cudaSuccess;
         if (!s->ev[ne]) { cudaError_t e = cudaEventCreate(&s->ev[ne]); if (e != cudaSuccess) return e; }
         return cudaEventRecord(s->ev[ne++], stream);
     };
+    auto span = [&](int entry) -> cudaError_t {
+        if (s->profile) s->spans[s->span_count++] = {entry, ne - 1, ne};
+        return mark();
+    };
     s->ev_count = 0;
     OSB_TRY(mark());
     osb::KeyCodec enc;
     if (codec) { enc = *codec; enc.flags = osb::kCodecEncodeOnLoad; }
-    if (whole_key)
-        OSB_TRY(osb::launch_global_histogram(keys_in ? keys_in : d_keys, n, key_bytes, s->ghist(), s->sm_count, stream,
-                                             codec ? &enc : nullptr));
-    else
-        OSB_TRY(osb::launch_global_histogram_bits(d_keys, n, key_bytes, s->ghist(), s->sm_count, stream, codec ? &enc : nullptr,
-                                                  static_cast<uint32_t>(begin_bit), places, last_bits));
-    OSB_TRY(mark());
     const bool hot_passes = use_plan && s->hot_passes && osb::binning_has_hot_twin(key_bytes, d_vals != nullptr, keys_in != nullptr, s->cfg);
-    OSB_TRY(osb::launch_scan(s->ghist(), s->gbase(), places, stream, use_plan ? s->plan() : nullptr, n, s->short_circuit, hot_passes));
-    OSB_TRY(mark());
+    const uint64_t region = osb::fused_region_keys(n);
+    const bool fused = s->fused_histogram && use_plan && whole_key && key_bytes == 4 && !d_vals && !keys_in && fused_size(n) &&
+                       osb::kRadix * region <= s->alt_key_slots;
+    uint32_t fused_epoch = 0;
+    if (fused) {
+        st = next_epoch(s, stream, &fused_epoch);
+        if (st != OSB200_OK) return st;
+        const uint32_t epoch = fused_epoch;
+        osb::BinningConfig cfg = s->cfg;
+        if (codec) cfg.codec = enc;
+        unsigned long long* fallback_hist = s->ghist() + 4 * osb::kRadix;
+        uint32_t* abort_word = s->tickets() + kFusedAbort;
+        uint32_t ctas = 0;
+        OSB_TRY(osb::launch_fused_first_pass(static_cast<const uint32_t*>(d_keys), static_cast<uint32_t*>(s->alt_keys), n, region,
+                                             s->ghist(), abort_word, s->desc, s->agg16, s->tickets() + kFusedTicket, epoch, cfg, stream,
+                                             &ctas));
+        OSB_TRY(span(2));
+        OSB_TRY(osb::launch_scan_fused(s->ghist(), s->gbase(), places, stream, s->plan(), n, s->short_circuit, hot_passes, false,
+                                       abort_word, region));
+        OSB_TRY(span(1));
+        OSB_TRY(osb::launch_fused_fallback_zero(s->plan(), s->tickets() + kFusedTicket, ctas, tiles_for(n, tile_keys), s->agg16, s->desc,
+                                                s->sm_count, stream));
+        OSB_TRY(osb::launch_global_histogram(d_keys, n, key_bytes, fallback_hist, s->sm_count, stream, codec ? &enc : nullptr, s->plan()));
+        OSB_TRY(span(0));
+        OSB_TRY(osb::launch_scan_fused(fallback_hist, s->gbase(), places, stream, s->plan(), n, s->short_circuit, hot_passes, true,
+                                       nullptr, 0));
+        OSB_TRY(span(1));
+    } else {
+        if (whole_key)
+            OSB_TRY(osb::launch_global_histogram(keys_in ? keys_in : d_keys, n, key_bytes, s->ghist(), s->sm_count, stream,
+                                                 codec ? &enc : nullptr));
+        else
+            OSB_TRY(osb::launch_global_histogram_bits(d_keys, n, key_bytes, s->ghist(), s->sm_count, stream, codec ? &enc : nullptr,
+                                                      static_cast<uint32_t>(begin_bit), places, last_bits));
+        OSB_TRY(span(0));
+        OSB_TRY(osb::launch_scan(s->ghist(), s->gbase(), places, stream, use_plan ? s->plan() : nullptr, n, s->short_circuit, hot_passes));
+        OSB_TRY(span(1));
+    }
 
     void* src = d_keys;
     void* dst = s->alt_keys;
     uint32_t* sv = d_vals;
     uint32_t* dv = d_vals ? s->alt_vals : nullptr;
     for (int p = 0; p < places; ++p) {
-        uint32_t epoch = 0;
-        st = next_epoch(s, stream, &epoch);
-        if (st != OSB200_OK) return st;
+        uint32_t epoch = fused_epoch;
+        if (!fused || p > 0) {
+            st = next_epoch(s, stream, &epoch);
+            if (st != OSB200_OK) return st;
+        }
         osb::BinningConfig cfg = s->cfg;
         cfg.digit_bits = p == places - 1 ? last_bits : 8u;
         cfg.place = static_cast<uint32_t>(p);
         if (use_plan) cfg.plan = s->plan();
         cfg.hot_passes = hot_passes;
         cfg.argsort_in = keys_in;
+        if (fused) { cfg.fused_region = region; cfg.fused_dense_base0 = s->gbase(); }
         if (codec) {
             cfg.codec = *codec;
             cfg.codec.flags = use_plan ? osb::kCodecFromPlan
@@ -194,7 +253,7 @@
                                           use_plan ? (d_vals ? s->alt_vals : nullptr) : dv, n, key_bytes,
                                           static_cast<uint32_t>(begin_bit + 8 * p), s->gbase() + p * osb::kRadix, s->desc,
                                           s->agg16 + p * agg_stride, s->tickets() + p, epoch, cfg, stream));
-        OSB_TRY(mark());
+        OSB_TRY(span(2 + p));
         void* t = src; src = dst; dst = t;
         uint32_t* tv = sv; sv = dv; dv = tv;
     }
@@ -302,7 +361,7 @@
 {
     if ((key_bytes != 4 && key_bytes != 8) || (value_bytes != 0 && value_bytes != 4)) return 0;
     const uint64_t tiles = tiles_for(max_n ? max_n : 1, smallest_tile(key_bytes, value_bytes != 0));
-    return max_n * key_bytes + max_n * value_bytes + tiles * osb::kRadix * sizeof(uint64_t) +
+    return alt_key_slots_for(max_n, key_bytes) * key_bytes + max_n * value_bytes + tiles * osb::kRadix * sizeof(uint64_t) +
            (tiles + 8) * osb::kRadix * sizeof(uint16_t) * key_bytes + ControlLayout::total;
 }
 
@@ -334,7 +393,8 @@
     if (e != cudaSuccess) { delete s; return cuda_status(e); }
 
     s->desc_tiles = tiles_for(max_n, smallest_tile(key_bytes, value_bytes != 0));
-    bool ok = cudaMalloc(&s->alt_keys, max_n * key_bytes) == cudaSuccess;
+    s->alt_key_slots = alt_key_slots_for(max_n, key_bytes);
+    bool ok = cudaMalloc(&s->alt_keys, s->alt_key_slots * key_bytes) == cudaSuccess;
     if (ok && value_bytes) ok = cudaMalloc(&s->alt_vals, max_n * sizeof(uint32_t)) == cudaSuccess;
     ok = ok && cudaMalloc(&s->control, ControlLayout::total) == cudaSuccess;
     ok = ok && cudaMalloc(&s->desc, s->desc_tiles * osb::kRadix * sizeof(uint64_t)) == cudaSuccess;
@@ -707,6 +767,7 @@
     if (!std::strcmp(key, "short_circuit")) { h->short_circuit = value != 0; return OSB200_OK; }
     if (!std::strcmp(key, "small_path")) { h->small_path = value != 0; return OSB200_OK; }
     if (!std::strcmp(key, "hot_passes")) { h->hot_passes = value != 0; return OSB200_OK; }
+    if (!std::strcmp(key, "fused_histogram")) { h->fused_histogram = value != 0; return OSB200_OK; }
     if (!std::strcmp(key, "spin_cap")) {
         if (value < 1 || value > (1ll << 30)) return OSB200_ERR_INVALID_ARG;
         h->cfg.spin_cap = static_cast<uint32_t>(value);
@@ -742,7 +803,14 @@
     if (h->ev_count < 2) return 0;
     OSB_TRY(cudaEventSynchronize(h->ev[h->ev_count - 1]));
     int k = 0;
-    for (int i = 0; i + 1 < h->ev_count && k < capacity; ++i, ++k) OSB_TRY(cudaEventElapsedTime(&out_ms[k], h->ev[i], h->ev[i + 1]));
+    for (int i = 0; i < h->span_count; ++i) {
+        const osb200_sorter::Span& sp = h->spans[i];
+        if (sp.entry >= capacity) continue;
+        for (; k <= sp.entry; ++k) out_ms[k] = 0.0f;
+        float ms = 0.0f;
+        OSB_TRY(cudaEventElapsedTime(&ms, h->ev[sp.from], h->ev[sp.to]));
+        out_ms[sp.entry] += ms;
+    }
     return k;
 }
 
@@ -759,6 +827,12 @@
     if (!std::strcmp(key, "short_circuit")) return h->short_circuit ? 1 : 0;
     if (!std::strcmp(key, "small_path")) return h->small_path ? 1 : 0;
     if (!std::strcmp(key, "hot_passes")) return h->hot_passes ? 1 : 0;
+    if (!std::strcmp(key, "fused_histogram")) return h->fused_histogram ? 1 : 0;
+    if (!std::strcmp(key, "last_fused_kept")) {
+        osb::SortPlan pl;
+        if (cudaMemcpy(&pl, h->plan(), sizeof(pl), cudaMemcpyDeviceToHost) != cudaSuccess) return OSB200_ERR_CUDA;
+        return (pl.skip_mask & osb::kPlanFusedKept) ? 1 : 0;
+    }
     if (!std::strcmp(key, "last_hot_mask")) {
         osb::SortPlan pl;
         if (cudaMemcpy(&pl, h->plan(), sizeof(pl), cudaMemcpyDeviceToHost) != cudaSuccess) return -1;
diff --git a/gpusorting_b200/csrc/osb_kernels.cu b/gpusorting_b200/csrc/osb_kernels.cu
--- a/gpusorting_b200/csrc/osb_kernels.cu
+++ b/gpusorting_b200/csrc/osb_kernels.cu
@@ -118,8 +118,9 @@
 template <typename KeyT, bool MASKED = false>
 __global__ void __launch_bounds__(kHistThreads, 1)
 global_histogram_kernel(const KeyT* __restrict__ keys, uint64_t n, unsigned long long* __restrict__ ghist, KeyCodec codec,
-                        int places = 0, uint32_t last_mask = 255u)
-{
+                        int places = 0, uint32_t last_mask = 255u, const SortPlan* gate = nullptr)
+{
+    if (gate != nullptr && (gate->skip_mask & kPlanFusedKept)) return;
     constexpr int PLACES = sizeof(KeyT);
     constexpr int VEC = 16 / sizeof(KeyT);
     constexpr int COLS = HistGeom<KeyT>::COLS;
@@ -179,21 +180,45 @@
 
 template <typename KeyT, bool MASKED>
 static cudaError_t launch_histogram_vec(const void* keys, uint64_t n, unsigned long long* ghist, int sm_count, cudaStream_t stream,
-                                        const KeyCodec& codec, int places = 0, uint32_t last_mask = 255u)
+                                        const KeyCodec& codec, int places = 0, uint32_t last_mask = 255u,
+                                        const SortPlan* gate = nullptr)
 {
     const unsigned grid = capped_grid(n / (16 / sizeof(KeyT)), kHistThreads, sm_count);
     global_histogram_kernel<KeyT, MASKED><<<grid, kHistThreads, hist_smem_bytes<KeyT>(), stream>>>(
-        static_cast<const KeyT*>(keys), n, ghist, codec, places, last_mask);
+        static_cast<const KeyT*>(keys), n, ghist, codec, places, last_mask, gate);
     return cudaGetLastError();
 }
 
 cudaError_t launch_global_histogram(const void* keys, uint64_t n, int key_bytes, unsigned long long* ghist,
-                                    int sm_count, cudaStream_t stream, const KeyCodec* codec_in)
+                                    int sm_count, cudaStream_t stream, const KeyCodec* codec_in, const SortPlan* gate)
 {
     const KeyCodec codec = codec_in ? *codec_in : KeyCodec();
     return with_key_type(HistKeys{}, key_bytes, [&](auto k) {
-        return launch_histogram_vec<decltype(k), false>(keys, n, ghist, sm_count, stream, codec);
+        return launch_histogram_vec<decltype(k), false>(keys, n, ghist, sm_count, stream, codec, 0, 255u, gate);
     });
+}
+
+__global__ void __launch_bounds__(512)
+fused_fallback_zero_kernel(const SortPlan* __restrict__ plan, const uint32_t* __restrict__ ticket, uint32_t ctas, uint64_t tiles,
+                           uint4* __restrict__ agg16, uint4* __restrict__ desc)
+{
+    if (plan->skip_mask & kPlanFusedKept) return;
+    uint64_t reached = static_cast<uint64_t>(ctas) + *ticket;
+    if (reached > tiles) reached = tiles;
+    const uint64_t agg_vecs = (reached + 7) / 8 * 8 * kRadix * sizeof(uint16_t) / 16;
+    const uint64_t desc_vecs = reached * kRadix * sizeof(uint64_t) / 16;
+    const uint64_t stride = static_cast<uint64_t>(gridDim.x) * blockDim.x;
+    for (uint64_t i = static_cast<uint64_t>(blockIdx.x) * blockDim.x + threadIdx.x; i < agg_vecs + desc_vecs; i += stride)
+        (i < agg_vecs ? agg16[i] : desc[i - agg_vecs]) = make_uint4(0, 0, 0, 0);
+}
+
+cudaError_t launch_fused_fallback_zero(const SortPlan* plan, const uint32_t* ticket, uint32_t ctas, uint64_t tiles, uint16_t* agg16,
+                                       uint64_t* desc, int sm_count, cudaStream_t stream)
+{
+    fused_fallback_zero_kernel<<<static_cast<unsigned>(sm_count) * 4, 512, 0, stream>>>(plan, ticket, ctas, tiles,
+                                                                                         reinterpret_cast<uint4*>(agg16),
+                                                                                         reinterpret_cast<uint4*>(desc));
+    return cudaGetLastError();
 }
 
 template <typename KeyT>
@@ -235,13 +260,18 @@
     });
 }
 
+enum ScanMode : int { kScanClassic = 0, kScanFused = 1, kScanFallback = 2 };
+
 __global__ void __launch_bounds__(kRadix)
 scan_kernel(const unsigned long long* __restrict__ ghist, unsigned long long* __restrict__ gbase, int places,
-            SortPlan* plan, unsigned long long n, int allow_skip, int allow_hot)
+            SortPlan* plan, unsigned long long n, int allow_skip, int allow_hot, int mode, const uint32_t* fused_abort,
+            unsigned long long region)
 {
     __shared__ unsigned long long s_warp[kRadix / 32];
+    if (mode == kScanFallback && (plan->skip_mask & kPlanFusedKept)) return;
     const int d = threadIdx.x, lane = d & 31, warp = d >> 5;
     uint32_t skip_mask = 0;
+    const int overfull = mode == kScanFused ? __syncthreads_or(ghist[d] > region || *fused_abort != 0) : 0;
     for (int p = 0; p < places; ++p) {
         const unsigned long long c = ghist[p * kRadix + d];
         unsigned long long incl = c;
@@ -267,6 +297,8 @@
         pl.executed = __popc(run);
         pl.first_exec = run ? static_cast<uint32_t>(__ffs(run) - 1) : 0xffffffffu;
         pl.last_exec = run ? static_cast<uint32_t>(31 - __clz(run)) : 0xffffffffu;
+        if (mode == kScanFused && !overfull && (run & 1u) && !((skip_mask >> kPlanHotShift) & 1u) && (run & ~1u))
+            pl.skip_mask |= kPlanFusedKept;
         *plan = pl;
     }
 }
@@ -274,7 +306,17 @@
 cudaError_t launch_scan(const unsigned long long* ghist, unsigned long long* gbase, int places, cudaStream_t stream,
                         SortPlan* plan, uint64_t n, bool allow_skip, bool allow_hot)
 {
-    scan_kernel<<<1, kRadix, 0, stream>>>(ghist, gbase, places, plan, n, allow_skip ? 1 : 0, allow_hot ? 1 : 0);
+    scan_kernel<<<1, kRadix, 0, stream>>>(ghist, gbase, places, plan, n, allow_skip ? 1 : 0, allow_hot ? 1 : 0, kScanClassic,
+                                          nullptr, 0ull);
+    return cudaGetLastError();
+}
+
+cudaError_t launch_scan_fused(const unsigned long long* ghist, unsigned long long* gbase, int places, cudaStream_t stream,
+                              SortPlan* plan, uint64_t n, bool allow_skip, bool allow_hot, bool fallback, const uint32_t* fused_abort,
+                              uint64_t region)
+{
+    scan_kernel<<<1, kRadix, 0, stream>>>(ghist, gbase, places, plan, n, allow_skip ? 1 : 0, allow_hot ? 1 : 0,
+                                          fallback ? kScanFallback : kScanFused, fused_abort, region);
     return cudaGetLastError();
 }
 
@@ -645,6 +687,27 @@
     KeyT ca, cb, cd;
 };
 
+constexpr long long kHookAbort = -1, kHookDefault = -2;
+struct NoStallHook {
+    __device__ __forceinline__ long long operator()(long long) const { return kHookDefault; }
+};
+
+template <typename KeyT>
+__device__ __noinline__ uint32_t rereduce_tile_gapped(const KeyT* in, uint64_t base, uint32_t tile_keys, uint32_t shift, uint32_t mask,
+                                                      const unsigned long long* gap, unsigned long long region, uint16_t* dst,
+                                                      uint32_t d)
+{
+    uint32_t c = 0, r = 0;
+    for (uint32_t step = kRadix / 2; step; step >>= 1) if (gap[r + step] <= base) r += step;
+    for (uint32_t i = 0; i < tile_keys; ++i) {
+        const uint64_t p = base + i;
+        while (r + 1 < kRadix && gap[r + 1] <= p) ++r;
+        c += digit_of(in[p + r * region - gap[r]], shift, mask) == d;
+    }
+    st_relaxed_gpu_u16(dst, kAggReady | c);
+    return c;
+}
+
 template <typename KeyT>
 __device__ __noinline__ uint32_t rereduce_tile(const KeyT* p, uint32_t tile_keys, uint32_t shift, uint32_t mask, uint32_t encode,
                                                KeyT ca, KeyT cb, KeyT cd, uint16_t* dst, uint32_t d)
@@ -674,10 +737,10 @@
     return (t & 1) ? (w >> 16) : (w & 0xffffu);
 }
 
-template <int NBLK, typename KeyT>
+template <int NBLK, typename KeyT, typename Hook = NoStallHook>
 __device__ __forceinline__ unsigned long long
 lookback_wide(uint16_t* agg16, const uint64_t* incl64, uint32_t tile, uint32_t d, uint32_t epoch, uint32_t spin_cap,
-              const TileRereduce<KeyT>& rr)
+              const TileRereduce<KeyT>& rr, Hook hook = Hook())
 {
     unsigned long long sum = 0;
     int64_t cur = static_cast<int64_t>(tile) - 1;
@@ -718,12 +781,17 @@
         }
         sum = run;
         if (stalled) {
+            if (hook(-1) == kHookAbort) return sum;
             polls = next == cur ? polls + 1 : 1;
             if (polls > spin_cap) {
                 const uint64_t w = ld_relaxed_gpu_u64(incl64 + next * kRadix + d);
                 if (desc_epoch(w) == epoch && (w & kFlagMask) == kFlagInclusive) return sum + desc_value(w);
-                sum += rereduce_tile<KeyT>(rr.in + static_cast<uint64_t>(next) * rr.tile_keys, rr.tile_keys, rr.shift, rr.mask,
-                                           rr.encode ? 1u : 0u, rr.ca, rr.cb, rr.cd, agg16 + agg_index(next, d), d);
+                const long long h = hook(next);
+                if (h >= 0)
+                    sum += static_cast<unsigned long long>(h);
+                else
+                    sum += rereduce_tile<KeyT>(rr.in + static_cast<uint64_t>(next) * rr.tile_keys, rr.tile_keys, rr.shift, rr.mask,
+                                               rr.encode ? 1u : 0u, rr.ca, rr.cb, rr.cd, agg16 + agg_index(next, d), d);
                 --next;
                 polls = 0;
             } else {
@@ -771,9 +839,17 @@
     uint32_t stall_every;
     const SortPlan* plan;
     const void* keys_in = nullptr;
+    unsigned long long region = 0;
+    uint32_t* fused_abort = nullptr;
+    unsigned long long* fused_hist = nullptr;
+    const unsigned long long* dense_base0 = nullptr;
 };
 
 constexpr uint32_t kPlanBitsFirstIndices = 8u;
+constexpr uint32_t kPlanBitsGapped = 16u;
+
+__device__ __forceinline__ void named_bar_arrive(uint32_t id, uint32_t threads) { asm volatile("bar.arrive %0, %1;" ::"r"(id), "r"(threads) : "memory"); }
+__device__ __forceinline__ void named_bar_sync(uint32_t id, uint32_t threads) { asm volatile("bar.sync %0, %1;" ::"r"(id), "r"(threads) : "memory"); }
 
 __device__ __forceinline__ uint32_t opaque_copy(const uint32_t* smem_copy)
 {
@@ -796,15 +872,21 @@
     uint32_t next_tile;
     uint32_t plan_bits;
     uint32_t digit_shift, digit_mask;
+    static constexpr bool kFusable = sizeof(KeyT) == 4 && !PAIRS;
+    unsigned long long gap_base[kFusable ? kRadix : 1];
+    uint32_t fhist[kFusable ? 3 * kRadix : 1];
+    uint32_t fused_stop;
 };
 
-template <typename KeyT, bool PAIRS, int K, int WARPS, int RANK_MODE, int LOOK, int MINB, bool HOT = false, bool INDICES = false>
+template <typename KeyT, bool PAIRS, int K, int WARPS, int RANK_MODE, int LOOK, int MINB, bool HOT = false, bool INDICES = false,
+          bool FUSED = false>
 __global__ void __launch_bounds__(WARPS * 32, HOT ? OSB_HOT_MINB : MINB)
 digit_binning_wide_kernel(KeyT* buf0, KeyT* buf1, uint32_t* val0, uint32_t* val1, uint64_t n,
                           const unsigned long long* __restrict__ gbase, uint16_t* agg16, uint64_t* incl64,
                           uint32_t* ticket, PassParams pp, KeyCodec codec)
 {
     static_assert(!INDICES || PAIRS, "the indices are the 32-bit payloads of a pairs pass");
+    static_assert(!FUSED || (sizeof(KeyT) == 4 && !PAIRS && !HOT && WARPS * 32 > kRadix), "the fused first pass: u32 keys, plain");
     using S = WideSmem<KeyT, PAIRS, K, WARPS>;
     constexpr int THREADS = S::THREADS;
     constexpr int T = S::T;
@@ -846,6 +928,8 @@
         if (codec.flags & kCodecFromPlan)
             my_bits |= (pp.place == pl.first_exec ? kCodecEncodeOnLoad << 1 : 0u) | (pp.place == pl.last_exec ? kCodecDecodeOnStore << 1 : 0u);
         if constexpr (INDICES) my_bits |= pp.place == pl.first_exec ? kPlanBitsFirstIndices : 0u;
+        if constexpr (S::kFusable) my_bits |= plan_reads_gapped(pl, pp.place) ? kPlanBitsGapped : 0u;
+        if (pp.place == 0 && (pl.skip_mask & kPlanFusedKept)) my_skip = true;
     }
     if (my_skip) return;
     if (HOT != my_hot) return;
@@ -855,7 +939,42 @@
     KeyReg key[K];
     uint32_t val[PAIRS ? K : 1];
     const uint32_t warp_off = warp * (32 * K) + lane;
+    auto region_of = [&](uint64_t p) {
+        uint32_t r = 0;
+#pragma unroll 1
+        for (uint32_t step = kRadix / 2; step; step >>= 1) if (sm.gap_base[r + step] <= p) r += step;
+        return r;
+    };
+    auto load_gapped = [&](uint32_t t) {
+        const KeyT* __restrict__ in = buf1;
+        const unsigned long long c = pp.region;
+        const uint64_t base = static_cast<uint64_t>(t) * T;
+        if (base + T <= n) {
+            const uint32_t r0 = region_of(base);
+            if (r0 == region_of(base + T - 1)) {
+                const KeyT* __restrict__ src = in + (base + r0 * c - sm.gap_base[r0]) + warp_off;
+#pragma unroll
+                for (int i = 0; i < K; ++i) key[i] = ld_stream(src + i * 32);
+                return;
+            }
+        }
+        const uint64_t live = base < n ? n - base : 0u;
+#pragma unroll
+        for (int i = 0; i < K; ++i) {
+            const uint32_t idx = warp_off + i * 32;
+            if (idx < live) {
+                const uint64_t p = base + idx;
+                const uint32_t r = region_of(p);
+                key[i] = in[p + r * c - sm.gap_base[r]];
+            } else {
+                key[i] = static_cast<KeyT>(~static_cast<KeyT>(0));
+            }
+        }
+    };
     auto load_tile = [&](uint32_t t) {
+        if constexpr (S::kFusable) {
+            if (my_bits & kPlanBitsGapped) { load_gapped(t); return; }
+        }
         const bool swap = my_bits & 1u;
         const bool iota = INDICES && (my_bits & kPlanBitsFirstIndices);
         const KeyT* __restrict__ in = iota ? static_cast<const KeyT*>(pp.keys_in) : swap ? buf1 : buf0;
@@ -886,11 +1005,22 @@
     };
 
     uint32_t tile = blockIdx.x;
+    if constexpr (S::kFusable) {
+        if (my_bits & kPlanBitsGapped) {
+            for (int i = tid; i < kRadix; i += THREADS) sm.gap_base[i] = pp.dense_base0[i];
+            __syncthreads();
+        }
+    }
     load_tile(tile);
     {
         uint4* h4 = reinterpret_cast<uint4*>(sm.hist);
         for (int i = tid; i < WARPS * kRadix / 4; i += THREADS) h4[i] = make_uint4(0, 0, 0, 0);
     }
+    if constexpr (FUSED) {
+        for (int i = tid; i < 3 * kRadix; i += THREADS) sm.fhist[i] = 0;
+        if (tid == 0) sm.fused_stop = 0;
+    }
+    uint32_t fused_count = 0;
     if (tid == 0) { sm.plan_bits = my_bits; sm.digit_shift = shift; sm.digit_mask = dmask; }
     __syncthreads();
     constexpr bool kPersistent = (sizeof(KeyT) <= 4 && !PAIRS) || HOT;
@@ -947,13 +1077,33 @@
             rr.tile_keys = T; rr.shift = shift; rr.mask = dmask;
             rr.encode = (sm.plan_bits >> 1) & kCodecEncodeOnLoad;
             rr.ca = static_cast<KeyT>(codec.a); rr.cb = static_cast<KeyT>(codec.b); rr.cd = static_cast<KeyT>(codec.d);
-            const unsigned long long prior = lookback_wide<LOOK / 8, KeyT>(agg16, incl64, tile, tid, epoch, pp.spin_cap, rr);
+            auto hook = [&](long long t) -> long long {
+                if (t < 0) {
+                    if constexpr (FUSED) return *reinterpret_cast<const volatile uint32_t*>(pp.fused_abort) ? kHookAbort : kHookDefault;
+                    return kHookDefault;
+                }
+                if (S::kFusable && (sm.plan_bits & kPlanBitsGapped))
+                    return rereduce_tile_gapped<KeyT>(buf1, static_cast<uint64_t>(t) * T, T, shift, dmask, pp.dense_base0, pp.region,
+                                                      agg16 + agg_index(t, tid), tid);
+                return kHookDefault;
+            };
+            const unsigned long long prior = lookback_wide<LOOK / 8, KeyT>(agg16, incl64, tile, tid, epoch, pp.spin_cap, rr, hook);
             const bool swap = sm.plan_bits & 1u;
             KeyT* out = swap ? buf0 : buf1;
             uint32_t* out_val = swap ? val0 : val1;
             st_relaxed_gpu_u64(incl64 + static_cast<uint64_t>(tile) * kRadix + tid,
                                desc_pack(epoch, kFlagInclusive, prior + tile_count));
-            const unsigned long long first = gbase[tid] + prior - tile_excl;
+            if constexpr (FUSED) {
+                const uint32_t live_d = tile_count - ((tid == kRadix - 1 && !full) ? (T - valid) : 0u);
+                fused_count += live_d;
+                if (prior + live_d > pp.region || live_d > T / 16) {
+                    *reinterpret_cast<volatile uint32_t*>(pp.fused_abort) = 1u;
+                    sm.fused_stop = 1u;
+                } else if (*reinterpret_cast<const volatile uint32_t*>(pp.fused_abort)) {
+                    sm.fused_stop = 1u;
+                }
+            }
+            const unsigned long long first = (FUSED ? tid * pp.region : gbase[tid]) + prior - tile_excl;
             sm.keyptr[tid] = reinterpret_cast<unsigned long long>(out) + first * sizeof(KeyT);
             if constexpr (PAIRS) sm.valptr[tid] = reinterpret_cast<unsigned long long>(out_val) + first * sizeof(uint32_t);
             if (tid < 32) {
@@ -1000,10 +1150,32 @@
     const uint32_t next = sm.next_tile;
     if constexpr (kPersistent) { if (!HOT || warp >= kRadix / 32) load_tile(next); }
     OSB_PHASE(4);
+    if constexpr (FUSED) {
+        if (warp < kRadix / 32) {
+            named_bar_arrive(1, THREADS);
+        } else {
+            named_bar_sync(1, THREADS);
+            const uint4* s4 = reinterpret_cast<const uint4*>(sm.sorted);
+#pragma unroll 1
+            for (uint32_t j = tid - kRadix; j < T / 4; j += THREADS - kRadix) {
+                const uint4 v = s4[j];
+                const uint32_t w[4] = {v.x, v.y, v.z, v.w};
+#pragma unroll
+                for (int q = 0; q < 4; ++q) {
+                    if (full || 4 * j + q < valid) {
+                        atomicAdd(&sm.fhist[(w[q] >> 8) & 255u], 1u);
+                        atomicAdd(&sm.fhist[kRadix + ((w[q] >> 16) & 255u)], 1u);
+                        atomicAdd(&sm.fhist[2 * kRadix + (w[q] >> 24)], 1u);
+                    }
+                }
+            }
+        }
+    }
     chained_scan();
     OSB_PHASE(5);
     __syncthreads();
     OSB_PHASE(8);
+    if constexpr (FUSED) { if (sm.fused_stop) break; }
     if constexpr (HOT) { if (warp < kRadix / 32) load_tile(next); }
 
     const bool dec = (sm.plan_bits >> 1) & kCodecDecodeOnStore;
@@ -1095,6 +1267,13 @@
     if (!kPersistent || next >= num_tiles) break;
     tile = next;
     }
+    if constexpr (FUSED) {
+        if (!sm.fused_stop) {
+            if (tid < kRadix && fused_count) atomicAdd(&pp.fused_hist[tid], static_cast<unsigned long long>(fused_count));
+            for (int i = tid; i < 3 * kRadix; i += THREADS)
+                if (sm.fhist[i]) atomicAdd(&pp.fused_hist[kRadix + i], static_cast<unsigned long long>(sm.fhist[i]));
+        }
+    }
 }
 
 #ifndef OSB_PAIRS16K
@@ -1441,6 +1620,8 @@
         pp.stall_every = cfg.debug_stall_every;
         pp.plan = cfg.plan;
         pp.keys_in = cfg.argsort_in;
+        pp.region = cfg.fused_region;
+        pp.dense_base0 = cfg.fused_dense_base0;
         return pp;
     }
 };
@@ -1645,6 +1826,50 @@
     return hot;
 }
 
+using FusedShape = WideShape<uint32_t, false>;
+template <int RANK_MODE>
+static auto fused_kernel()
+{
+    using G = FusedShape::G;
+    return digit_binning_wide_kernel<uint32_t, false, G::K, G::WARPS, RANK_MODE, G::LOOK, G::MINB, false, false, true>;
+}
+
+cudaError_t launch_fused_first_pass(const uint32_t* keys, uint32_t* alt, uint64_t n, uint64_t region, unsigned long long* ghist,
+                                    uint32_t* abort_word, uint64_t* desc, uint16_t* agg16, uint32_t* ticket, uint32_t epoch,
+                                    const BinningConfig& cfg, cudaStream_t stream, uint32_t* ctas)
+{
+    return with_rank_mode(cfg.rank_mode, [&](auto r) {
+        constexpr int RANK_MODE = decltype(r)::value;
+        const auto kern = fused_kernel<RANK_MODE>();
+        static int per_sm = 0;
+        if (per_sm == 0) {
+            int b = 0;
+            if (cudaOccupancyMaxActiveBlocksPerMultiprocessor(&b, kern, FusedShape::S::THREADS, FusedShape::smem) != cudaSuccess || b < 1) b = 1;
+            per_sm = b;
+        }
+        const uint64_t tiles = (n + FusedShape::T - 1) / FusedShape::T;
+        uint64_t cap = static_cast<uint64_t>(cfg.sm_count) * per_sm;
+        if (cfg.debug_max_ctas && cfg.debug_max_ctas < cap) cap = cfg.debug_max_ctas;
+        PassParams pp;
+        pp.shift = 0;
+        pp.dbits = 8;
+        pp.epoch = epoch;
+        pp.place = 0;
+        pp.spin_cap = cfg.spin_cap;
+        pp.stall_every = cfg.debug_stall_every;
+        pp.plan = nullptr;
+        pp.region = region;
+        pp.fused_abort = abort_word;
+        pp.fused_hist = ghist;
+        KeyCodec codec = cfg.codec;
+        codec.flags &= kCodecEncodeOnLoad;
+        *ctas = static_cast<uint32_t>(tiles < cap ? tiles : cap);
+        kern<<<*ctas, FusedShape::S::THREADS, FusedShape::smem, stream>>>(
+            const_cast<uint32_t*>(keys), alt, nullptr, nullptr, n, nullptr, agg16, desc, ticket, pp, codec);
+        return cudaGetLastError();
+    });
+}
+
 cudaError_t launch_digit_binning(const void* in, void* out, const uint32_t* in_val, uint32_t* out_val, uint64_t n,
                                  int key_bytes, uint32_t shift, const unsigned long long* gbase_place, uint64_t* desc,
                                  uint16_t* agg16, uint32_t* ticket, uint32_t epoch, const BinningConfig& cfg,
@@ -2014,6 +2239,8 @@
     if (e == cudaSuccess) e = for_each_type(RingShapes{}, shape);
     if (e == cudaSuccess) e = for_each_type(TileShapes{}, shape);
     if (e == cudaSuccess) e = for_each_type(SegShapes{}, shape);
+    if (e == cudaSuccess) e = set_smem(fused_kernel<kRankAtomic>(), FusedShape::smem);
+    if (e == cudaSuccess) e = set_smem(fused_kernel<kRankBallot>(), FusedShape::smem);
     return e;
 }
 
diff --git a/gpusorting_b200/csrc/osb_kernels.cuh b/gpusorting_b200/csrc/osb_kernels.cuh
--- a/gpusorting_b200/csrc/osb_kernels.cuh
+++ b/gpusorting_b200/csrc/osb_kernels.cuh
@@ -30,6 +30,8 @@
     uint32_t debug_max_ctas = 0;
     bool hot_passes = false;
     const void* argsort_in = nullptr;
+    uint64_t fused_region = 0;
+    const unsigned long long* fused_dense_base0 = nullptr;
 };
 
 uint32_t binning_tile_keys(int key_bytes, bool pairs, const BinningConfig& cfg);
@@ -38,7 +40,16 @@
 cudaError_t configure_kernels();
 
 cudaError_t launch_global_histogram(const void* keys, uint64_t n, int key_bytes, unsigned long long* ghist,
-                                    int sm_count, cudaStream_t stream, const KeyCodec* codec = nullptr);
+                                    int sm_count, cudaStream_t stream, const KeyCodec* codec = nullptr, const SortPlan* gate = nullptr);
+
+cudaError_t launch_fused_first_pass(const uint32_t* keys, uint32_t* alt, uint64_t n, uint64_t region, unsigned long long* ghist,
+                                    uint32_t* abort_word, uint64_t* desc, uint16_t* agg16, uint32_t* ticket, uint32_t epoch,
+                                    const BinningConfig& cfg, cudaStream_t stream, uint32_t* ctas);
+cudaError_t launch_scan_fused(const unsigned long long* ghist, unsigned long long* gbase, int places, cudaStream_t stream,
+                              SortPlan* plan, uint64_t n, bool allow_skip, bool allow_hot, bool fallback, const uint32_t* fused_abort,
+                              uint64_t region);
+cudaError_t launch_fused_fallback_zero(const SortPlan* plan, const uint32_t* ticket, uint32_t ctas, uint64_t tiles, uint16_t* agg16,
+                                       uint64_t* desc, int sm_count, cudaStream_t stream);
 
 cudaError_t launch_digit_histogram(const void* keys, uint64_t n, int key_bytes, uint32_t shift,
                                    unsigned long long* hist256, int sm_count, cudaStream_t stream);
```

Measured after the change: 68.21, median of 6. +5.4%, better.
